# owkin/PyDESeq2

Measured on AMD Instinct MI355X. Metric: genes/sec end-to-end deseq2() (size factors->dispersion->IRLS->Wald), higher is better.
Workload: dtype f64

## Files before the change

include/deseq_hip.h:

```cpp
#ifndef DESEQ_HIP_H
#define DESEQ_HIP_H

#include <stddef.h>
#include <stdint.h>

#ifdef __cplusplus
extern "C" {
#endif

#define DSQ_ABI_VERSION 5
#define DSQ_MAX_P 128
#define DSQ_SHRINK_MAX_P 48
#define DSQ_BFGS_MAX_P 12

typedef struct dsq_ctx dsq_ctx;

enum dsq_status {
    DSQ_OK = 0,
    DSQ_ERR_HIP = -1,
    DSQ_ERR_ARG = -2,
    DSQ_ERR_RANGE = -3,
    DSQ_ERR_NOMEM = -4
};

// ... 15 lines not shown
int dsq_sync(dsq_ctx* ctx);
const char* dsq_debug_pending_error(void);
int dsq_timer_start(dsq_ctx* ctx);
int dsq_timer_stop(dsq_ctx* ctx, float* elapsed_ms);
int dsq_last_alpha_kernel(dsq_ctx* ctx, float* kernel_ms, int* n_grid_fallback);

int dsq_malloc(dsq_ctx* ctx, size_t bytes, void** dptr);
int dsq_free(dsq_ctx* ctx, void* dptr);
int dsq_memset(dsq_ctx* ctx, void* dptr, int value, size_t bytes);
int dsq_h2d(dsq_ctx* ctx, void* dst, const void* src, size_t bytes);
int dsq_d2h(dsq_ctx* ctx, void* dst, const void* src, size_t bytes);
int dsq_h2d_2d(dsq_ctx* ctx, void* dst, size_t dpitch, const void* src, size_t spitch,
               size_t row_bytes, size_t rows);
int dsq_d2h_2d(dsq_ctx* ctx, void* dst, size_t dpitch, const void* src, size_t spitch,
               size_t row_bytes, size_t rows);

int dsq_abi_version(void);
int dsq_plugin_cache_config(dsq_ctx* ctx, int enabled, long long budget_bytes);
int dsq_plugin_cache_clear(dsq_ctx* ctx);
int dsq_plugin_cache_stats(dsq_ctx* ctx, double* out, int n);
int dsq_plugin_digest_host(const void* data, int elem_type, int layout, int N, int G, int n_threads,
                           unsigned long long* out2);

int dsq_inf_lin_reg_mu(dsq_ctx* ctx, const void* counts, int count_type, int count_layout,
                       const double* size_factors, const double* design, int N, int G, int P,
                       double min_mu, double* mu_out);

int dsq_inf_irls2(dsq_ctx* ctx, const void* counts, int count_type, int count_layout,
                  const double* size_factors, const double* design, const double* disp, int N,
                  int G, int P, double min_mu, double beta_tol, double min_beta, double max_beta,
                  int maxiter, double* beta_out, double* mu_out, double* hat_out,
                  uint8_t* converged, int optimizer);
int dsq_inf_irls(dsq_ctx* ctx, const void* counts, int count_type, int count_layout,
                 const double* size_factors, const double* design, const double* disp, int N,
                 int G, int P, double min_mu, double beta_tol, double min_beta, double max_beta,
                 int maxiter, double* beta_out, double* mu_out, double* hat_out,
                 uint8_t* converged);

int dsq_inf_alpha_mle2(dsq_ctx* ctx, const void* counts, int count_type, int count_layout,
                       const double* design, const double* mu, int mu_layout,
                       const double* alpha_hat, int N, int G, int P, double min_disp,
                       double max_disp, double prior_disp_var, int cr_reg, int prior_reg,
                       double* alpha_out, uint8_t* converged, int optimizer);
int dsq_inf_alpha_mle(dsq_ctx* ctx, const void* counts, int count_type, int count_layout,
                      const double* design, const double* mu, int mu_layout,
                      const double* alpha_hat, int N, int G, int P, double min_disp,
                      double max_disp, double prior_disp_var, int cr_reg, int prior_reg,
                      double* alpha_out, uint8_t* converged);

int dsq_inf_wald_test(dsq_ctx* ctx, const double* design, const double* disp, const double* lfc,
                      const double* mu, int mu_layout, const double* ridge,
                      const double* contrast, double lfc_null, int alt, int N, int G, int P,
                      double* pvals, double* stats, double* se);

int dsq_inf_fit_rough_dispersions(dsq_ctx* ctx, const double* normed, int layout,
                                  const double* design, int N, int G, int P, double* alpha_out);
int dsq_inf_fit_moments_dispersions(dsq_ctx* ctx, const double* normed, int layout,
                                    const double* size_factors, int N, int G, double* alpha_out);
int dsq_inf_fit_moments_dispersions2(dsq_ctx* ctx, const double* normed, int layout, const double* size_factors,
                                     int N, int G, double* alpha_out, uint8_t* all_zero);

int dsq_inf_dispersion_trend_gamma_glm(dsq_ctx* ctx, const double* covariates, const double* targets, int n,
                                       double* coeffs2, double* predictions, int* converged);

int dsq_inf_grid_fit_alpha(dsq_ctx* ctx, const void* counts, int count_type, int count_layout, const double* design,
                           const double* mu, int mu_layout, int N, int G, int P, double min_disp, double max_disp,
                           double* log_alpha_out);
int dsq_inf_grid_fit_beta(dsq_ctx* ctx, const void* counts, int count_type, int count_layout,
                          const double* size_factors, const double* design, const double* disp, int N, int G,
                          double min_mu, int grid_length, double min_beta, double max_beta, double* beta_out);

int dsq_dev_trend_loss_grad(dsq_ctx* ctx, const double* d_cov, const double* d_targets,
                            const uint8_t* d_keep, int n, double a0, double a1, double* loss,
                            double* grad2);

int dsq_dev_trend_fit(dsq_ctx* ctx, const double* d_disp, const double* d_means, int n,
                      double min_disp, double max_disp, uint8_t* d_keep, double* h_coeffs2,
                      int* h_ok, int* h_n_outer);

size_t dsq_prior_mad_work_doubles(int n);
int dsq_dev_prior_mad(dsq_ctx* ctx, const double* d_gw_raw, const double* d_fitted, int n,
                      double min_disp, double max_disp, double* d_work, double* h_squared_logres);


int dsq_dev_counts_to_gene_major(dsq_ctx* ctx, const void* d_src, int count_type, int layout,
                                 int N, int G, int32_t* d_dst, int ldn, int* h_bad);
int dsq_dev_f64_to_gene_major(dsq_ctx* ctx, const double* d_src, int layout, int N, int G,
                              double* d_dst, int ldn);

int dsq_dev_logmeans(dsq_ctx* ctx, const int32_t* d_y, int ldn, int N, int G, double* d_logmeans,
                     uint8_t* d_nonzero);
size_t dsq_size_factors_work_doubles(int N, int G);
int dsq_dev_size_factors(dsq_ctx* ctx, const void* d_counts_sm, int count_type, int N, int G,
                         const double* d_logmeans, const uint8_t* d_gene_mask, double* d_work,
                         double* d_size_factors);
int dsq_dev_size_factors_new(dsq_ctx* ctx, const void* d_counts_sm, int count_type, int N, int G,
                             const double* d_logmeans, const uint8_t* d_gene_mask, double* d_work,
                             double* d_size_factors);
int dsq_dev_mom_lin_mu(dsq_ctx* ctx, const int32_t* d_y, int ldn, const double* d_sf, const double* d_Xt,
                       const double* d_pinvXt, int ldx, int N, int G, int P, double min_disp, double max_disp,
                       double min_mu, double* d_normed_mean, double* d_mom, double* d_mu);
int dsq_dev_mom(dsq_ctx* ctx, const int32_t* d_y, int ldn, const double* d_sf, const double* d_Xt,
                const double* d_pinvXt, int ldx, int N, int G, int P, double min_disp,
                double max_disp, double* d_normed_mean, double* d_rough, double* d_moments,
                double* d_mom);
int dsq_dev_lin_mu(dsq_ctx* ctx, const int32_t* d_y, int ldn, const double* d_sf,
                   const double* d_Xt, const double* d_pinvXt, int ldx, int N, int G, int P,
                   double min_mu, double* d_mu);
int dsq_dev_alpha_mle(dsq_ctx* ctx, const int32_t* d_y, const double* d_mu, int ldn,
                      const double* d_Xt, int ldx, int N, int G, int P, const double* d_alpha_hat,
                      double min_disp, double max_disp, double prior_disp_var, int cr_reg,
                      int prior_reg, double* d_alpha, uint8_t* d_converged, int32_t* d_nfev,
                      double* d_nll_const, int const_mode);
typedef struct dsq_cells {
    const int32_t* d_cell_of;
    const double* d_Xc;
    const double* d_XX;
    int n_cells;
} dsq_cells;
int dsq_dev_mom_lin_coef(dsq_ctx* ctx, const int32_t* d_y, int ldn, const double* d_sf, const double* d_Xt,
                         const double* d_pinvXt, int ldx, int N, int G, int P, double min_disp, double max_disp,
                         double min_mu, double* d_normed_mean, double* d_mom, double* d_mu, double* d_coef);
int dsq_dev_alpha_mle2(dsq_ctx* ctx, const int32_t* d_y, const double* d_mu, int ldn, const double* d_Xt, int ldx,
                       int N, int G, int P, const double* d_alpha_hat, double min_disp, double max_disp,
                       double prior_disp_var, int cr_reg, int prior_reg, double* d_alpha, uint8_t* d_converged,
                       int32_t* d_nfev, double* d_nll_const, int const_mode, const dsq_cells* cells,
                       const double* d_coef, const double* d_sf, double min_mu);
int dsq_dev_alpha_mle3(dsq_ctx* ctx, const int32_t* d_y, const double* d_mu, int ldn, const double* d_Xt, int ldx,
                       int N, int G, int P, const double* d_alpha_hat, double min_disp, double max_disp,
                       double prior_disp_var, int cr_reg, int prior_reg, double* d_alpha, uint8_t* d_converged,
                       int32_t* d_nfev, double* d_nll_const, int const_mode, const dsq_cells* cells,
                       const double* d_coef, const double* d_sf, double min_mu, const int32_t* d_rows, int n_rows,
                       const int32_t* d_waves, int n_waves, const double* d_cell_mu);
typedef struct dsq_mix dsq_mix;
int dsq_mix_create(dsq_ctx* ctx, const double* design, int N, int P, dsq_mix** out);
void dsq_mix_destroy(dsq_mix* mix);
int dsq_mix_info(const dsq_mix* mix, int* n_slots, int* n_cells, int* n_continuous);
int dsq_mix_slots(const dsq_mix* mix, int32_t* h_slot_of);
int dsq_mix_bind(dsq_ctx* ctx, const uint16_t* d_ys, const uint8_t* d_big, const double* d_mu_slots);
int dsq_mix_bind2(dsq_ctx* ctx, const uint16_t* d_ys, const uint8_t* d_big, const double* d_mu_slots, int G);
int dsq_dev_mix_counts_to_slots(dsq_ctx* ctx, const int32_t* d_y, int ldn, int G, const dsq_mix* mix, uint16_t* d_ys,
                                uint8_t* d_big);
int dsq_dev_mix_mu_slots(dsq_ctx* ctx, const dsq_mix* mix, const double* d_beta, const double* d_sf, int G,
                         double* d_mu_slots);
int dsq_mix_takes_irls(const dsq_mix* mix, int full_rank);
int dsq_mix_launch_count(void);
int dsq_dev_alpha_mle4(dsq_ctx* ctx, const int32_t* d_y, const double* d_mu, int ldn, const double* d_Xt, int ldx,
                       int N, int G, int P, const double* d_alpha_hat, double min_disp, double max_disp,
                       double prior_disp_var, int cr_reg, int prior_reg, double* d_alpha, uint8_t* d_converged,
                       int32_t* d_nfev, double* d_nll_const, int const_mode, const dsq_cells* cells,
                       const double* d_coef, const double* d_sf, double min_mu, const int32_t* d_rows, int n_rows,
                       const int32_t* d_waves, int n_waves, const double* d_cell_mu, const dsq_mix* mix,
                       const double* d_beta);
int dsq_alpha_rows_eligible(int N, int P, int n_cells);
int dsq_alpha_needs_mu(int N, int P, int n_cells);
int dsq_dev_cell_mu(dsq_ctx* ctx, const double* d_beta, const dsq_cells* cells, int G, int P, double* d_cell_mu);
int dsq_dev_alpha_row_split(dsq_ctx* ctx, const int32_t* d_y, int ldn, int N, int G, int32_t* d_flags);
int dsq_dev_robust_disp(dsq_ctx* ctx, const int32_t* d_y, int ldn, const double* d_sf, const int32_t* d_cell_offsets,
                        const int32_t* d_cell_index, int n_cells, int whole, int max_cell, int N, int G,
                        double* d_robust_disp);
int dsq_dev_robust_disp2(dsq_ctx* ctx, const int32_t* d_y, int ldn, const double* d_sf, const int32_t* d_cell_offsets,
                         const int32_t* d_cell_index, int n_cells, int whole, int max_cell, int min_cell, int N, int G,
                         double* d_robust_disp);
int dsq_dev_lfc_fit(dsq_ctx* ctx, const int32_t* d_y, int ldn, const double* d_sf, const double* d_Xt,
                    const double* d_pinvXt, int ldx, int N, int G, int P, int full_rank, const double* d_disp,
                    double min_mu, double beta_tol, double min_beta, double max_beta, int maxiter, double* d_beta,
                    double* d_mu, double* d_hat, uint8_t* d_converged, int32_t* d_iters, const dsq_cells* cells,
                    const double* d_robust_disp, const uint8_t* d_flags, double cutoff, double* d_cooks,
                    uint8_t* d_any_all, uint8_t* d_any_use, uint8_t* d_any_use_nr, uint8_t* d_few_above,
                    const double* h_ridge, const double* h_contrast, double lfc_null, int alt, double* d_pvals,
                    double* d_stats, double* d_se);
int dsq_dev_lfc_fit2(dsq_ctx* ctx, const int32_t* d_y, int ldn, const double* d_sf, const double* d_Xt,
                     const double* d_pinvXt, int ldx, int N, int G, int P, int full_rank, const double* d_disp,
                     double min_mu, double beta_tol, double min_beta, double max_beta, int maxiter, double* d_beta,
                     double* d_mu, double* d_hat, uint8_t* d_converged, int32_t* d_iters, const dsq_cells* cells,
                     const double* d_robust_disp, const uint8_t* d_flags, double cutoff, double* d_cooks,
                     uint8_t* d_any_all, uint8_t* d_any_use, uint8_t* d_any_use_nr, uint8_t* d_few_above,
                     const double* h_ridge, const double* h_contrast, double lfc_null, int alt, double* d_pvals,
                     double* d_stats, double* d_se, const dsq_mix* mix, int cooks_ld);
int dsq_dev_replace_outliers2(dsq_ctx* ctx, const int32_t* d_y, const double* d_cooks, int ldn, const double* d_sf,
                              const uint8_t* d_flags, const int32_t* d_gene_idx, int n_sel, int N, double cutoff,
                              int32_t* d_y_out, uint8_t* d_all_zero, int cooks_ld, const dsq_mix* mix);
int dsq_dev_irls_layers(dsq_ctx* ctx, const int32_t* d_y, int ldn, const double* d_sf, const double* d_Xt, int ldx,
                        int N, int G, int P, const double* d_disp, const double* d_beta, double min_mu, double* d_mu,
                        double* d_hat);
int dsq_side_begin(dsq_ctx* ctx);
int dsq_side_end(dsq_ctx* ctx);
int dsq_side_wait(dsq_ctx* ctx);
int dsq_side_abort(dsq_ctx* ctx);
int dsq_dev_irls(dsq_ctx* ctx, const int32_t* d_y, int ldn, const double* d_sf, const double* d_Xt,
                 const double* d_pinvXt, int ldx, int N, int G, int P, int full_rank,
                 const double* d_disp, double min_mu, double beta_tol, double min_beta,
                 double max_beta, int maxiter, double* d_beta, double* d_mu, double* d_hat,
                 uint8_t* d_converged, int32_t* d_iters);
int dsq_dev_cooks(dsq_ctx* ctx, const int32_t* d_y, int ldn, const double* d_sf, const double* d_mu,
                  const double* d_hat, const int32_t* d_cell_offsets, const int32_t* d_cell_index,
                  int n_cells, int whole, int max_cell, const uint8_t* d_flags, int N, int G, int P,
                  double cutoff, double* d_cooks, double* d_robust_disp, uint8_t* d_any_all,
                  uint8_t* d_any_use, uint8_t* d_any_use_nr, uint8_t* d_few_above);
int dsq_dev_replace_outliers(dsq_ctx* ctx, const int32_t* d_y, const double* d_cooks, int ldn,
                             const double* d_sf, const uint8_t* d_flags, const int32_t* d_gene_idx,
                             int n_sel, int N, double cutoff, int32_t* d_y_out,
                             uint8_t* d_all_zero);
int dsq_dev_wald(dsq_ctx* ctx, const double* d_mu, int ldn, const double* d_sf, const double* d_Xt,
                 int ldx, int N, int G, int P, const double* d_disp, const double* d_beta,
                 const double* h_ridge, const double* h_contrast, double lfc_null, int alt,
                 double* d_pvals, double* d_stats, double* d_se);
int dsq_dev_lrt(dsq_ctx* ctx, const int32_t* d_y, int ldn, const double* d_sf, const double* d_Xt, int ldx, int P,
                const double* d_Xt_reduced, int ldx_reduced, int P_reduced, int N, int G, const double* d_disp,
                const double* d_beta, const double* d_beta_reduced, double* d_stats, double* d_pvals);
int dsq_dev_chisq_sf(dsq_ctx* ctx, const double* d_x, int n, int df, double* d_out);
int dsq_dev_trend_prior(dsq_ctx* ctx, const double* d_disp, const double* d_means, int n, double min_disp,
                        double max_disp, uint8_t* d_keep, double* d_fitted, double* d_work, double* h_coeffs2,
                        int* h_ok, int* h_n_outer, double* h_squared_logres);
int dsq_lfc_fork_begin(dsq_ctx* ctx);
int dsq_lfc_fork_end(dsq_ctx* ctx);
int dsq_lfc_set_part(dsq_ctx* ctx, const uint8_t* d_part, int want, int phase);
int dsq_lfc_takes_parts(int N, int P, const dsq_cells* cells, const dsq_mix* mix, int full_rank);
int dsq_dev_select_dispersions_part(dsq_ctx* ctx, double* d_genewise_raw, double* d_map_raw, const double* d_fitted, int n,
                                    double min_disp, double max_disp, double squared_logres, double* d_disp,
                                    uint8_t* d_outlier, uint8_t* d_map_converged, const uint8_t* d_conv_late, uint8_t* d_part,
                                    int mode, int ready_limit);
int dsq_alpha_set_late_flags(dsq_ctx* ctx, uint8_t* d_conv_late);
int dsq_lfc_prepare(dsq_ctx* ctx, const double* d_sf, int N, const double* h_ridge, const double* h_contrast, int P);
int dsq_dev_trend_eval(dsq_ctx* ctx, const double* d_normed_means, int n, double a0, double a1,
                       double* d_fitted);
int dsq_dev_select_dispersions(dsq_ctx* ctx, double* d_genewise_raw, double* d_map_raw,
                               const double* d_fitted, int n, double min_disp, double max_disp,
                               double squared_logres, double* d_disp, uint8_t* d_outlier);
int dsq_dev_scatter_rows_f64(dsq_ctx* ctx, const double* d_src, const int32_t* d_idx, int n_idx, int width,
                             double* d_dst);
int dsq_dev_mom_raw(dsq_ctx* ctx, const int32_t* d_y, int ldn, const double* d_ones, const double* d_sf,
                    const double* d_Xt, const double* d_pinvXt, int ldx, int N, int G, int P, double min_disp,
                    double max_disp, double* d_normed_mean, double* d_mom);
int dsq_dev_nll_const(dsq_ctx* ctx, const int32_t* d_y, int ldn, int N, int G, const double* d_disp, double* d_cst);
int dsq_dev_nll_scaled(dsq_ctx* ctx, const int32_t* d_y, const double* d_mu, int ldn, int N, int G,
                       const double* d_disp, const double* d_scale, const double* d_cst, double* d_nll);
int dsq_dev_logmeans_poscounts(dsq_ctx* ctx, const int32_t* d_y, int ldn, int N, int G, double* d_logmeans,
                               uint8_t* d_usable);
int dsq_dev_vst(dsq_ctx* ctx, const void* d_counts_sm, int count_type, int N, int G, const double* d_sf, int mode,
                double a0, double a1, double* d_out);
int dsq_inf_lfc_shrink_nbinom_glm2(dsq_ctx* ctx, const void* counts, int count_type, int count_layout,
                                   const double* design, const double* size, const double* offset, int N, int G,
                                   int P, double prior_no_shrink_scale, double prior_scale, int shrink_index,
                                   double* beta_out, double* inv_hessian_out, uint8_t* converged, int optimizer);
int dsq_inf_lfc_shrink_nbinom_glm(dsq_ctx* ctx, const void* counts, int count_type, int count_layout,
                                  const double* design, const double* size, const double* offset, int N, int G,
                                  int P, double prior_no_shrink_scale, double prior_scale, int shrink_index,
                                  double* beta_out, double* inv_hessian_out, uint8_t* converged);
int dsq_dev_lfc_shrink(dsq_ctx* ctx, const int32_t* d_y, int ldn, const double* d_offset, const double* d_Xt,
                       int ldx, int N, int G, int P, const double* d_size, double prior_no_shrink_scale,
                       double prior_scale, int shrink_index, double* d_beta, double* d_inv_hessian,
                       uint8_t* d_converged);
int dsq_dev_lfc_shrink2(dsq_ctx* ctx, const int32_t* d_y, int ldn, const double* d_offset, const double* d_Xt,
                        int ldx, int N, int G, int P, const double* d_size, double prior_no_shrink_scale,
                        double prior_scale, int shrink_index, double* d_beta, double* d_inv_hessian,
                        uint8_t* d_converged, double* d_ih_entry);
int dsq_dev_lfc_shrink3(dsq_ctx* ctx, const int32_t* d_y, int ldn, const double* d_offset, const double* d_Xt,
                        int ldx, int N, int G, int P, const double* d_size, double prior_no_shrink_scale,
                        double prior_scale, int shrink_index, double* d_beta, double* d_inv_hessian,
                        uint8_t* d_converged, double* d_ih_entry, int optimizer);
int dsq_dev_padj_prepare(dsq_ctx* ctx, const double* d_base_mean, const double* d_pvalue, int n, double alpha,
                         unsigned long long* d_sorted_p, int32_t* d_sorted_idx, uint8_t* d_bins,
                         double* h_out200, int* h_n_valid);
int dsq_dev_padj_finish(dsq_ctx* ctx, const unsigned long long* d_sorted_p, const int32_t* d_sorted_idx,
                        const uint8_t* d_bins, int n, int n_valid, int j, double* d_padj);
int dsq_upload_counts_i32(dsq_ctx* ctx, const void* counts, int count_type, size_t n_elems, int32_t* d_dst,
                          int* h_bad);
int dsq_d2d(dsq_ctx* ctx, void* d_dst, const void* d_src, size_t bytes);
int dsq_host_alloc(dsq_ctx* ctx, size_t bytes, void** out);
int dsq_host_free(dsq_ctx* ctx, void* p);
int dsq_d2h_async(dsq_ctx* ctx, void* pinned_dst, const void* d_src, size_t bytes);
int dsq_h2d_async(dsq_ctx* ctx, void* d_dst, const void* pinned_src, size_t bytes);
int dsq_dev_gather_rows_f64(dsq_ctx* ctx, const double* d_src, int ld, const int32_t* d_idx,
                            int n_idx, int ncols, double* d_dst);
int dsq_dev_gather_rows_i32(dsq_ctx* ctx, const int32_t* d_src, int ld, const int32_t* d_idx,
                            int n_idx, int ncols, int32_t* d_dst);

int dsq_comm_unique_id(dsq_ctx* ctx, char* out128, int len);
int dsq_comm_init(dsq_ctx* ctx, const char* uid128, int rank, int world);
int dsq_comm_destroy(dsq_ctx* ctx);
int dsq_comm_allreduce_sum(dsq_ctx* ctx, void* d_buf, size_t count, int dtype );
int dsq_comm_allgather(dsq_ctx* ctx, const void* d_send, void* d_recv, size_t bytes_per_rank);
int dsq_comm_info(dsq_ctx* ctx, int* nranks, int* rank);
unsigned long long dsq_host_sync_count(void);
int dsq_dev_pack2(dsq_ctx* ctx, const double* d_a, const double* d_b, int n, int len, double* d_send);
int dsq_dev_unzip2(dsq_ctx* ctx, const double* d_recv, int world, int len, double* d_a_all, double* d_b_all);

int dsq_dev_sf_keys(dsq_ctx* ctx, const void* d_counts_sm, int count_type, int N, int G,
                    const double* d_logmeans, const uint8_t* d_gene_mask, void* d_keys);
int dsq_dev_sf_keys_compact(dsq_ctx* ctx, const void* d_counts_sm, int count_type, int N, int G,
                            const double* d_logmeans, const uint8_t* d_gene_mask, int32_t* d_idx_work, void* d_keys,
                            int* h_n_usable);
int dsq_dev_sf_count(dsq_ctx* ctx, const void* d_keys, int N, int G, uint32_t* d_counts);
int dsq_dev_sf_init(dsq_ctx* ctx, const uint32_t* d_total, int N, void* d_prefix, uint32_t* d_rank);
int dsq_dev_sf_hist(dsq_ctx* ctx, const void* d_keys, int N, int G, const void* d_prefix, int shift,
                    uint32_t* d_hist);
int dsq_dev_sf_pick(dsq_ctx* ctx, const uint32_t* d_hist, int N, int shift, void* d_prefix,
                    uint32_t* d_rank);
int dsq_dev_sf_finish(dsq_ctx* ctx, const void* d_prefix, const uint32_t* d_total, int N, double* d_sf);

#ifdef __cplusplus
}
#endif
#endif
```

pydeseq2_amd/_lib.py:

```python
from __future__ import annotations

import ctypes as C
import os

import numpy as np

_HERE = os.path.dirname(os.path.abspath(__file__))
LIB_PATH = os.environ.get("DSQ_LIB", os.path.join(_HERE, "libdeseq_hip.so"))

DSQ_MAX_P = 128
DSQ_SHRINK_MAX_P = 48
_DEBUG = bool(os.environ.get("DSQ_DEBUG"))
SAMPLE_MAJOR, GENE_MAJOR = 0, 1
I32, I64 = 0, 1
ALT = {None: 0, "greaterAbs": 1, "lessAbs": 2, "greater": 3, "less": 4}

c_void_p, c_int, c_double, c_size_t = C.c_void_p, C.c_int, C.c_double, C.c_size_t
_vp = c_void_p
HOOK_FN = C.CFUNCTYPE(None, c_void_p)


class DsqCells(C.Structure):

    _fields_ = [("d_cell_of", C.c_void_p), ("d_Xc", C.c_void_p), ("d_XX", C.c_void_p), ("n_cells", C.c_int)]


class DsqError(RuntimeError):
    """A libdeseq_hip call failed (HIP error, bad argument, out of memory)."""


_lib = None


def load():
    global _lib
    if _lib is not None:
        return _lib
    if not os.path.exists(LIB_PATH):
        raise DsqError(
            f"{LIB_PATH} not found: build it with `make -C pydeseq2_amd/csrc` "
            "(or __graft_entry__.build()).  pydeseq2_amd has no CPU fallback."
        )
    lib = C.CDLL(LIB_PATH)

    def proto(name, *argtypes, res=c_int):
        fn = getattr(lib, name)
        fn.argtypes = list(argtypes)
        fn.restype = res
        return fn

    proto("dsq_create", c_int, C.POINTER(_vp))
    proto("dsq_destroy", _vp, res=None)
    proto("dsq_last_error", _vp, res=C.c_char_p)
    proto("dsq_device_info", _vp, C.c_char_p, c_int, C.POINTER(c_int), C.POINTER(c_size_t), C.c_char_p, c_int)
    proto("dsq_sync", _vp)
    proto("dsq_debug_pending_error", res=C.c_char_p)
    proto("dsq_timer_start", _vp)
    proto("dsq_timer_stop", _vp, C.POINTER(C.c_float))
    proto("dsq_last_alpha_kernel", _vp, C.POINTER(C.c_float), C.POINTER(c_int))
    proto("dsq_malloc", _vp, c_size_t, C.POINTER(_vp))
    proto("dsq_free", _vp, _vp)
    proto("dsq_memset", _vp, _vp, c_int, c_size_t)
    proto("dsq_h2d", _vp, _vp, _vp, c_size_t)
    proto("dsq_d2h", _vp, _vp, _vp, c_size_t)
    proto("dsq_h2d_2d", _vp, _vp, c_size_t, _vp, c_size_t, c_size_t, c_size_t)
    proto("dsq_d2h_2d", _vp, _vp, c_size_t, _vp, c_size_t, c_size_t, c_size_t)
    proto("dsq_inf_lin_reg_mu", _vp, _vp, c_int, c_int, _vp, _vp, c_int, c_int, c_int, c_double, _vp)
    proto("dsq_inf_irls2", _vp, _vp, c_int, c_int, _vp, _vp, _vp, c_int, c_int, c_int, c_double, c_double,
          c_double, c_double, c_int, _vp, _vp, _vp, _vp, c_int)
    proto("dsq_inf_irls", _vp, _vp, c_int, c_int, _vp, _vp, _vp, c_int, c_int, c_int, c_double, c_double,
          c_double, c_double, c_int, _vp, _vp, _vp, _vp)
    proto("dsq_inf_alpha_mle2", _vp, _vp, c_int, c_int, _vp, _vp, c_int, _vp, c_int, c_int, c_int, c_double,
          c_double, c_double, c_int, c_int, _vp, _vp, c_int)
    proto("dsq_inf_alpha_mle", _vp, _vp, c_int, c_int, _vp, _vp, c_int, _vp, c_int, c_int, c_int, c_double,
          c_double, c_double, c_int, c_int, _vp, _vp)
    proto("dsq_abi_version", res=c_int)
    proto("dsq_plugin_cache_config", _vp, c_int, C.c_longlong)
    proto("dsq_plugin_cache_clear", _vp)
    proto("dsq_plugin_cache_stats", _vp, C.POINTER(c_double), c_int)
    proto("dsq_comm_info", _vp, C.POINTER(c_int), C.POINTER(c_int))
    proto("dsq_mix_bind", _vp, _vp, _vp, _vp)
    proto("dsq_mix_bind2", _vp, _vp, _vp, _vp, c_int)
    proto("dsq_dev_mix_counts_to_slots", _vp, _vp, c_int, c_int, _vp, _vp, _vp)
    proto("dsq_dev_mix_mu_slots", _vp, _vp, _vp, _vp, c_int, _vp)
    proto("dsq_host_sync_count", res=C.c_ulonglong)
    proto("dsq_dev_pack2", _vp, _vp, _vp, c_int, c_int, _vp)
    proto("dsq_dev_unzip2", _vp, _vp, c_int, c_int, _vp, _vp)
    proto("dsq_plugin_digest_host", _vp, c_int, c_int, c_int, c_int, c_int, C.POINTER(C.c_ulonglong))
    proto("dsq_inf_wald_test", _vp, _vp, _vp, _vp, _vp, c_int, _vp, _vp, c_double, c_int, c_int, c_int,
          c_int, _vp, _vp, _vp)
    proto("dsq_inf_fit_rough_dispersions", _vp, _vp, c_int, _vp, c_int, c_int, c_int, _vp)
    proto("dsq_inf_fit_moments_dispersions", _vp, _vp, c_int, _vp, c_int, c_int, _vp)
    proto("dsq_inf_fit_moments_dispersions2", _vp, _vp, c_int, _vp, c_int, c_int, _vp, _vp)
    proto("dsq_inf_dispersion_trend_gamma_glm", _vp, _vp, _vp, c_int, _vp, _vp, C.POINTER(c_int))
    proto("dsq_inf_grid_fit_alpha", _vp, _vp, c_int, c_int, _vp, _vp, c_int, c_int, c_int, c_int, c_double, c_double,
          _vp)
    proto("dsq_inf_grid_fit_beta", _vp, _vp, c_int, c_int, _vp, _vp, _vp, c_int, c_int, c_double, c_int, c_double,
          c_double, _vp)
    proto("dsq_dev_trend_loss_grad", _vp, _vp, _vp, _vp, c_int, c_double, c_double, C.POINTER(c_double),
          C.POINTER(c_double))
    proto("dsq_dev_trend_fit", _vp, _vp, _vp, c_int, c_double, c_double, _vp, C.POINTER(c_double),
          C.POINTER(c_int), C.POINTER(c_int))
    proto("dsq_dev_prior_mad", _vp, _vp, _vp, c_int, c_double, c_double, _vp, C.POINTER(c_double))
    proto("dsq_dev_counts_to_gene_major", _vp, _vp, c_int, c_int, c_int, c_int, _vp, c_int, C.POINTER(c_int))
    proto("dsq_dev_f64_to_gene_major", _vp, _vp, c_int, c_int, c_int, _vp, c_int)
    proto("dsq_dev_logmeans", _vp, _vp, c_int, c_int, c_int, _vp, _vp)
    proto("dsq_dev_size_factors", _vp, _vp, c_int, c_int, c_int, _vp, _vp, _vp, _vp)
    proto("dsq_dev_size_factors_new", _vp, _vp, c_int, c_int, c_int, _vp, _vp, _vp, _vp)
    proto("dsq_dev_mom", _vp, _vp, c_int, _vp, _vp, _vp, c_int, c_int, c_int, c_int, c_double, c_double,
          _vp, _vp, _vp, _vp)
    proto("dsq_dev_lin_mu", _vp, _vp, c_int, _vp, _vp, _vp, c_int, c_int, c_int, c_int, c_double, _vp)
    proto("dsq_dev_trend_eval", _vp, _vp, c_int, c_double, c_double, _vp)
    proto("dsq_dev_trend_prior", _vp, _vp, _vp, c_int, c_double, c_double, _vp, _vp, _vp, _vp, _vp, _vp, _vp)
    proto("dsq_dev_select_dispersions", _vp, _vp, _vp, _vp, c_int, c_double, c_double, c_double, _vp, _vp)
    proto("dsq_dev_scatter_rows_f64", _vp, _vp, _vp, c_int, c_int, _vp)
    proto("dsq_dev_sf_keys_compact", _vp, _vp, c_int, c_int, c_int, _vp, _vp, _vp, _vp, C.POINTER(c_int))
    proto("dsq_prior_mad_work_doubles", c_int, res=c_size_t)
    proto("dsq_size_factors_work_doubles", c_int, c_int, res=c_size_t)
    proto("dsq_dev_mom_lin_mu", _vp, _vp, c_int, _vp, _vp, _vp, c_int, c_int, c_int, c_int, c_double, c_double,
          c_double, _vp, _vp, _vp)
    proto("dsq_dev_mom_raw", _vp, _vp, c_int, _vp, _vp, _vp, _vp, c_int, c_int, c_int, c_int, c_double, c_double,
          _vp, _vp)
    proto("dsq_dev_nll_const", _vp, _vp, c_int, c_int, c_int, _vp, _vp)
    proto("dsq_dev_nll_scaled", _vp, _vp, _vp, c_int, c_int, c_int, _vp, _vp, _vp, _vp)
    proto("dsq_dev_logmeans_poscounts", _vp, _vp, c_int, c_int, c_int, _vp, _vp)
    proto("dsq_dev_vst", _vp, _vp, c_int, c_int, c_int, _vp, c_int, c_double, c_double, _vp)
    proto("dsq_inf_lfc_shrink_nbinom_glm2", _vp, _vp, c_int, c_int, _vp, _vp, _vp, c_int, c_int, c_int, c_double,
          c_double, c_int, _vp, _vp, _vp, c_int)
    proto("dsq_inf_lfc_shrink_nbinom_glm", _vp, _vp, c_int, c_int, _vp, _vp, _vp, c_int, c_int, c_int, c_double,
          c_double, c_int, _vp, _vp, _vp)
    proto("dsq_dev_lfc_shrink", _vp, _vp, c_int, _vp, _vp, c_int, c_int, c_int, c_int, _vp, c_double, c_double,
          c_int, _vp, _vp, _vp)
    proto("dsq_dev_lfc_shrink2", _vp, _vp, c_int, _vp, _vp, c_int, c_int, c_int, c_int, _vp, c_double, c_double,
          c_int, _vp, _vp, _vp, _vp)
    proto("dsq_dev_lfc_shrink3", _vp, _vp, c_int, _vp, _vp, c_int, c_int, c_int, c_int, _vp, c_double, c_double,
          c_int, _vp, _vp, _vp, _vp, c_int)
    proto("dsq_dev_padj_prepare", _vp, _vp, _vp, c_int, c_double, _vp, _vp, _vp, _vp, C.POINTER(c_int))
    proto("dsq_dev_padj_finish", _vp, _vp, _vp, _vp, c_int, c_int, c_int, _vp)
    proto("dsq_d2d", _vp, _vp, _vp, c_size_t)
    cells_p = C.POINTER(DsqCells)
    proto("dsq_dev_mom_lin_coef", _vp, _vp, c_int, _vp, _vp, _vp, c_int, c_int, c_int, c_int, c_double, c_double,
          c_double, _vp, _vp, _vp, _vp)
    proto("dsq_dev_alpha_mle2", _vp, _vp, _vp, c_int, _vp, c_int, c_int, c_int, c_int, _vp, c_double, c_double,
          c_double, c_int, c_int, _vp, _vp, _vp, _vp, c_int, cells_p, _vp, _vp, c_double)
    proto("dsq_dev_alpha_mle3", _vp, _vp, _vp, c_int, _vp, c_int, c_int, c_int, c_int, _vp, c_double, c_double,
          c_double, c_int, c_int, _vp, _vp, _vp, _vp, c_int, cells_p, _vp, _vp, c_double, _vp, c_int, _vp, c_int, _vp)
    proto("dsq_dev_alpha_mle4", _vp, _vp, _vp, c_int, _vp, c_int, c_int, c_int, c_int, _vp, c_double, c_double,
          c_double, c_int, c_int, _vp, _vp, _vp, _vp, c_int, cells_p, _vp, _vp, c_double, _vp, c_int, _vp, c_int, _vp,
          _vp, _vp)
    proto("dsq_mix_create", _vp, _vp, c_int, c_int, C.POINTER(_vp))
    proto("dsq_mix_destroy", _vp, res=None)
    proto("dsq_mix_launch_count")
    proto("dsq_mix_slots", _vp, _vp)
    proto("dsq_mix_takes_irls", _vp, c_int)
    proto("dsq_mix_info", _vp, C.POINTER(c_int), C.POINTER(c_int), C.POINTER(c_int))
    proto("dsq_alpha_rows_eligible", c_int, c_int, c_int)
    proto("dsq_alpha_needs_mu", c_int, c_int, c_int)
    proto("dsq_dev_cell_mu", _vp, _vp, cells_p, c_int, c_int, _vp)
    proto("dsq_dev_alpha_row_split", _vp, _vp, c_int, c_int, c_int, _vp)
    proto("dsq_dev_robust_disp", _vp, _vp, c_int, _vp, _vp, _vp, c_int, c_int, c_int, c_int, c_int, _vp)
    proto("dsq_dev_robust_disp2", _vp, _vp, c_int, _vp, _vp, _vp, c_int, c_int, c_int, c_int, c_int, c_int, _vp)
    proto("dsq_dev_lfc_fit", _vp, _vp, c_int, _vp, _vp, _vp, c_int, c_int, c_int, c_int, c_int, _vp, c_double,
          c_double, c_double, c_double, c_int, _vp, _vp, _vp, _vp, _vp, cells_p, _vp, _vp, c_double, _vp, _vp, _vp,
          _vp, _vp, _vp, _vp, c_double, c_int, _vp, _vp, _vp)
    proto("dsq_dev_lfc_fit2", _vp, _vp, c_int, _vp, _vp, _vp, c_int, c_int, c_int, c_int, c_int, _vp, c_double,
          c_double, c_double, c_double, c_int, _vp, _vp, _vp, _vp, _vp, cells_p, _vp, _vp, c_double, _vp, _vp, _vp,
          _vp, _vp, _vp, _vp, c_double, c_int, _vp, _vp, _vp, _vp, c_int)
    proto("dsq_dev_irls_layers", _vp, _vp, c_int, _vp, _vp, c_int, c_int, c_int, c_int, _vp, _vp, c_double, _vp, _vp)
    proto("dsq_side_begin", _vp)
    proto("dsq_side_end", _vp)
    proto("dsq_side_wait", _vp)
    proto("dsq_side_abort", _vp)
    proto("dsq_set_deferred", _vp, c_int)
    proto("dsq_lfc_fork_begin", _vp)
    proto("dsq_lfc_fork_end", _vp)
    proto("dsq_lfc_set_part", _vp, _vp, c_int, c_int)
    proto("dsq_lfc_takes_parts", c_int, c_int, cells_p, _vp, c_int)
    proto("dsq_dev_select_dispersions_part", _vp, _vp, _vp, _vp, c_int, c_double, c_double, c_double, _vp, _vp, _vp, _vp, _vp,
          c_int, c_int)
    proto("dsq_alpha_set_late_flags", _vp, _vp)
    proto("dsq_lfc_prepare", _vp, _vp, c_int, _vp, _vp, c_int)
    proto("dsq_irls_order_hint", _vp, _vp, c_int)
    proto("dsq_set_alpha_hook", _vp, _vp, _vp)
    proto("dsq_upload_counts_i32", _vp, _vp, c_int, c_size_t, _vp, C.POINTER(c_int))
    proto("dsq_host_alloc", _vp, c_size_t, C.POINTER(_vp))
    proto("dsq_host_free", _vp, _vp)
    proto("dsq_d2h_async", _vp, _vp, _vp, c_size_t)
    proto("dsq_h2d_async", _vp, _vp, _vp, c_size_t)
    proto("dsq_dev_alpha_mle", _vp, _vp, _vp, c_int, _vp, c_int, c_int, c_int, c_int, _vp, c_double,
          c_double, c_double, c_int, c_int, _vp, _vp, _vp, _vp, c_int)
    proto("dsq_dev_irls", _vp, _vp, c_int, _vp, _vp, _vp, c_int, c_int, c_int, c_int, c_int, _vp, c_double,
          c_double, c_double, c_double, c_int, _vp, _vp, _vp, _vp, _vp)
    proto("dsq_dev_cooks", _vp, _vp, c_int, _vp, _vp, _vp, _vp, _vp, c_int, c_int, c_int, _vp, c_int, c_int,
          c_int, c_double, _vp, _vp, _vp, _vp, _vp, _vp)
    proto("dsq_dev_replace_outliers", _vp, _vp, _vp, c_int, _vp, _vp, _vp, c_int, c_int, c_double, _vp, _vp)
    proto("dsq_dev_replace_outliers2", _vp, _vp, _vp, c_int, _vp, _vp, _vp, c_int, c_int, c_double, _vp, _vp, c_int, _vp)
    proto("dsq_dev_wald", _vp, _vp, c_int, _vp, _vp, c_int, c_int, c_int, c_int, _vp, _vp, _vp, _vp,
          c_double, c_int, _vp, _vp, _vp)
    proto("dsq_dev_lrt", _vp, _vp, c_int, _vp, _vp, c_int, c_int, _vp, c_int, c_int, c_int, c_int, _vp, _vp, _vp, _vp, _vp)
    proto("dsq_dev_chisq_sf", _vp, _vp, c_int, c_int, _vp)
    proto("dsq_dev_gather_rows_f64", _vp, _vp, c_int, _vp, c_int, c_int, _vp)
    proto("dsq_dev_gather_rows_i32", _vp, _vp, c_int, _vp, c_int, c_int, _vp)
    proto("dsq_comm_unique_id", _vp, C.c_char_p, c_int)
    proto("dsq_comm_init", _vp, C.c_char_p, c_int, c_int)
    proto("dsq_comm_destroy", _vp)
    proto("dsq_comm_allreduce_sum", _vp, _vp, c_size_t, c_int)
    proto("dsq_comm_allgather", _vp, _vp, _vp, c_size_t)
    proto("dsq_dev_sf_keys", _vp, _vp, c_int, c_int, c_int, _vp, _vp, _vp)
    proto("dsq_dev_sf_count", _vp, _vp, c_int, c_int, _vp)
    proto("dsq_dev_sf_init", _vp, _vp, c_int, _vp, _vp)
    proto("dsq_dev_sf_hist", _vp, _vp, c_int, c_int, _vp, c_int, _vp)
    proto("dsq_dev_sf_pick", _vp, _vp, c_int, c_int, _vp, _vp)
    proto("dsq_dev_sf_finish", _vp, _vp, _vp, c_int, _vp)
    _lib = lib
    return lib


EXPORTS = [
    "dsq_create", "dsq_destroy", "dsq_last_error", "dsq_device_info", "dsq_sync", "dsq_debug_pending_error", "dsq_timer_start",
    "dsq_timer_stop", "dsq_last_alpha_kernel", "dsq_malloc", "dsq_free", "dsq_memset", "dsq_h2d", "dsq_d2h", "dsq_h2d_2d",
    "dsq_d2h_2d", "dsq_inf_lin_reg_mu", "dsq_inf_irls", "dsq_inf_alpha_mle", "dsq_inf_wald_test",
    "dsq_inf_fit_rough_dispersions", "dsq_inf_fit_moments_dispersions", "dsq_dev_trend_loss_grad", "dsq_dev_trend_fit", "dsq_dev_prior_mad",
    "dsq_dev_counts_to_gene_major", "dsq_dev_f64_to_gene_major", "dsq_dev_logmeans",
    "dsq_dev_size_factors", "dsq_dev_mom", "dsq_dev_lin_mu", "dsq_dev_alpha_mle", "dsq_dev_irls",
    "dsq_dev_cooks", "dsq_dev_replace_outliers", "dsq_dev_wald", "dsq_dev_gather_rows_f64",
    "dsq_dev_gather_rows_i32", "dsq_comm_unique_id", "dsq_comm_init", "dsq_comm_destroy",
    "dsq_comm_allreduce_sum", "dsq_comm_allgather", "dsq_dev_sf_keys", "dsq_dev_sf_count", "dsq_dev_sf_init",
    "dsq_dev_sf_hist", "dsq_dev_sf_pick", "dsq_dev_sf_finish", "dsq_dev_trend_eval", "dsq_dev_trend_prior", "dsq_dev_select_dispersions",
    "dsq_dev_scatter_rows_f64", "dsq_d2d", "dsq_dev_mom_lin_mu", "dsq_dev_sf_keys_compact", "dsq_prior_mad_work_doubles", "dsq_size_factors_work_doubles", "dsq_dev_mom_raw", "dsq_dev_nll_const", "dsq_dev_nll_scaled", "dsq_dev_logmeans_poscounts", "dsq_dev_vst", "dsq_inf_lfc_shrink_nbinom_glm", "dsq_dev_lfc_shrink", "dsq_dev_lfc_shrink2", "dsq_dev_lfc_shrink3", "dsq_dev_padj_prepare", "dsq_dev_padj_finish", "dsq_host_alloc", "dsq_host_free", "dsq_d2h_async", "dsq_h2d_async",
    "dsq_dev_size_factors_new", "dsq_dev_mom_lin_coef", "dsq_dev_alpha_mle2", "dsq_dev_robust_disp", "dsq_dev_robust_disp2", "dsq_dev_lfc_fit", "dsq_dev_lfc_fit2", "dsq_dev_irls_layers",
    "dsq_side_begin", "dsq_side_end", "dsq_side_wait", "dsq_side_abort", "dsq_set_deferred", "dsq_irls_order_hint", "dsq_set_alpha_hook", "dsq_dev_alpha_mle3", "dsq_dev_alpha_mle4", "dsq_mix_create", "dsq_mix_destroy", "dsq_mix_info", "dsq_mix_slots", "dsq_mix_takes_irls", "dsq_dev_replace_outliers2", "dsq_mix_launch_count", "dsq_alpha_rows_eligible", "dsq_alpha_needs_mu", "dsq_dev_cell_mu", "dsq_dev_alpha_row_split",
    "dsq_upload_counts_i32", "dsq_inf_dispersion_trend_gamma_glm", "dsq_inf_grid_fit_alpha", "dsq_inf_grid_fit_beta",
    "dsq_inf_irls2", "dsq_inf_alpha_mle2", "dsq_inf_lfc_shrink_nbinom_glm2", "dsq_inf_fit_moments_dispersions2",
    "dsq_abi_version", "dsq_plugin_cache_config", "dsq_plugin_cache_clear", "dsq_plugin_cache_stats",
    "dsq_plugin_digest_host", "dsq_comm_info", "dsq_host_sync_count", "dsq_dev_pack2", "dsq_dev_unzip2",
    "dsq_mix_bind", "dsq_mix_bind2", "dsq_dev_mix_counts_to_slots", "dsq_dev_mix_mu_slots",
    "dsq_lfc_fork_begin", "dsq_lfc_fork_end", "dsq_lfc_set_part", "dsq_lfc_takes_parts", "dsq_dev_select_dispersions_part", "dsq_lfc_prepare", "dsq_alpha_set_late_flags",
    "dsq_dev_lrt", "dsq_dev_chisq_sf",
]


def ptr(a):
    if a is None:
        return None
    if isinstance(a, np.ndarray):
        return a.ctypes.data
    return a


class Context:

    def __init__(self, device: int = 0):
        self.lib = load()
        h = _vp()
        rc = self.lib.dsq_create(int(device), C.byref(h))
        if rc != 0 or not h.value:
            raise DsqError(
                f"dsq_create(device={device}) failed (rc={rc}): no usable MI355X / HIP runtime. "
                "pydeseq2_amd runs on the GPU only."
            )
        self.h = h
        self.device = device

    def close(self):
        if getattr(self, "h", None) is not None and self.h.value:
            for bufs in self.__dict__.pop("_padj_buffers", {}).values():
                for b in bufs:
                    b.free()
            self.lib.dsq_destroy(self.h)
            self.h = _vp()

    def __del__(self):
        try:
            self.close()
        except Exception:
            pass

    def call(self, name, *args):
        rc = getattr(self.lib, name)(self.h, *args)
        if _DEBUG:
            pend = self.lib.dsq_debug_pending_error().decode()
            if pend:
                print(f"[dsq debug] pending HIP error after {name}: {pend}", flush=True)
        if rc != 0:
            msg = self.lib.dsq_last_error(self.h).decode(errors="replace")
            if rc == -2:
                raise ValueError(msg)
            raise DsqError(f"{name} failed (rc={rc}): {msg}")

    def device_info(self):
        name, arch = C.create_string_buffer(256), C.create_string_buffer(256)
        cu, mem = c_int(), c_size_t()
        self.call("dsq_device_info", name, 256, C.byref(cu), C.byref(mem), arch, 256)
        return dict(name=name.value.decode(), arch=arch.value.decode(), cu_count=cu.value, mem_bytes=mem.value)

    def sync(self):
        self.call("dsq_sync")

    def timer_start(self):
        self.call("dsq_timer_start")

    def timer_stop(self) -> float:
        ms = C.c_float()
        self.call("dsq_timer_stop", C.byref(ms))
        return float(ms.value)

    def malloc(self, nbytes: int) -> int:
        p = _vp()
        self.call("dsq_malloc", c_size_t(int(nbytes)), C.byref(p))
        return p.value

    def free(self, dptr):
        if dptr:
            self.call("dsq_free", _vp(dptr))

    def memset(self, dptr, value, nbytes):
        self.call("dsq_memset", _vp(dptr), int(value), c_size_t(int(nbytes)))

    def h2d(self, dptr, arr: np.ndarray):
        arr = np.ascontiguousarray(arr)
        self.call("dsq_h2d", _vp(dptr), _vp(arr.ctypes.data), c_size_t(arr.nbytes))

    def d2h(self, arr: np.ndarray, dptr):
        assert arr.flags.c_contiguous
        self.call("dsq_d2h", _vp(arr.ctypes.data), _vp(dptr), c_size_t(arr.nbytes))
        return arr

    def d2h_rows(self, dptr, rows, cols, ld, dtype=np.float64):
        out = np.empty((rows, cols), dtype=dtype)
        isz = out.itemsize
        self.call("dsq_d2h_2d", _vp(out.ctypes.data), c_size_t(cols * isz), _vp(dptr), c_size_t(ld * isz),
                  c_size_t(cols * isz), c_size_t(rows))
        return out

    def h2d_rows(self, dptr, arr: np.ndarray, ld):
        arr = np.ascontiguousarray(arr)
        rows, cols = arr.shape
        isz = arr.itemsize
        self.call("dsq_h2d_2d", _vp(dptr), c_size_t(ld * isz), _vp(arr.ctypes.data), c_size_t(cols * isz),
                  c_size_t(cols * isz), c_size_t(rows))


class DeviceArray:

    def __init__(self, ctx: Context, shape, dtype, ld=None):
        self.ctx = ctx
        self.shape = tuple(shape) if isinstance(shape, (tuple, list)) else (int(shape),)
        self.dtype = np.dtype(dtype)
        self.ld = ld if ld is not None else (self.shape[-1] if len(self.shape) > 1 else None)
        n = self.shape[0] * (self.ld if len(self.shape) > 1 else 1)
        self.nbytes = int(n) * self.dtype.itemsize
        self.ptr = ctx.malloc(self.nbytes)

    @classmethod
    def from_host(cls, ctx, arr, ld=None):
        arr = np.ascontiguousarray(arr)
        self = cls(ctx, arr.shape, arr.dtype, ld)
        if arr.ndim == 2 and self.ld != arr.shape[1]:
            ctx.h2d_rows(self.ptr, arr, self.ld)
        else:
            ctx.h2d(self.ptr, arr)
        return self

    def to_host(self):
        if len(self.shape) == 2 and self.ld != self.shape[1]:
            return self.ctx.d2h_rows(self.ptr, self.shape[0], self.shape[1], self.ld, self.dtype)
        out = np.empty(self.shape, dtype=self.dtype)
        return self.ctx.d2h(out, self.ptr)

    def free(self):
        if self.ptr:
            self.ctx.free(self.ptr)
            self.ptr = 0

    def __del__(self):
        try:
            self.free()
        except Exception:
            pass


class _PinnedPool:

    def __init__(self, ctx):
        self.ctx, self.free, self.closed = ctx, [], False

    def take(self, nbytes):
        best = None
        for k, (cap, ptr) in enumerate(self.free):
            if nbytes <= cap <= 2 * nbytes + 65536 and (best is None or cap < self.free[best][0]):
                best = k
# ... 46 lines not shown
```

pydeseq2_amd/csrc/dsq_alpha_rows.h:

```cpp
#pragma once
#include "dsq_alpha.h"
#include "dsq_launch.h"

namespace dsq {

constexpr int kRowLanes = 16;
constexpr int kRowSlots = 4;
constexpr int kRowWaves = 4;
constexpr int kRowBlock = 64 * kRowWaves;

struct RowGene {
    Lbfgsb1d m;
    double cst, la_hat;
    double q[4];
    int g;
    int n_tail;
    int n_big;
    int pad_;
};

DSQ_HD size_t row_slot_bytes(int npad) {
    return (sizeof(RowGene) + (size_t)npad * 2 + (size_t)kRowTail * 2 + 15) & ~(size_t)15;
}

DSQ_D void stirling_big(double z, double& lg, double& psi) {
    const double l = flog_t(z), rc = frcp(z);
    lg = (z - 0.5) * l - z + kHalfLog2Pi + stirling_tail_big(rc);
    psi = l + digamma_tail_big(rc);
}


}
```

pydeseq2_amd/csrc/dsq_capi_dev.hip:

```cpp
#include "dsq_capi_internal.h"

extern "C" {

int dsq_dev_counts_to_gene_major(dsq_ctx* ctx, const void* d_src, int count_type, int layout, int N, int G,
                                 int32_t* d_dst, int ldn, int* h_bad) {
    DSQ_CHECK_ARG(ldn >= N, "ldn < N");
    int* d_bad = (int*)ctx->d_scratch;
    DSQ_HIP(hipMemsetAsync(d_bad, 0, sizeof(int), ctx->stream));
    DSQ_HIP(dsq::launch_transpose_counts(ctx->stream, d_src, count_type, layout, N, G, d_dst, ldn, d_bad));
    if (h_bad) {
        DSQ_HIP(hipMemcpyAsync(h_bad, d_bad, sizeof(int), hipMemcpyDeviceToHost, ctx->stream));
        DSQ_HIP(hipStreamSynchronize(ctx->stream));
    }
    return DSQ_OK;
}

int dsq_dev_f64_to_gene_major(dsq_ctx* ctx, const double* d_src, int layout, int N, int G, double* d_dst,
                              int ldn) {
    DSQ_HIP(dsq::launch_transpose_f64(ctx->stream, d_src, layout, N, G, d_dst, ldn));
    return DSQ_OK;
}

int dsq_dev_logmeans(dsq_ctx* ctx, const int32_t* d_y, int ldn, int N, int G, double* d_logmeans,
                     uint8_t* d_nonzero) {
    DSQ_HIP(dsq::launch_logmeans(ctx->stream, d_y, ldn, N, G, d_logmeans, d_nonzero));
    return DSQ_OK;
}

int dsq_dev_logmeans_poscounts(dsq_ctx* ctx, const int32_t* d_y, int ldn, int N, int G, double* d_logmeans,
                               uint8_t* d_usable) {
    DSQ_HIP(dsq::launch_logmeans_pos(ctx->stream, d_y, ldn, N, G, d_logmeans, d_usable));
    return DSQ_OK;
}

size_t dsq_size_factors_work_doubles(int N, int G) { return dsq::size_factors_work_doubles(N, G); }

int dsq_dev_size_factors(dsq_ctx* ctx, const void* d_counts_sm, int count_type, int N, int G,
                         const double* d_logmeans, const uint8_t* d_gene_mask, double* d_work,
                         double* d_size_factors) {
    DSQ_HIP(dsq::launch_size_factors(ctx->stream, d_counts_sm, count_type, N, G, d_logmeans, d_gene_mask,
                                     d_work, d_size_factors));
    return DSQ_OK;
}

int dsq_dev_size_factors_new(dsq_ctx* ctx, const void* d_counts_sm, int count_type, int N, int G,
                             const double* d_logmeans, const uint8_t* d_gene_mask, double* d_work,
                             double* d_size_factors) {
    DSQ_HIP(dsq::launch_size_factors(ctx->stream, d_counts_sm, count_type, N, G, d_logmeans, d_gene_mask,
                                     d_work, d_size_factors, 1));
    return DSQ_OK;
}

int dsq_dev_mom(dsq_ctx* ctx, const int32_t* d_y, int ldn, const double* d_sf, const double* d_Xt,
                const double* d_pinvXt, int ldx, int N, int G, int P, double min_disp, double max_disp,
                double* d_normed_mean, double* d_rough, double* d_moments, double* d_mom) {
    DSQ_CHECK_ARG(P >= 1 && P <= DSQ_MAX_P, "P out of range");
    DSQ_CHECK_ARG(N != P, "The number of samples and the number of design variables are equal, i.e., "
                          "there are no replicates to estimate the dispersion.");
    DSQ_HIP(dsq::launch_mom(ctx->stream, d_y, ldn, d_sf, d_Xt, d_pinvXt, ldx, N, G, P, min_disp, max_disp,
                            d_normed_mean, d_rough, d_moments, d_mom, ctx->d_scratch + 8));
    return DSQ_OK;
}

int dsq_dev_mom_lin_mu(dsq_ctx* ctx, const int32_t* d_y, int ldn, const double* d_sf, const double* d_Xt,
                       const double* d_pinvXt, int ldx, int N, int G, int P, double min_disp, double max_disp,
                       double min_mu, double* d_normed_mean, double* d_mom, double* d_mu) {
    DSQ_CHECK_ARG(P >= 1 && P <= DSQ_MAX_P, "P out of range");
    DSQ_CHECK_ARG(N != P, "The number of samples and the number of design variables are equal, i.e., "
                          "there are no replicates to estimate the dispersion.");
    DSQ_HIP(dsq::launch_mom_lin_mu(ctx->stream, d_y, ldn, d_sf, d_Xt, d_pinvXt, ldx, N, G, P, min_disp, max_disp,
                                   min_mu, d_normed_mean, d_mom, d_mu, ctx->d_scratch + 8));
    return DSQ_OK;
}

int dsq_dev_mom_lin_coef(dsq_ctx* ctx, const int32_t* d_y, int ldn, const double* d_sf, const double* d_Xt,
                         const double* d_pinvXt, int ldx, int N, int G, int P, double min_disp, double max_disp,
                         double min_mu, double* d_normed_mean, double* d_mom, double* d_mu, double* d_coef) {
    DSQ_CHECK_ARG(P >= 1 && P <= DSQ_MAX_P, "P out of range");
    DSQ_CHECK_ARG(N != P, "The number of samples and the number of design variables are equal, i.e., "
                          "there are no replicates to estimate the dispersion.");
    DSQ_HIP(dsq::launch_mom_lin_mu(ctx->stream, d_y, ldn, d_sf, d_Xt, d_pinvXt, ldx, N, G, P, min_disp, max_disp,
                                   min_mu, d_normed_mean, d_mom, d_mu, ctx->d_scratch + 8, d_coef));
    return DSQ_OK;
}

int dsq_dev_mom_raw(dsq_ctx* ctx, const int32_t* d_y, int ldn, const double* d_ones, const double* d_sf,
                    const double* d_Xt, const double* d_pinvXt, int ldx, int N, int G, int P, double min_disp,
                    double max_disp, double* d_normed_mean, double* d_mom) {
    DSQ_CHECK_ARG(P >= 1 && P <= DSQ_MAX_P, "P out of range");
    DSQ_CHECK_ARG(N != P, "The number of samples and the number of design variables are equal, i.e., "
                          "there are no replicates to estimate the dispersion.");
    DSQ_HIP(dsq::launch_mom(ctx->stream, d_y, ldn, d_ones, d_Xt, d_pinvXt, ldx, N, G, P, min_disp, max_disp,
                            d_normed_mean, nullptr, nullptr, d_mom, ctx->d_scratch + 8, d_sf));
    return DSQ_OK;
}

int dsq_dev_nll_const(dsq_ctx* ctx, const int32_t* d_y, int ldn, int N, int G, const double* d_disp, double* d_cst) {
    DSQ_HIP(dsq::launch_nll_const(ctx->stream, d_y, ldn, N, G, d_disp, d_cst));
    return DSQ_OK;
}

int dsq_dev_nll_scaled(dsq_ctx* ctx, const int32_t* d_y, const double* d_mu, int ldn, int N, int G,
                       const double* d_disp, const double* d_scale, const double* d_cst, double* d_nll) {
    DSQ_HIP(dsq::launch_nll_scaled(ctx->stream, d_y, d_mu, ldn, N, G, d_disp, d_scale, d_cst, d_nll));
    return DSQ_OK;
}

int dsq_dev_lin_mu(dsq_ctx* ctx, const int32_t* d_y, int ldn, const double* d_sf, const double* d_Xt,
                   const double* d_pinvXt, int ldx, int N, int G, int P, double min_mu, double* d_mu) {
    DSQ_CHECK_ARG(P >= 1 && P <= DSQ_MAX_P, "P out of range");
    DSQ_HIP(dsq::launch_lin_mu(ctx->stream, d_y, ldn, d_sf, d_Xt, d_pinvXt, ldx, N, G, P, min_mu, d_mu));
    return DSQ_OK;
}

int dsq_dev_alpha_mle(dsq_ctx* ctx, const int32_t* d_y, const double* d_mu, int ldn, const double* d_Xt,
                      int ldx, int N, int G, int P, const double* d_alpha_hat, double min_disp,
                      double max_disp, double prior_disp_var, int cr_reg, int prior_reg, double* d_alpha,
                      uint8_t* d_converged, int32_t* d_nfev, double* d_nll_const, int const_mode) {
    DSQ_CHECK_ARG(P >= 1 && P <= DSQ_MAX_P, "P out of range");
    DSQ_CHECK_ARG(const_mode >= DSQ_CONST_COMPUTE && const_mode <= DSQ_CONST_LOAD, "const_mode out of range");
    return run_alpha(ctx, d_y, d_mu, ldn, d_Xt, ldx, N, G, P, d_alpha_hat, min_disp, max_disp, prior_disp_var,
                     cr_reg, prior_reg, d_alpha, d_converged, d_nfev, d_nll_const, const_mode);
}


int dsq_set_alpha_hook(dsq_ctx* ctx, dsq_hook_fn fn, void* arg) {
    ctx->alpha_hook = fn;
    ctx->alpha_hook_arg = arg;
    return DSQ_OK;
}

int dsq_irls_order_hint(dsq_ctx* ctx, const int32_t* d_iters, int G) {
    ctx->d_irls_hint = d_iters;
    ctx->irls_hint_genes = d_iters != nullptr ? G : 0;
    return DSQ_OK;
}


int dsq_dev_irls(dsq_ctx* ctx, const int32_t* d_y, int ldn, const double* d_sf, const double* d_Xt,
                 const double* d_pinvXt, int ldx, int N, int G, int P, int full_rank, const double* d_disp,
                 double min_mu, double beta_tol, double min_beta, double max_beta, int maxiter,
                 double* d_beta, double* d_mu, double* d_hat, uint8_t* d_converged, int32_t* d_iters) {
    DSQ_CHECK_ARG(P >= 1 && P <= DSQ_MAX_P, "P out of range");
    return run_irls(ctx, d_y, ldn, d_sf, d_Xt, d_pinvXt, ldx, N, G, P, full_rank, d_disp, min_mu, beta_tol, min_beta,
                    max_beta, maxiter, d_beta, d_mu, d_hat, d_converged, d_iters, nullptr);
}


int dsq_dev_alpha_mle4(dsq_ctx* ctx, const int32_t* d_y, const double* d_mu, int ldn, const double* d_Xt, int ldx,
                       int N, int G, int P, const double* d_alpha_hat, double min_disp, double max_disp,
                       double prior_disp_var, int cr_reg, int prior_reg, double* d_alpha, uint8_t* d_converged,
                       int32_t* d_nfev, double* d_nll_const, int const_mode, const dsq_cells* cells,
                       const double* d_coef, const double* d_sf, double min_mu, const int32_t* d_rows, int n_rows,
                       const int32_t* d_waves, int n_waves, const double* d_cell_mu, const dsq_mix* mix,
                       const double* d_beta) {
    DSQ_CHECK_ARG(P >= 1 && P <= DSQ_MAX_P, "P out of range");
    DSQ_CHECK_ARG(const_mode >= DSQ_CONST_COMPUTE && const_mode <= DSQ_CONST_LOAD, "const_mode out of range");
    DSQ_CHECK_ARG(d_mu != nullptr || (d_coef != nullptr && d_sf != nullptr) ||
                      (d_cell_mu != nullptr && d_sf != nullptr && cells != nullptr && cells->n_cells > 0) ||
                      (mix != nullptr && d_beta != nullptr && d_sf != nullptr),
                  "mu_hat is needed as a matrix, as (coef, sf), as (cell_mu, sf, cells) or as (mix, beta, sf)");
    DSQ_CHECK_ARG(mix == nullptr || (mix->d.P == P && mix->d.N == N && d_rows != nullptr),
                  "mix: built for another design, or the gene lists are missing");
    DSQ_CHECK_ARG(d_beta == nullptr || (mix != nullptr && d_mu == nullptr && d_coef == nullptr && d_cell_mu == nullptr &&
                                        n_waves == 0),
                  "beta: with mix only, alone, and every gene on the mixed-design kernel");
    DSQ_CHECK_ARG(d_cell_mu == nullptr || (d_mu == nullptr && d_coef == nullptr && !dsq::alpha_is_wide(P, cells->n_cells)),
                  "cell_mu: alone, on the register kernels");
    DSQ_CHECK_ARG(cells == nullptr || cells->n_cells <= dsq::kMaxCells, "too many design cells for the cell path");
    DSQ_CHECK_ARG(d_rows == nullptr || (n_rows >= 0 && n_waves >= 0 && n_rows + n_waves == G &&
                                        (n_waves == 0 || d_waves != nullptr)),
                  "the two gene lists must partition the G genes of the call");
    dsq::AlphaExtras ex{};
    ex.cells = to_cells(cells);
    if (d_mu == nullptr) { ex.coef = d_coef; ex.cell_mu = d_cell_mu; ex.sf = d_sf; ex.min_mu = min_mu; }
    if (d_rows != nullptr) { ex.rows = d_rows; ex.n_rows = n_rows; ex.waves = d_waves; ex.n_waves = n_waves; }
    if (mix != nullptr) { ex.mix = &mix->d; ex.mix_beta = d_beta; ex.sf = d_sf; }
    return run_alpha(ctx, d_y, d_mu, ldn, d_Xt, ldx, N, G, P, d_alpha_hat, min_disp, max_disp, prior_disp_var, cr_reg,
                     prior_reg, d_alpha, d_converged, d_nfev, d_nll_const, const_mode, &ex);
}

int dsq_dev_alpha_mle3(dsq_ctx* ctx, const int32_t* d_y, const double* d_mu, int ldn, const double* d_Xt, int ldx,
                       int N, int G, int P, const double* d_alpha_hat, double min_disp, double max_disp,
                       double prior_disp_var, int cr_reg, int prior_reg, double* d_alpha, uint8_t* d_converged,
                       int32_t* d_nfev, double* d_nll_const, int const_mode, const dsq_cells* cells,
                       const double* d_coef, const double* d_sf, double min_mu, const int32_t* d_rows, int n_rows,
                       const int32_t* d_waves, int n_waves, const double* d_cell_mu) {
    return dsq_dev_alpha_mle4(ctx, d_y, d_mu, ldn, d_Xt, ldx, N, G, P, d_alpha_hat, min_disp, max_disp, prior_disp_var,
                              cr_reg, prior_reg, d_alpha, d_converged, d_nfev, d_nll_const, const_mode, cells, d_coef,
                              d_sf, min_mu, d_rows, n_rows, d_waves, n_waves, d_cell_mu, nullptr, nullptr);
}

int dsq_dev_alpha_mle2(dsq_ctx* ctx, const int32_t* d_y, const double* d_mu, int ldn, const double* d_Xt, int ldx,
                       int N, int G, int P, const double* d_alpha_hat, double min_disp, double max_disp,
                       double prior_disp_var, int cr_reg, int prior_reg, double* d_alpha, uint8_t* d_converged,
                       int32_t* d_nfev, double* d_nll_const, int const_mode, const dsq_cells* cells,
                       const double* d_coef, const double* d_sf, double min_mu) {
    return dsq_dev_alpha_mle3(ctx, d_y, d_mu, ldn, d_Xt, ldx, N, G, P, d_alpha_hat, min_disp, max_disp, prior_disp_var,
                              cr_reg, prior_reg, d_alpha, d_converged, d_nfev, d_nll_const, const_mode, cells, d_coef,
                              d_sf, min_mu, nullptr, 0, nullptr, 0, nullptr);
}

int dsq_mix_create(dsq_ctx* ctx, const double* design, int N, int P, dsq_mix** out) {
    DSQ_CHECK_ARG(out != nullptr && design != nullptr, "null argument");
    *out = nullptr;
    DSQ_HIP(hipSetDevice(ctx->device));
    if (P < 1 || P > dsq::kMixMaxP || N < 2 || N > 65535 || !dsq::alpha_mix_enabled()) return DSQ_OK;
    const bool force = getenv("DSQ_MIX_FORCE") != nullptr;
    std::vector<int> nd((size_t)P), order((size_t)P);
    for (int j = 0; j < P; ++j) {
        std::vector<double> col((size_t)N);
        for (int n = 0; n < N; ++n) col[(size_t)n] = design[(size_t)n * P + j];
        std::sort(col.begin(), col.end());
        nd[(size_t)j] = (int)(std::unique(col.begin(), col.end()) - col.begin());
        order[(size_t)j] = j;
    }
    std::stable_sort(order.begin(), order.end(), [&](int a, int b) { return nd[(size_t)a] > nd[(size_t)b]; });
    std::vector<char> cont((size_t)P, 0);
    std::vector<int> idx((size_t)N), cell((size_t)N);
    int C = 0;
    auto less_cat = [&](int a, int b) {
        for (int j = 0; j < P; ++j) {
            if (cont[(size_t)j]) continue;
            const double va = design[(size_t)a * P + j], vb = design[(size_t)b * P + j];
            if (va != vb) return va < vb;
        }
        return a < b;
    };
    auto same_cat = [&](int a, int b) {
        for (int j = 0; j < P; ++j)
            if (!cont[(size_t)j] && design[(size_t)a * P + j] != design[(size_t)b * P + j]) return false;
        return true;
    };
    auto find_cells = [&]() {
        for (int n = 0; n < N; ++n) idx[(size_t)n] = n;
        std::sort(idx.begin(), idx.end(), less_cat);
        C = 0;
        for (int k = 0; k < N; ++k) {
            if (k > 0 && !same_cat(idx[(size_t)k - 1], idx[(size_t)k])) ++C;
            cell[(size_t)idx[(size_t)k]] = C;
        }
        ++C;
    };
    int Q = 0;
    find_cells();
    while (C > dsq::kMixMaxCells && Q < dsq::kMixMaxQ && Q < P) {
        cont[(size_t)order[(size_t)Q]] = 1;
        ++Q;
        find_cells();
    }
    if (Q == 0 || C > dsq::kMixMaxCells) return DSQ_OK;
    std::vector<int> count((size_t)C, 0);
    for (int n = 0; n < N; ++n) ++count[(size_t)cell[(size_t)n]];
    const int blk = 64 * dsq::kMixU;
    int Ns = 0;
    for (int c = 0; c < C; ++c) Ns += (count[(size_t)c] + blk - 1) / blk * blk;
    Ns = (Ns + 255) & ~255;
    if (!force && Ns > N + N / 2 + 256) return DSQ_OK;
    dsq::MixDesign M{};
    M.Ns = Ns; M.C = C; M.Q = Q; M.P = P; M.N = N;
    {
        int q = 0;
        for (int j = 0; j < P; ++j) {
            M.colq[j] = cont[(size_t)j] ? q : -1;
            if (cont[(size_t)j]) M.zcol[q++] = j;
        }
    }
    if (!dsq::alpha_mix_fits(M)) return DSQ_OK;
    std::vector<int32_t> perm((size_t)Ns, -1), slot_of((size_t)N, 0);
    std::vector<uint8_t> trip_cell((size_t)(Ns / 64), (uint8_t)(C - 1));
    std::vector<double> Zs((size_t)Q * Ns, 0.0), Xc((size_t)C * P, 0.0), Ginv;
    {
        int s = 0, k = 0;
        for (int c = 0; c < C; ++c) {
            const int s0 = s;
            for (int i = 0; i < count[(size_t)c]; ++i, ++k, ++s) {
                const int n = idx[(size_t)k];
                perm[(size_t)s] = n;
                slot_of[(size_t)n] = s;
                for (int q = 0; q < Q; ++q) Zs[(size_t)q * Ns + s] = design[(size_t)n * P + M.zcol[q]];
                if (i == 0)
                    for (int j = 0; j < P; ++j) Xc[(size_t)c * P + j] = cont[(size_t)j] ? 0.0 : design[(size_t)n * P + j];
            }
            s = s0 + (count[(size_t)c] + blk - 1) / blk * blk;
            for (int t = s0 / 64; t < s / 64; ++t) trip_cell[(size_t)t] = (uint8_t)c;
        }
    }
    {
        std::vector<long double> A((size_t)P * P, 0.0L), Li((size_t)P * P, 0.0L);
        for (int n = 0; n < N; ++n)
            for (int i = 0; i < P; ++i)
                for (int j = 0; j <= i; ++j) A[(size_t)i * P + j] += (long double)design[(size_t)n * P + i] * design[(size_t)n * P + j];
        bool ok = true;
        long double dmax_ = 0.0L;
        for (int i = 0; i < P; ++i) dmax_ = std::max(dmax_, A[(size_t)i * P + i]);
        for (int j = 0; j < P && ok; ++j) {
            long double d = A[(size_t)j * P + j];
            for (int k = 0; k < j; ++k) d -= A[(size_t)j * P + k] * A[(size_t)j * P + k];
            if (!(d > dmax_ * 1e-13L)) { ok = false; break; }
            d = std::sqrt(d);
            A[(size_t)j * P + j] = d;
            for (int i = j + 1; i < P; ++i) {
                long double v = A[(size_t)i * P + j];
                for (int k = 0; k < j; ++k) v -= A[(size_t)i * P + k] * A[(size_t)j * P + k];
                A[(size_t)i * P + j] = v / d;
            }
        }
        if (ok) {
            for (int j = 0; j < P; ++j) {
                Li[(size_t)j * P + j] = 1.0L / A[(size_t)j * P + j];
                for (int i = j + 1; i < P; ++i) {
                    long double v = 0.0L;
                    for (int k = j; k < i; ++k) v -= A[(size_t)i * P + k] * Li[(size_t)k * P + j];
                    Li[(size_t)i * P + j] = v / A[(size_t)i * P + i];
                }
            }
            Ginv.assign((size_t)P * P, 0.0);
            for (int i = 0; i < P; ++i)
                for (int j = 0; j < P; ++j) {
                    long double v = 0.0L;
                    for (int k = std::max(i, j); k < P; ++k) v += Li[(size_t)k * P + i] * Li[(size_t)k * P + j];
                    Ginv[(size_t)i * P + j] = (double)v;
                }
        }
    }
    auto up = [](size_t b) { return (b + 255) & ~(size_t)255; };
    const size_t b_perm = up((size_t)Ns * 4), b_tc = up((size_t)Ns / 64), b_z = up((size_t)Q * Ns * 8),
                 b_xc = up((size_t)C * P * 8), b_g = up((size_t)P * P * 8), b_so = up((size_t)N * 4);
    dsq_mix* m = new dsq_mix();
    m->device = ctx->device;
    hipError_t e = hipMalloc(&m->d_block, b_perm + b_tc + b_z + b_xc + b_g + b_so);
    if (e != hipSuccess) { delete m; return fail(ctx, DSQ_ERR_HIP, std::string("dsq_mix_create: ") + hipGetErrorString(e)); }
    char* p = (char*)m->d_block;
    auto put = [&](const void* src, size_t bytes, size_t slot) {
        char* dst = p;
        if (e == hipSuccess && bytes) e = hipMemcpy(dst, src, bytes, hipMemcpyHostToDevice);
        p += slot;
        return dst;
    };
    M.perm = (const int32_t*)put(perm.data(), (size_t)Ns * 4, b_perm);
    M.trip_cell = (const uint8_t*)put(trip_cell.data(), (size_t)Ns / 64, b_tc);
    M.Zs = (const double*)put(Zs.data(), (size_t)Q * Ns * 8, b_z);
    M.Xc = (const double*)put(Xc.data(), (size_t)C * P * 8, b_xc);
    const char* g = put(Ginv.empty() ? nullptr : Ginv.data(), Ginv.empty() ? 0 : (size_t)P * P * 8, b_g);
    M.Ginv = Ginv.empty() ? nullptr : (const double*)g;
    M.slot_of = (const int32_t*)put(slot_of.data(), (size_t)N * 4, b_so);
    if (e != hipSuccess) {
        (void)hipFree(m->d_block);
        delete m;
        return fail(ctx, DSQ_ERR_HIP, std::string("dsq_mix_create: ") + hipGetErrorString(e));
    }
    m->d = M;
    *out = m;
    return DSQ_OK;
}

void dsq_mix_destroy(dsq_mix* mix) {
    if (mix == nullptr) return;
    (void)hipSetDevice(mix->device);
    if (mix->d_block) (void)hipFree(mix->d_block);
    delete mix;
}

int dsq_mix_slots(const dsq_mix* mix, int32_t* h_slot_of) {
    if (mix == nullptr || h_slot_of == nullptr) return DSQ_ERR_ARG;
    return hipMemcpy(h_slot_of, mix->d.slot_of, (size_t)mix->d.N * sizeof(int32_t), hipMemcpyDeviceToHost) == hipSuccess
               ? DSQ_OK
               : DSQ_ERR_HIP;
}

int dsq_mix_bind(dsq_ctx* ctx, const uint16_t* d_ys, const uint8_t* d_big, const double* d_mu_slots) {
    ctx->bind_ys = d_ys;
    ctx->bind_big = d_big;
    ctx->bind_mu = d_mu_slots;
    ctx->bind_G = 0;
    return DSQ_OK;
}

int dsq_mix_bind2(dsq_ctx* ctx, const uint16_t* d_ys, const uint8_t* d_big, const double* d_mu_slots, int G) {
    const int rc = dsq_mix_bind(ctx, d_ys, d_big, d_mu_slots);
    ctx->bind_G = (rc == DSQ_OK && G > 0) ? G : 0;
    return rc;
}
int dsq_dev_mix_counts_to_slots(dsq_ctx* ctx, const int32_t* d_y, int ldn, int G, const dsq_mix* mix, uint16_t* d_ys,
                                uint8_t* d_big) {
    DSQ_CHECK_ARG(mix != nullptr && d_y != nullptr && d_ys != nullptr && d_big != nullptr, "null argument");
    DSQ_HIP(dsq::launch_mix_counts_to_slots(ctx->stream, d_y, ldn, mix->d, G, d_ys, d_big));
    return DSQ_OK;
}
int dsq_dev_mix_mu_slots(dsq_ctx* ctx, const dsq_mix* mix, const double* d_beta, const double* d_sf, int G,
                         double* d_mu_slots) {
    DSQ_CHECK_ARG(mix != nullptr && d_beta != nullptr && d_sf != nullptr && d_mu_slots != nullptr, "null argument");
    DSQ_HIP(dsq::launch_mix_mu_slots(ctx->stream, d_beta, d_sf, mix->d, G, d_mu_slots));
    return DSQ_OK;
}

int dsq_mix_takes_irls(const dsq_mix* mix, int full_rank) {
    return (mix != nullptr && dsq::irls_takes_mix(&mix->d, full_rank)) ? 1 : 0;
}

int dsq_mix_launch_count(void) { return dsq::alpha_mix_launches(); }

int dsq_mix_info(const dsq_mix* mix, int* n_slots, int* n_cells, int* n_continuous) {
    if (mix == nullptr) return DSQ_ERR_ARG;
    if (n_slots) *n_slots = mix->d.Ns;
    if (n_cells) *n_cells = mix->d.C;
    if (n_continuous) *n_continuous = mix->d.Q;
    return DSQ_OK;
}

int dsq_alpha_needs_mu(int N, int P, int n_cells) { return dsq::alpha_needs_mu(N, P, n_cells) ? 1 : 0; }

int dsq_alpha_rows_eligible(int N, int P, int n_cells) {
    if (dsq::alpha_rows_eligible(N, P, n_cells, true, 1)) return 1;
    return dsq::alpha_rowsc_tail(N, P, n_cells) > 0 ? 2 : 0;
}

int dsq_dev_cell_mu(dsq_ctx* ctx, const double* d_beta, const dsq_cells* cells, int G, int P, double* d_cell_mu) {
    DSQ_CHECK_ARG(P >= 1 && P <= 12 && cells != nullptr && cells->n_cells > 0, "cells / P out of range");
    DSQ_HIP(dsq::launch_cell_mu(ctx->stream, d_beta, cells->d_Xc, cells->n_cells, G, P, d_cell_mu));
    return DSQ_OK;
}

int dsq_dev_alpha_row_split(dsq_ctx* ctx, const int32_t* d_y, int ldn, int N, int G, int32_t* d_flags) {
    DSQ_HIP(dsq::launch_count_big(ctx->stream, d_y, ldn, N, G, d_flags));
    return DSQ_OK;
}

int dsq_dev_robust_disp2(dsq_ctx* ctx, const int32_t* d_y, int ldn, const double* d_sf, const int32_t* d_cell_offsets,
                         const int32_t* d_cell_index, int n_cells, int whole, int max_cell, int min_cell, int N, int G,
                         double* d_robust_disp) {
    if (whole) min_cell = N;
    {
        const hipError_t pend = hipGetLastError();
        if (pend != hipSuccess)
            return fail(ctx, DSQ_ERR_HIP, std::string("HIP error pending before dsq_dev_robust_disp2: ") + hipGetErrorString(pend));
    }
    if ((size_t)G + 1 > ctx->redo_cap) {
        if (ctx->d_redo) (void)hipFree(ctx->d_redo);
        ctx->d_redo = nullptr; ctx->redo_cap = 0;
        DSQ_HIP(hipMalloc((void**)&ctx->d_redo, ((size_t)G + 1 + (size_t)G / 4) * sizeof(int32_t)));
        ctx->redo_cap = (size_t)G + 1 + (size_t)G / 4;
    }
    DSQ_HIP(dsq::launch_robust_disp(ctx->stream, d_y, ldn, d_sf, d_cell_offsets, d_cell_index, n_cells, whole, max_cell,
                                    N, G, d_robust_disp, min_cell, ctx->d_redo));
    return DSQ_OK;
}

int dsq_dev_robust_disp(dsq_ctx* ctx, const int32_t* d_y, int ldn, const double* d_sf, const int32_t* d_cell_offsets,
                        const int32_t* d_cell_index, int n_cells, int whole, int max_cell, int N, int G,
                        double* d_robust_disp) {
    return dsq_dev_robust_disp2(ctx, d_y, ldn, d_sf, d_cell_offsets, d_cell_index, n_cells, whole, max_cell, 0, N, G,
                                d_robust_disp);
}

int dsq_dev_irls_layers(dsq_ctx* ctx, const int32_t* d_y, int ldn, const double* d_sf, const double* d_Xt, int ldx,
                        int N, int G, int P, const double* d_disp, const double* d_beta, double min_mu, double* d_mu,
                        double* d_hat) {
    DSQ_CHECK_ARG(P >= 1 && P <= DSQ_MAX_P, "P out of range");
    DSQ_HIP(dsq::launch_irls_layers(ctx->stream, d_y, ldn, d_sf, d_Xt, ldx, N, G, P, d_disp, d_beta, min_mu, d_mu,
                                    d_hat));
    return DSQ_OK;
}


int dsq_dev_lfc_fit2(dsq_ctx* ctx, const int32_t* d_y, int ldn, const double* d_sf, const double* d_Xt,
                     const double* d_pinvXt, int ldx, int N, int G, int P, int full_rank, const double* d_disp,
                     double min_mu, double beta_tol, double min_beta, double max_beta, int maxiter, double* d_beta,
                     double* d_mu, double* d_hat, uint8_t* d_converged, int32_t* d_iters, const dsq_cells* cells,
                     const double* d_robust_disp, const uint8_t* d_flags, double cutoff, double* d_cooks,
                     uint8_t* d_any_all, uint8_t* d_any_use, uint8_t* d_any_use_nr, uint8_t* d_few_above,
                     const double* h_ridge, const double* h_contrast, double lfc_null, int alt, double* d_pvals,
                     double* d_stats, double* d_se, const dsq_mix* mix, int cooks_ld) {
    DSQ_CHECK_ARG(P >= 1 && P <= DSQ_MAX_P, "P out of range");
    DSQ_CHECK_ARG(mix == nullptr || (mix->d.P == P && mix->d.N == N), "mix: built for another design");
    DSQ_CHECK_ARG(cooks_ld == 0 || (mix != nullptr && cooks_ld >= mix->d.Ns && dsq::irls_takes_mix(&mix->d, full_rank)),
                  "cooks_ld: a slot-ordered Cook's layer needs a mixed design the kernel takes and a pitch >= its slots");
    DSQ_CHECK_ARG(cells == nullptr || cells->n_cells <= dsq::kMaxCells, "too many design cells for the cell path");
    DSQ_CHECK_ARG(d_flags == nullptr || (d_robust_disp && d_any_all && d_any_use && d_any_use_nr && d_few_above),
                  "the fused Cook's bookkeeping needs the robust dispersions and the four flag vectors");
    DSQ_CHECK_ARG(h_ridge == nullptr || (h_contrast && d_pvals && d_stats && d_se && alt >= 0 && alt <= 4),
                  "the fused Wald test needs contrast, outputs and a valid alternative");
    if (G <= 0) return DSQ_OK;
    dsq::IrlsExtras ex{};
    ex.cells = to_cells(cells);
    if (mix != nullptr) ex.mix = &mix->d;
    ex.cooks_ld = cooks_ld;
    if (d_flags != nullptr) {
        ex.robust_disp = d_robust_disp; ex.flags = d_flags; ex.cutoff = cutoff; ex.cooks = d_cooks;
        ex.any_all = d_any_all; ex.any_use = d_any_use; ex.any_use_nr = d_any_use_nr; ex.few_above = d_few_above;
    }
    if (h_ridge != nullptr) {
        double* d_ridge;
        double* h_stage;
        { const int rc = ridge_stage(ctx, P, &d_ridge, &h_stage); if (rc != DSQ_OK) return fail(ctx, rc, "ridge staging: out of memory"); }
        double* d_contrast = d_ridge + P * P;
        const bool in_place = ctx->lfc_part != nullptr &&
                              (ctx->lfc_phase == 2 || (ctx->lfc_phase == 1 && ctx->lfc_prepared_wald &&
                                                       ctx->lfc_prepared_N == N && ctx->lfc_prepared_P == P));
        if (!in_place) {
            std::memcpy(h_stage, h_ridge, (size_t)P * P * sizeof(double));
            std::memcpy(h_stage + P * P, h_contrast, (size_t)P * sizeof(double));
            DSQ_HIP(hipMemcpyAsync(d_ridge, h_stage, (size_t)(P * P + P) * sizeof(double), hipMemcpyHostToDevice,
                                   ctx->stream));
        }
        ex.ridge = d_ridge; ex.contrast = d_contrast; ex.lfc_null = lfc_null; ex.alt = alt;
        ex.pvals = d_pvals; ex.stats = d_stats; ex.se = d_se;
    }
    return run_irls(ctx, d_y, ldn, d_sf, d_Xt, d_pinvXt, ldx, N, G, P, full_rank, d_disp, min_mu, beta_tol, min_beta,
                    max_beta, maxiter, d_beta, d_mu, d_hat, d_converged, d_iters, &ex);
}

int dsq_dev_lfc_fit(dsq_ctx* ctx, const int32_t* d_y, int ldn, const double* d_sf, const double* d_Xt,
                    const double* d_pinvXt, int ldx, int N, int G, int P, int full_rank, const double* d_disp,
                    double min_mu, double beta_tol, double min_beta, double max_beta, int maxiter, double* d_beta,
                    double* d_mu, double* d_hat, uint8_t* d_converged, int32_t* d_iters, const dsq_cells* cells,
                    const double* d_robust_disp, const uint8_t* d_flags, double cutoff, double* d_cooks,
                    uint8_t* d_any_all, uint8_t* d_any_use, uint8_t* d_any_use_nr, uint8_t* d_few_above,
                    const double* h_ridge, const double* h_contrast, double lfc_null, int alt, double* d_pvals,
                    double* d_stats, double* d_se) {
    return dsq_dev_lfc_fit2(ctx, d_y, ldn, d_sf, d_Xt, d_pinvXt, ldx, N, G, P, full_rank, d_disp, min_mu, beta_tol,
                            min_beta, max_beta, maxiter, d_beta, d_mu, d_hat, d_converged, d_iters, cells, d_robust_disp,
                            d_flags, cutoff, d_cooks, d_any_all, d_any_use, d_any_use_nr, d_few_above, h_ridge, h_contrast,
                            lfc_null, alt, d_pvals, d_stats, d_se, nullptr, 0);
}

int dsq_dev_cooks(dsq_ctx* ctx, const int32_t* d_y, int ldn, const double* d_sf, const double* d_mu,
                  const double* d_hat, const int32_t* d_cell_offsets, const int32_t* d_cell_index,
                  int n_cells, int whole, int max_cell, const uint8_t* d_flags, int N, int G, int P,
                  double cutoff, double* d_cooks, double* d_robust_disp, uint8_t* d_any_all,
                  uint8_t* d_any_use, uint8_t* d_any_use_nr, uint8_t* d_few_above) {
    DSQ_CHECK_ARG((whole ? N : max_cell) <= 16384, "a design cell with more than 16384 samples is not supported");
    DSQ_HIP(dsq::launch_cooks(ctx->stream, d_y, ldn, d_sf, d_mu, d_hat, d_cell_offsets, d_cell_index,
                              n_cells, whole, max_cell, d_flags, N, G, P, cutoff, d_cooks, d_robust_disp,
                              d_any_all, d_any_use, d_any_use_nr, d_few_above));
    return DSQ_OK;
}

int dsq_dev_replace_outliers2(dsq_ctx* ctx, const int32_t* d_y, const double* d_cooks, int ldn,
                              const double* d_sf, const uint8_t* d_flags, const int32_t* d_gene_idx,
                              int n_sel, int N, double cutoff, int32_t* d_y_out, uint8_t* d_all_zero, int cooks_ld,
                              const dsq_mix* mix) {
    DSQ_CHECK_ARG(cooks_ld == 0 || (mix != nullptr && mix->d.N == N && cooks_ld >= mix->d.Ns),
                  "cooks_ld: a slot-ordered Cook's layer comes with the mixed design that wrote it");
    DSQ_HIP(dsq::launch_replace(ctx->stream, d_y, d_cooks, ldn, d_sf, d_flags, d_gene_idx, n_sel, N, cutoff,
                                d_y_out, d_all_zero, cooks_ld, cooks_ld != 0 ? mix->d.slot_of : nullptr));
    return DSQ_OK;
}

int dsq_dev_replace_outliers(dsq_ctx* ctx, const int32_t* d_y, const double* d_cooks, int ldn,
                             const double* d_sf, const uint8_t* d_flags, const int32_t* d_gene_idx,
                             int n_sel, int N, double cutoff, int32_t* d_y_out, uint8_t* d_all_zero) {
    return dsq_dev_replace_outliers2(ctx, d_y, d_cooks, ldn, d_sf, d_flags, d_gene_idx, n_sel, N, cutoff, d_y_out,
                                     d_all_zero, 0, nullptr);
}

int dsq_dev_wald(dsq_ctx* ctx, const double* d_mu, int ldn, const double* d_sf, const double* d_Xt, int ldx,
                 int N, int G, int P, const double* d_disp, const double* d_beta, const double* h_ridge,
                 const double* h_contrast, double lfc_null, int alt, double* d_pvals, double* d_stats,
                 double* d_se) {
    DSQ_CHECK_ARG(P >= 1 && P <= DSQ_MAX_P, "P out of range");
    DSQ_CHECK_ARG(alt >= 0 && alt <= 4, "unknown alternative hypothesis");
    double* d_ridge;
    double* h_unused;
    { const int rc = ridge_stage(ctx, P, &d_ridge, &h_unused); if (rc != DSQ_OK) return fail(ctx, rc, "ridge staging: out of memory"); }
// ... 289 lines not shown
```

pydeseq2_amd/csrc/dsq_k_alpha.hip:

```cpp
#include <atomic>
#include <type_traits>

#include "dsq_alpha.h"
#include "dsq_dispatch.h"
#include "dsq_launch.h"

#ifndef DSQ_ALPHA_WAVES_WIDE
#define DSQ_ALPHA_WAVES_WIDE 2
#endif
#ifndef DSQ_ALPHA_WAVES_NARROW
#define DSQ_ALPHA_WAVES_NARROW 3
#endif
constexpr int alpha_min_waves(int p) { return p <= 3 ? DSQ_ALPHA_WAVES_NARROW : (p <= 5 ? 2 : DSQ_ALPHA_WAVES_WIDE); }

namespace dsq {

#if defined(DSQ_PHASE_TIMING)
__device__ unsigned long long g_phase_total[16];
#endif

template <int P, bool STAGE, bool CELL = false>
__global__ __launch_bounds__(kBlock, CELL ? cell_min_waves(P) : alpha_min_waves(P)) void k_alpha(const int32_t* __restrict__ y,
                                                  const double* __restrict__ mu, int ldn,
                                                  const double* __restrict__ Xt, int ldx, int N, int G,
// ... 186 lines not shown
        GridBest o;
        o.f = __shfl_xor(best.f, m, 64);
        o.i = __shfl_xor(best.i, m, 64);
        o.nan = __shfl_xor((int)best.nan, m, 64) != 0;
        if (o.i != 0x7fffffff && (best.i == 0x7fffffff || grid_better(o, best))) best = o;
    }
    if (lane == 0) {
        const double c = linspace_at(lo, hi, kGridLen, best.i);
        if (stage == 0) {
            const double delta = linspace_at(lo, hi, kGridLen, 1) - linspace_at(lo, hi, kGridLen, 0);
            lohi[2 * k] = c - delta;
            lohi[2 * k + 1] = c + delta;
            done[k] = 0;
        } else {
            alpha[g] = exp(c);
        }
    }
}

template <int P>
__global__ __launch_bounds__(kBlock, alpha_min_waves(P)) void k_alpha_bfgs(const int32_t* __restrict__ y, const double* __restrict__ mu,
                                                       int ldn, const double* __restrict__ Xt, int ldx, int N, int G,
                                                       const double* __restrict__ alpha_hat, double min_disp,
                                                       double max_disp, double prior_var, int cr_reg, int prior_reg,
                                                       double* __restrict__ alpha, uint8_t* __restrict__ conv,
                                                       int32_t* __restrict__ nfev, int32_t* __restrict__ grid_count,
                                                       int32_t* __restrict__ grid_list) {
    log_tab_fill();
    __syncthreads();
    const int g = blockIdx.x * kWavesPerBlock + (threadIdx.x >> 6);
    if (g >= G) return;
    const int32_t* yg = y + (size_t)g * ldn;
    int maxc = 0;
    for (int n = threadIdx.x & 63; n < N; n += 64) maxc = yg[n] > maxc ? yg[n] : maxc;
    maxc = DeviceWave::maxi(maxc);
    const int memo_blocks = __builtin_amdgcn_readfirstlane(min(kMemoBlocks, (maxc >> 6) + 1));
    const AlphaOut o = fit_alpha_gene_bfgs<DeviceWave, P, false>(yg, mu + (size_t)g * ldn, Xt, ldx, N, alpha_hat[g],
                                                                 min_disp, max_disp, prior_var, cr_reg != 0,
                                                                 prior_reg != 0, memo_blocks);
    if ((threadIdx.x & 63) == 0) {
        alpha[g] = o.alpha;
        conv[g] = (uint8_t)o.converged;
        if (nfev != nullptr) nfev[g] = o.nfev;
        if (!o.converged) grid_list[atomicAdd(grid_count, 1)] = g;
    }
}

bool no_two_phase();

#define DSQ_MIX_DECL(Q_)                                                                                               \
    void alpha_mix_grid_q##Q_(int Ns, int P, int n_list, int* blocks, int* nw);                                        \
    hipError_t launch_alpha_mix_q##Q_(hipStream_t, const uint16_t*, const double*, const MixDesign&, const int32_t*, int, \
                                      const int32_t*, int32_t*, const double*, double, double, double, int, double*,   \
                                      uint8_t*, int32_t*, int32_t*, int32_t*, double*, int, int, int, void*, int32_t*,  \
                                      int32_t*);
DSQ_MIX_DECL(1)
DSQ_MIX_DECL(2)
DSQ_MIX_DECL(3)
#undef DSQ_MIX_DECL

static std::atomic<int> g_mix_launches{0};
int alpha_mix_launches() { return g_mix_launches.load(std::memory_order_relaxed); }

bool alpha_mix_enabled() {
    static const bool off = getenv("DSQ_NO_ALPHA_MIX") != nullptr;
    return !off;
}

bool alpha_mix_fits(const MixDesign& D) {
    int blocks = 0, nw = 0;
    if (D.Q == 1) alpha_mix_grid_q1(D.Ns, D.P, 1, &blocks, &nw);
    else if (D.Q == 2) alpha_mix_grid_q2(D.Ns, D.P, 1, &blocks, &nw);
    else if (D.Q == 3) alpha_mix_grid_q3(D.Ns, D.P, 1, &blocks, &nw);
    return blocks > 0;
}

hipError_t launch_alpha_mix(hipStream_t st, const uint16_t* ys, const double* mu_s, const MixDesign& D, const int32_t* list,
                            int n_list, const int32_t* n_dev, int32_t* queue, const double* alpha_hat, double min_disp,
                            double max_disp, double prior_var, int prior_reg, double* alpha, uint8_t* conv, int32_t* nfev,
                            int32_t* grid_count, int32_t* grid_list, double* nll_const, int const_mode, int eval_cap,
                            int resume, void* park_state, int32_t* park_count, int32_t* park_list) {
    g_mix_launches.fetch_add(1, std::memory_order_relaxed);
#define DSQ_MIX_CALL(Q_)                                                                                              \
    return launch_alpha_mix_q##Q_(st, ys, mu_s, D, list, n_list, n_dev, queue, alpha_hat, min_disp, max_disp, prior_var, \
                                  prior_reg, alpha, conv, nfev, grid_count, grid_list, nll_const, const_mode, eval_cap, \
                                  resume, park_state, park_count, park_list)
    switch (D.Q) {
        case 1: DSQ_MIX_CALL(1);
        case 2: DSQ_MIX_CALL(2);
        case 3: DSQ_MIX_CALL(3);
        default: return hipErrorInvalidValue;
    }
#undef DSQ_MIX_CALL
}

hipError_t launch_alpha_bfgs(hipStream_t st, const int32_t* y, const double* mu, int ldn, const double* Xt, int ldx,
                             int N, int G, int P_, const double* alpha_hat, double min_disp, double max_disp,
                             double prior_var, int cr_reg, int prior_reg, double* alpha, uint8_t* conv,
                             int32_t* nfev, int32_t* grid_count, int32_t* grid_list) {
    if (G <= 0) return hipSuccess;
    if (P_ > DSQ_REG_MAX_P || mu == nullptr) return hipErrorInvalidValue;
    DSQ_DISPATCH_P(P_, hipLaunchKernelGGL(k_alpha_bfgs<P>, dim3(genes_to_blocks(G)), dim3(kBlock), 0, st, y, mu, ldn,
                                          Xt, ldx, N, G, alpha_hat, min_disp, max_disp, prior_var, cr_reg, prior_reg,
                                          alpha, conv, nfev, grid_count, grid_list))
    return hipGetLastError();
}

hipError_t launch_alpha(hipStream_t st, const int32_t* y, const double* mu, int ldn, const double* Xt,
                        int ldx, int N, int G, int P_, const double* alpha_hat, double min_disp,
                        double max_disp, double prior_var, int cr_reg, int prior_reg, double* alpha,
                        uint8_t* conv, int32_t* nfev, int32_t* grid_count, int32_t* grid_list,
                        double* nll_const, int const_mode, const AlphaExtras* extras, int32_t* queue) {
    if (G <= 0) return hipSuccess;
    if (nll_const == nullptr) const_mode = DSQ_CONST_COMPUTE;
    AlphaExtras ex{};
    if (extras != nullptr) ex = *extras;
    ex.list = nullptr;
    bool parked = false;
    const int G_rows = ex.n_rows;
    ex.cell_mu_of = ex.cells.cell_of;
    ex.cell_mu_C = ex.cells.C;
    const bool have_lists = ex.rows != nullptr && queue != nullptr && ex.n_rows + ex.n_waves == G;
    const bool rows_reg = have_lists && ex.cell_mu == nullptr &&
                          alpha_rows_eligible(N, P_, ex.cells.C, ex.coef != nullptr, cr_reg);
    const bool rows_lds = have_lists && !rows_reg && cr_reg != 0 && (ex.coef != nullptr || ex.cell_mu != nullptr) &&
                          alpha_rowsc_tail(N, P_, ex.cells.C) > 0;
    const bool rows_mix = have_lists && ex.mix != nullptr && cr_reg != 0 && ex.mix_ys != nullptr && ex.mix_mu != nullptr &&
                          alpha_mix_enabled();
    if (rows_mix) {
        const bool park = ex.resume_state != nullptr && ex.resume_count != nullptr && ex.resume_list != nullptr &&
                          nll_const != nullptr && ex.eval_cap > 0 && !no_two_phase();
        hipError_t e = launch_alpha_mix(st, ex.mix_ys, ex.mix_mu, *ex.mix, ex.rows, ex.n_rows, nullptr, queue, alpha_hat,
                                        min_disp, max_disp, prior_var, prior_reg, alpha, conv, nfev, grid_count, grid_list,
                                        nll_const, const_mode, park ? ex.eval_cap : 0, 0, ex.resume_state, ex.resume_count,
                                        ex.resume_list);
        if (e != hipSuccess) return e;
        if (ex.mid_hook != nullptr) { ex.mid_hook(ex.mid_arg); ex.mid_hook = nullptr; }
        if (ex.conv_late != nullptr) conv = ex.conv_late;
        if (park) {
            e = launch_alpha_mix(st, ex.mix_ys, ex.mix_mu, *ex.mix, ex.resume_list, ex.n_rows, ex.resume_count, queue + 2,
                                 alpha_hat, min_disp, max_disp, prior_var, prior_reg, alpha, conv, nfev, grid_count,
                                 grid_list, nll_const, const_mode, 0, 1, ex.resume_state, ex.resume_count, ex.resume_list);
            if (e != hipSuccess) return e;
        }
        if (ex.n_waves <= 0) return hipSuccess;
        ex.list = ex.waves;
        G = ex.n_waves;
    }
    if (!rows_mix && (rows_reg || rows_lds)) {
        const bool park = ex.resume_state != nullptr && ex.resume_count != nullptr && ex.resume_list != nullptr &&
                          nll_const != nullptr && ex.eval_cap > 0 && !no_two_phase();
        hipError_t e;
        if (rows_reg)
            e = launch_alpha_rows(st, y, ldn, N, ex.rows, ex.n_rows, queue, ex.coef, ex.sf, ex.cells, P_, ex.min_mu,
                                  alpha_hat, min_disp, max_disp, prior_var, cr_reg, prior_reg, alpha, conv, nfev,
                                  grid_count, grid_list, nll_const, const_mode, park ? ex.eval_cap : 0, ex.resume_state,
                                  ex.resume_count, ex.resume_list);
        else
            e = launch_alpha_rows_c(st, y, ldn, N, ex.rows, ex.n_rows, queue, ex.coef, ex.cell_mu, ex.sf, ex.cells, P_,
                                    ex.min_mu, alpha_hat, min_disp, max_disp, prior_var, prior_reg, alpha, conv, nfev,
                                    grid_count, grid_list, nll_const, const_mode, park ? ex.eval_cap : 0,
                                    ex.resume_state, ex.resume_count, ex.resume_list);
        if (e != hipSuccess) return e;
        if (ex.mid_hook != nullptr) { ex.mid_hook(ex.mid_arg); ex.mid_hook = nullptr; }
        if (ex.conv_late != nullptr) conv = ex.conv_late;
        parked = park;
        if (parked && rows_reg && alpha_wg_eligible(N)) {
            const hipError_t e2 = launch_alpha_wg(st, y, ldn, N, ex.resume_list, ex.resume_count, ex.n_rows, ex.coef,
                                                  ex.sf, ex.cells, P_, ex.min_mu, alpha_hat, prior_var, prior_reg, alpha,
                                                  conv, nfev, grid_count, grid_list, nll_const, ex.resume_state);
            if (e2 != hipSuccess) return e2;
            parked = false;
        }
        if (ex.n_waves <= 0 && !parked) return hipSuccess;
        ex.list = ex.waves;
        G = ex.n_waves;
    }
    if (ex.cells.C <= kSmallCells) ex.cells = CellDesign{};
    if (P_ > DSQ_REG_MAX_P || (P_ >= wide_min_p() && (ex.cells.C == 0 || wide_with_cells()))) {
        if (mu == nullptr) return hipErrorInvalidValue;
        return launch_wide_alpha(st, y, mu, ldn, Xt, ldx, N, G, P_, alpha_hat, min_disp, max_disp, prior_var, cr_reg,
                                 prior_reg, alpha, conv, nfev, nll_const, const_mode,
                                 ex.cells.C > 0 ? &ex.cells : nullptr);
    }
    const dim3 block(kBlock);
    const int npad = (N + 63) & ~63;
    const size_t smem = (size_t)kWavesPerBlock * (npad + npad / 2) * sizeof(double);
    const bool stage = smem <= 80 * 1024;
    if (!stage && (ex.coef != nullptr || ex.cell_mu != nullptr)) return hipErrorInvalidValue;
    const bool cell = stage && ex.cells.C > kSmallCells && P_ >= 3 && cr_reg != 0;
#define DSQ_ALPHA_LAUNCH(KERNEL, SMEM)                                                                            \
    do {                                                                                                          \
        if ((SMEM) > 48 * 1024) {                                                                                 \
            (void)hipFuncSetAttribute((const void*)KERNEL, hipFuncAttributeMaxDynamicSharedMemorySize, (int)(SMEM)); \
            (void)hipGetLastError();                                                                              \
        }                                                                                                         \
        hipLaunchKernelGGL(KERNEL, grid, block, (SMEM), st, y, mu, ldn, Xt, ldx, N, G, alpha_hat, min_disp,      \
                           max_disp, prior_var, cr_reg, prior_reg, alpha, conv, nfev, grid_count, grid_list,     \
                           nll_const, const_mode, ex);                                                           \
    } while (0)
    ex.eval_cap = 0;
    for (int pass = 0; pass < (parked ? 2 : 1); ++pass) {
        if (pass == 1) {
            ex.resume = 1;
            ex.list = ex.resume_list;
            ex.n_dev = ex.resume_count;
            G = G_rows;
        }
        if (G <= 0) continue;
        const dim3 grid(genes_to_blocks(G));
        if (cell) {
            const size_t smem_c = smem + (size_t)ex.cells.C * (P_ * (P_ + 1) / 2 + P_) * sizeof(double);
            DSQ_DISPATCH_P(P_, {
                if constexpr (P >= 3) DSQ_ALPHA_LAUNCH((k_alpha<P, true, true>), smem_c);
            })
        } else if (stage) {
            DSQ_DISPATCH_P(P_, DSQ_ALPHA_LAUNCH((k_alpha<P, true, false>), smem))
        } else {
            DSQ_DISPATCH_P(P_, DSQ_ALPHA_LAUNCH((k_alpha<P, false, false>), (size_t)0))
        }
        if (ex.mid_hook != nullptr) {
            ex.mid_hook(ex.mid_arg); ex.mid_hook = nullptr;
            if (ex.conv_late != nullptr) conv = ex.conv_late;
        }
    }
#undef DSQ_ALPHA_LAUNCH
    return hipGetLastError();
}

size_t alpha_resume_bytes(int G) { return (size_t)G * sizeof(Lbfgsb1d); }
bool no_two_phase() {
    static const bool off = getenv("DSQ_NO_TWO_PHASE") != nullptr;
    return off;
}

bool alpha_is_wide(int P_, int n_cells) {
    if (n_cells <= kSmallCells) n_cells = 0;
    return P_ > DSQ_REG_MAX_P || (P_ >= wide_min_p() && (n_cells == 0 || wide_with_cells()));
}

bool alpha_needs_mu(int N, int P_, int n_cells) {
    if (alpha_is_wide(P_, n_cells)) return true;
    const int npad = (N + 63) & ~63;
    return (size_t)kWavesPerBlock * (npad + npad / 2) * sizeof(double) > 80 * 1024;
}

hipError_t launch_alpha_grid(hipStream_t st, const int32_t* y, const double* mu, int ldn, const double* Xt,
                             int ldx, int N, int P_, double min_disp, double max_disp, double* alpha,
                             const int32_t* grid_list, int n_grid, double* work, const int32_t* n_dev,
                             bool mu_compact) {
    if (n_grid <= 0) return hipSuccess;
    if (P_ > DSQ_REG_MAX_P) {
        if (n_dev != nullptr || mu_compact) return hipErrorInvalidValue;
        return launch_wide_alpha_grid(st, y, mu, ldn, Xt, ldx, N, P_, min_disp, max_disp, alpha, grid_list, n_grid);
    }
    double* lohi = work;
    double* ll = work + 2 * (size_t)n_grid;
    int32_t* done = (int32_t*)(ll + (size_t)n_grid * kGridLen);
    const dim3 ge(genes_to_blocks(n_grid * kGridLen)), block(kBlock);
    hipError_t e = hipMemsetAsync(done, 0, (size_t)n_grid * sizeof(int32_t), st);
    if (e != hipSuccess) return e;
    for (int stage = 0; stage < 2; ++stage) {
        DSQ_DISPATCH_P(P_, hipLaunchKernelGGL(k_alpha_grid_eval<P>, ge, block, 0, st, y, mu, ldn, Xt, ldx, N,
                                              grid_list, n_grid, mu_compact ? 1 : 0, stage, log(min_disp),
                                              log(max_disp), lohi, ll, done, alpha, n_dev))
    }
    return hipGetLastError();
}

}

#if defined(DSQ_PHASE_TIMING)
extern "C" int dsq_debug_phase_read(unsigned long long* out, int reset) {
    if (hipMemcpyFromSymbol(out, HIP_SYMBOL(dsq::g_phase_total), 16 * sizeof(unsigned long long)) != hipSuccess) return -1;
    if (reset) {
        unsigned long long z[16] = {0};
        if (hipMemcpyToSymbol(HIP_SYMBOL(dsq::g_phase_total), z, sizeof(z)) != hipSuccess) return -1;
    }
    return 0;
}
#endif
```

pydeseq2_amd/csrc/dsq_k_alpha_rows.hip:

```cpp
#include <cstdio>
#include <type_traits>

#include "dsq_alpha_rows.h"
#include "dsq_dispatch.h"

namespace dsq {

#if defined(DSQ_ROWS_PHASES)
__device__ unsigned long long g_rows_phase[8];
#define ROWS_PH(k)                                                      \
    do {                                                                \
        __builtin_amdgcn_sched_barrier(0);                              \
        const long long t_ = clock64();                                 \
        ph_acc[ph_cur] += t_ - ph_last; ph_last = t_; ph_cur = (k);     \
        __builtin_amdgcn_sched_barrier(0);                              \
    } while (0)
#else
#define ROWS_PH(k) ((void)0)
#endif

template <int P>
__global__ __launch_bounds__(kRowBlock, 2) void k_alpha_rows(
    const int32_t* __restrict__ y, int ldn, int N, const int32_t* __restrict__ list, int n_list,
    int32_t* __restrict__ queue, const double* __restrict__ coef, const double* __restrict__ sf,
    const int32_t* __restrict__ cell_of, const double* __restrict__ Xc, const double* __restrict__ XXc, double min_mu,
    const double* __restrict__ alpha_hat, double min_disp, double max_disp, double prior_var, int cr_reg, int prior_reg,
    double* __restrict__ alpha_out, uint8_t* __restrict__ conv, int32_t* __restrict__ nfev,
    int32_t* __restrict__ grid_count, int32_t* __restrict__ grid_list, double* __restrict__ nll_const, int const_mode,
    int eval_cap, Lbfgsb1d* __restrict__ park_state, int32_t* __restrict__ park_count, int32_t* __restrict__ park_list) {
    constexpr int C = P;
    constexpr int T = Tri<P>::N;
    extern __shared__ __attribute__((aligned(16))) double dyn[];
    const int npad = (N + 63) & ~63;
    double* const sf_s = dyn;
    uint8_t* const cell_s = (uint8_t*)(sf_s + npad);
    char* const slots0 = (char*)(cell_s + npad);
    const size_t slot_bytes = row_slot_bytes(npad);
    unsigned int* const hist0 = (unsigned int*)(slots0 + slot_bytes * kRowSlots * kRowWaves);

    const int lane = threadIdx.x & 63, w = threadIdx.x >> 6;
    const int row = lane >> 4, rl = lane & 15;
    log_tab_fill();
    for (int n = threadIdx.x; n < npad; n += kRowBlock) {
        sf_s[n] = n < N ? sf[n] : 0.0;
        cell_s[n] = (uint8_t)(n < N ? cell_of[n] : 0);
    }
    __syncthreads();

    auto slot_of = [&](int r) { return (RowGene*)(slots0 + slot_bytes * (size_t)(w * kRowSlots + r)); };
    RowGene* const S = slot_of(row);
    uint16_t* const cnt = (uint16_t*)((char*)S + sizeof(RowGene));
    uint16_t* const tail = cnt + npad;
    unsigned int* const hist = hist0 + (size_t)w * kRowTail;
    if (rl == 0) { S->g = -1; S->n_tail = 0; S->n_big = 0; }
    DeviceWave::sync();

    const double lo = log(min_disp), hi = log(max_disp);
    double xx[C][T];
#pragma unroll
    for (int c = 0; c < C; ++c)
#pragma unroll
        for (int k = 0; k < T; ++k) xx[c][k] = XXc[c * T + k];

#if defined(DSQ_ROWS_PHASES)
    long long ph_acc[8] = {0, 0, 0, 0, 0, 0, 0, 0}, ph_last = clock64();
    int ph_cur = 0;
#endif
    bool queue_open = true;
    for (;;) {
        ROWS_PH(1);
        int mine = S->g;
        if (queue_open) {
            int want = -1;
            if (mine < 0 && rl == 0) {
                const int k = atomicAdd(queue, 1);
                want = k < n_list ? (list != nullptr ? list[k] : k) : -2;
            }
            unsigned long long todo = __ballot(want >= 0);
            if (__any(want == -2)) queue_open = false;
            while (todo) {
                const int src = __ffsll((long long)todo) - 1;
                todo &= todo - 1;
                const int g = __shfl(want, src, 64);
                const int r = src >> 4;
                RowGene* const Sr = slot_of(r);
                uint16_t* const cr = (uint16_t*)((char*)Sr + sizeof(RowGene));
                uint16_t* const tr = cr + npad;
                for (int i = lane; i < kRowTail; i += 64) hist[i] = 0u;
                double q[C];
                {
                    double b[P];
#pragma unroll
                    for (int j = 0; j < P; ++j) b[j] = coef[(size_t)g * P + j];
#pragma unroll
                    for (int c = 0; c < C; ++c) {
                        double yh = 0.0;
#pragma unroll
                        for (int j = 0; j < P; ++j) yh += Xc[c * P + j] * b[j];
                        q[c] = yh;
                    }
                }
                DeviceWave::sync();
                const int32_t* yg = y + (size_t)g * ldn;
                const bool want_cst = const_mode != DSQ_CONST_LOAD;
                KSum cs;
                int maxc = 0, nbig = 0;
                constexpr int CH = 8;
                for (int base = 0; base < npad; base += 64 * CH) {
                    int v8[CH];
#pragma unroll
                    for (int k = 0; k < CH; ++k) {
                        const int n = base + 64 * k + lane;
                        v8[k] = n < N ? yg[n] : 0;
                    }
#pragma unroll
                    for (int k = 0; k < CH; ++k) {
                        const int n = base + 64 * k + lane;
                        if (base + 64 * k >= npad) break;
                        const bool in = n < N;
                        const int v = v8[k];
                        cr[n] = (uint16_t)v;
                        maxc = v > maxc ? v : maxc;
                        const bool isbig = v >= kRowTail;
                        if (in && v > 0 && !isbig) atomicAdd(&hist[v], 1u);
                        const unsigned long long bm = __ballot(isbig);
                        if (isbig) {
                            if (want_cst) {
                                const double z = (double)v + 1.0, zM = (double)kRowTail + 1.0;
                                cs.add(((z - 0.5) * flog(z) - z + stirling_tail(frcp(z))) -
                                       ((zM - 0.5) * flog(zM) - zM + stirling_tail(frcp(zM))));
                            }
                        }
                        nbig += __popcll(bm);
                        if (want_cst && in) {
                            const int cl = cell_s[n];
                            double qq = q[0];
#pragma unroll
                            for (int c = 1; c < C; ++c) qq = (cl == c) ? q[c] : qq;
                            const double mu = dmax(sf_s[n] * qq, min_mu);
                            cs.add(-((double)v * flog_t(mu)));
                        }
                    }
                }
                maxc = DeviceWave::maxi(maxc);
                DeviceWave::sync();
                {
                    constexpr int BPL = kRowTail / 64;
                    int h[BPL], tot = 0;
#pragma unroll
                    for (int k = 0; k < BPL; ++k) { h[k] = (int)hist[lane * BPL + k]; tot += h[k]; }
                    const int below = DeviceWave::excl_scan_i(tot);
                    const int all = DeviceWave::sumi(tot);
                    int above = all - below - tot + nbig;
#pragma unroll
                    for (int k = BPL - 1; k >= 0; --k) {
                        tr[lane * BPL + k] = (uint16_t)above;
                        if (want_cst && above > 0) cs.add((double)above * flog_t((double)(lane * BPL + k + 1)));
                        above += h[k];
                    }
                }
                double cst = 0.0;
                if (want_cst) cst = DeviceWave::sum_comp(cs);
                else cst = nll_const[g];
                if (const_mode == DSQ_CONST_STORE && lane == 0) nll_const[g] = cst;
                if (lane == 0) {
                    Sr->g = g;
                    Sr->cst = cst;
                    const int mt = maxc < kRowTail ? maxc : kRowTail;
                    Sr->n_tail = (mt + 2 * kRowLanes - 1) & ~(2 * kRowLanes - 1);
                    Sr->n_big = nbig;
#pragma unroll
                    for (int c = 0; c < C; ++c) Sr->q[c] = q[c];
                    const double lah = log(alpha_hat[g]);
                    Sr->la_hat = lah;
                    Sr->m.start(lah, lo, hi);
                }
                DeviceWave::sync();
            }
            mine = S->g;
        }
        if (!__any(mine >= 0)) break;
        const bool active = mine >= 0;
        ROWS_PH(2);

        const double la = active ? S->m.x : 0.0;
        const double alpha = exp(la);
        const double a = frcp(alpha);
        const double lal = flog_t(alpha);
        KSum accf;
        double accg = 0.0;
        {
            const int ntl = active ? S->n_tail : 0;
            for (int i = rl; i < ntl; i += kRowLanes) {
                const double t = a + (double)i;
                const double ti = (double)tail[i];
                accf.add(-(ti * flog_t(t)));
                accg -= ti * frcp(t);
            }
            const int nb = active ? S->n_big : 0;
            if (__any(nb > 0)) {
                double lgM, psiM;
                stirling_big((double)kRowTail + a, lgM, psiM);
                if (nb > 0) {
                    for (int n = rl; n < npad; n += kRowLanes) {
                        const int yi = cnt[n];
                        if (yi >= kRowTail) {
                            double lgz, psiz;
                            stirling_big((double)yi + a, lgz, psiz);
                            accf.add(lgM - lgz);
                            accg += psiM - psiz;
                        }
                    }
                }
            }
        }
        ROWS_PH(3);
        double q[C], wc[C], dwc[C];
#pragma unroll
        for (int c = 0; c < C; ++c) { q[c] = S->q[c]; wc[c] = 0.0; dwc[c] = 0.0; }
        constexpr int U = 4;
        KSum af[U];
        double ag[U];
#pragma unroll
        for (int u = 0; u < U; ++u) ag[u] = 0.0;
        double wt = 0.0, dwt = 0.0;
        for (int n0 = rl; n0 < npad; n0 += kRowLanes * U) {
            int yi[U], cl[U];
            double sfn[U], m[U], r1[U], L1[U];
#pragma unroll
            for (int u = 0; u < U; ++u) {
                yi[u] = cnt[n0 + kRowLanes * u];
                sfn[u] = sf_s[n0 + kRowLanes * u];
                cl[u] = cell_s[n0 + kRowLanes * u];
            }
#pragma unroll
            for (int u = 0; u < U; ++u) {
                double qq = q[0];
#pragma unroll
                for (int c = 1; c < C; ++c) qq = (cl[u] == c) ? q[c] : qq;
                const double mm = dmax(sfn[u] * qq, min_mu);
                m[u] = (sfn[u] == 0.0) ? 0.0 : mm;
            }
#pragma unroll
            for (int u = 0; u < U; ++u) r1[u] = frcp(1.0 + m[u] * alpha);
            {
                int kk[U];
                double cc[U], rc[U], tt[U], mant[U];
#pragma unroll
                for (int u = 0; u < U; ++u) {
                    const double ma = m[u] * alpha;
                    const double wv = 1.0 + ma;
                    cc[u] = (ma - (wv - 1.0)) * r1[u];
                    detail::log_split(wv, kk[u], rc[u], tt[u], mant[u]);
                }
#pragma unroll
                for (int u = 0; u < U; ++u) {
                    const double r = fma(mant[u], rc[u], -1.0);
                    const double pl = detail::log1p_tail(r);
                    const double dk = (double)kk[u];
                    L1[u] = fma(dk, detail::kLn2Hi, tt[u] + (r + (pl + fma(dk, detail::kLn2Lo, cc[u]))));
                }
            }
#pragma unroll
            for (int u = 0; u < U; ++u) {
                const double yv = (double)yi[u];
                af[u].add(yv * (L1[u] - lal) + a * L1[u]);
                ag[u] += L1[u] + (yv - m[u]) * alpha * r1[u];
                const double wv = m[u] * r1[u];
                const double dwv = -(wv * wv);
                wt += wv;
                dwt += dwv;
#pragma unroll
                for (int c = 1; c < C; ++c) {
                    const double on = (cl[u] == c) ? 1.0 : 0.0;
                    wc[c] = fma(wv, on, wc[c]);
                    dwc[c] = fma(dwv, on, dwc[c]);
                }
            }
        }
        {
            double rest = 0.0, drest = 0.0;
#pragma unroll
            for (int c = 1; c < C; ++c) { rest += wc[c]; drest += dwc[c]; }
            wc[0] = wt - rest;
            dwc[0] = dwt - drest;
        }
#pragma unroll
        for (int u = 0; u < U; ++u) { accf.merge(af[u].s, af[u].c); accg += ag[u]; }
        const bool cr = true;
        ROWS_PH(4);
        const double sumf = RowWave::sum_comp(accf);
        accg = RowWave::sum(accg);
        double f = sumf + S->cst;
        double gr = alpha * (-(a * a * accg));
        if (cr) {
            double M[T], dM[T];
#pragma unroll
            for (int k = 0; k < T; ++k) { M[k] = 0.0; dM[k] = 0.0; }
#pragma unroll
            for (int c = 0; c < C; ++c) {
                const double ws = RowWave::sum(wc[c]), dws = RowWave::sum(dwc[c]);
#pragma unroll
                for (int k = 0; k < T; ++k) { M[k] += ws * xx[c][k]; dM[k] += dws * xx[c][k]; }
            }
            chol<P>(M);
            f += 0.5 * chol_logdet<P>(M);
            double inv[T];
            chol_inverse<P>(M, inv);
            gr += 0.5 * sym_frob<P>(inv, dM) * alpha;
        }
        if (prior_reg != 0) {
            const double dl = la - S->la_hat;
            f += dl * dl / (2.0 * prior_var);
            gr += dl / prior_var;
        }
        ROWS_PH(5);
        if (active) {
            S->m.feed(f, gr);
            if (S->m.done) {
                if (rl == 0) {
                    const int g = mine;
                    alpha_out[g] = exp(S->m.x);
                    conv[g] = (uint8_t)(S->m.success ? 1 : 0);
                    if (nfev != nullptr) nfev[g] = S->m.nfev;
                    if (!S->m.success) grid_list[atomicAdd(grid_count, 1)] = g;
                    S->g = -1;
                }
            } else if (eval_cap > 0 && S->m.nfev >= eval_cap) {
                constexpr int kDw = (int)(sizeof(Lbfgsb1d) / 4);
                uint32_t* dst = (uint32_t*)(park_state + mine);
                const uint32_t* src = (const uint32_t*)&S->m;
                for (int i = rl; i < kDw; i += kRowLanes) dst[i] = src[i];
                if (rl == 0) {
                    park_list[atomicAdd(park_count, 1)] = mine;
                    S->g = -1;
                }
            }
        }
        DeviceWave::sync();
    }
#if defined(DSQ_ROWS_PHASES)
    ROWS_PH(0);
    if (lane == 0) {
        unsigned long long life = 0;
        for (int k = 0; k < 6; ++k) { atomicAdd(&g_rows_phase[k], (unsigned long long)ph_acc[k]); life += ph_acc[k]; }
        atomicMax(&g_rows_phase[6], life);
        atomicAdd(&g_rows_phase[7], 1ull);
    }
#endif
}

constexpr int kWgSpt = 4;

template <int P, int TPB>
__global__ __launch_bounds__(TPB) void k_alpha_wg(
    const int32_t* __restrict__ y, int ldn, int N, const int32_t* __restrict__ list, const int32_t* __restrict__ n_dev,
    const double* __restrict__ coef, const double* __restrict__ sf, const int32_t* __restrict__ cell_of,
    const double* __restrict__ Xc, const double* __restrict__ XXc, double min_mu, const double* __restrict__ alpha_hat,
    double prior_var, int prior_reg, double* __restrict__ alpha_out, uint8_t* __restrict__ conv,
    int32_t* __restrict__ nfev, int32_t* __restrict__ grid_count, int32_t* __restrict__ grid_list,
    const double* __restrict__ nll_const, const Lbfgsb1d* __restrict__ park_state) {
    constexpr int C = P;
    constexpr int T = Tri<P>::N;
    constexpr int NV = 3 + 2 * C;
    const int n_parked = *n_dev;
    if ((int)blockIdx.x >= n_parked) return;
    __shared__ unsigned int hist[kRowTail];
    __shared__ int wave_tot[kRowTail / 64];
    __shared__ double part[16][NV];
    __shared__ Lbfgsb1d mach[16];
    __shared__ int s_nbig;
    const int tid = threadIdx.x, lane = tid & 63, w = tid >> 6, nthreads = blockDim.x, nwaves = nthreads >> 6;
    log_tab_fill();
    double xx[C][T];
#pragma unroll
    for (int c = 0; c < C; ++c)
#pragma unroll
        for (int k = 0; k < T; ++k) xx[c][k] = XXc[c * T + k];
    for (int item = blockIdx.x; item < n_parked; item += gridDim.x) {
    const int g = list[item];
    __syncthreads();
    for (int i = tid; i < kRowTail; i += nthreads) hist[i] = 0u;
    if (tid == 0) s_nbig = 0;
    {
        constexpr int kDw = (int)(sizeof(Lbfgsb1d) / 4);
        const uint32_t* src = (const uint32_t*)(park_state + g);
        uint32_t* dst = (uint32_t*)&mach[w];
        for (int i = lane; i < kDw; i += 64) dst[i] = src[i];
    }
    double q[C];
    {
        double b[P];
#pragma unroll
        for (int j = 0; j < P; ++j) b[j] = coef[(size_t)g * P + j];
#pragma unroll
        for (int c = 0; c < C; ++c) {
            double yh = 0.0;
#pragma unroll
            for (int j = 0; j < P; ++j) yh += Xc[c * P + j] * b[j];
            q[c] = yh;
        }
    }
    __syncthreads();
    const int32_t* yg = y + (size_t)g * ldn;
    int yi[kWgSpt], cl[kWgSpt];
    double mu[kWgSpt];
    int nbig = 0;
#pragma unroll
    for (int k = 0; k < kWgSpt; ++k) {
        const int n = tid + k * nthreads;
        const bool in = n < N;
        yi[k] = in ? yg[n] : 0;
        cl[k] = in ? cell_of[n] : 0;
        double qq = q[0];
#pragma unroll
        for (int c = 1; c < C; ++c) qq = (cl[k] == c) ? q[c] : qq;
        mu[k] = in ? dmax(sf[n] * qq, min_mu) : 0.0;
        if (yi[k] >= kRowTail) nbig += 1;
        else if (yi[k] > 0) atomicAdd(&hist[yi[k]], 1u);
    }
    nbig = DeviceWave::sumi(nbig);
    if (lane == 0 && nbig > 0) atomicAdd(&s_nbig, nbig);
    __syncthreads();
    constexpr int TPT = (kRowTail + TPB - 1) / TPB;
    double my_tail[TPT];
    {
        int suf[TPT];
#pragma unroll
        for (int k = 0; k < TPT; ++k) {
            const int i = tid + k * TPB;
            suf[k] = 0;
            if (i < kRowTail) {
                const int h = (int)hist[i];
                int v = h;
#pragma unroll
                for (int d = 1; d < 64; d <<= 1) {
                    const int o = __shfl_down(v, d, 64);
                    if (lane + d < 64) v += o;
// ... 9 lines not shown
            my_tail[k] = 0.0;
            if (i < kRowTail) {
                int above = s_nbig + suf[k];
                for (int cc = (i >> 6) + 1; cc < kRowTail / 64; ++cc) above += wave_tot[cc];
                my_tail[k] = (double)above;
            }
        }
    }
    const double cst = nll_const[g];
    const double la_hat = log(alpha_hat[g]);
    Lbfgsb1d m = mach[w];
    DeviceWave::sync();
    while (!m.done) {
        const double la = m.x;
        const double alpha = exp(la);
        const double a = frcp(alpha);
        const double lal = flog_t(alpha);
        KSum accf;
        double accg = 0.0, wc[C], dwc[C];
#pragma unroll
        for (int c = 0; c < C; ++c) { wc[c] = 0.0; dwc[c] = 0.0; }
#pragma unroll
        for (int k = 0; k < TPT; ++k) {
            if (my_tail[k] > 0.0) {
                const double t = a + (double)(tid + k * TPB);
                accf.add(-(my_tail[k] * flog_t(t)));
                accg -= my_tail[k] * frcp(t);
            }
        }
        double lgM = 0.0, psiM = 0.0;
        if (s_nbig > 0) stirling_big((double)kRowTail + a, lgM, psiM);
#pragma unroll
        for (int k = 0; k < kWgSpt; ++k) {
            if (tid + k * nthreads < N) {
                const double mm = mu[k], yv = (double)yi[k];
                const double ma = mm * alpha;
                const double r1 = frcp(1.0 + ma);
                const double L1 = flog1p_t(ma, r1);
                accf.add(yv * (L1 - lal) + a * L1);
                accg += L1 + (yv - mm) * alpha * r1;
                const double wv = mm * r1, dwv = -(wv * wv);
#pragma unroll
                for (int c = 0; c < C; ++c) {
                    wc[c] += (cl[k] == c) ? wv : 0.0;
                    dwc[c] += (cl[k] == c) ? dwv : 0.0;
                }
                if (yi[k] >= kRowTail) {
                    double lgz, psiz;
                    stirling_big(yv + a, lgz, psiz);
                    accf.add(lgM - lgz);
                    accg += psiM - psiz;
                }
            }
        }
        {
            KSum k1 = accf;
            const double f1 = DeviceWave::sum_comp(k1);
            const double g1 = DeviceWave::sum(accg);
            double v[NV];
            v[0] = f1; v[1] = 0.0; v[2] = g1;
#pragma unroll
            for (int c = 0; c < C; ++c) { v[3 + c] = DeviceWave::sum(wc[c]); v[3 + C + c] = DeviceWave::sum(dwc[c]); }
            if (lane == 0)
#pragma unroll
                for (int i = 0; i < NV; ++i) part[w][i] = v[i];
        }
        __syncthreads();
        KSum fs;
        double gs = 0.0, ws[C], dws[C];
#pragma unroll
        for (int c = 0; c < C; ++c) { ws[c] = 0.0; dws[c] = 0.0; }
        for (int ww = 0; ww < nwaves; ++ww) {
            fs.add(part[ww][0]);
            gs += part[ww][2];
#pragma unroll
            for (int c = 0; c < C; ++c) { ws[c] += part[ww][3 + c]; dws[c] += part[ww][3 + C + c]; }
        }
        __syncthreads();
        double f = fs.value() + cst;
        double gr = alpha * (-(a * a * gs));
        {
            double M[T], dM[T];
#pragma unroll
            for (int k = 0; k < T; ++k) { M[k] = 0.0; dM[k] = 0.0; }
#pragma unroll
            for (int c = 0; c < C; ++c)
#pragma unroll
                for (int k = 0; k < T; ++k) { M[k] += ws[c] * xx[c][k]; dM[k] += dws[c] * xx[c][k]; }
            chol<P>(M);
            f += 0.5 * chol_logdet<P>(M);
            double inv[T];
            chol_inverse<P>(M, inv);
            gr += 0.5 * sym_frob<P>(inv, dM) * alpha;
        }
        if (prior_reg != 0) {
            const double dl = la - la_hat;
            f += dl * dl / (2.0 * prior_var);
            gr += dl / prior_var;
        }
        m.feed(f, gr);
        DeviceWave::sync();
    }
    if (tid == 0) {
        alpha_out[g] = exp(m.x);
        conv[g] = (uint8_t)(m.success ? 1 : 0);
        if (nfev != nullptr) nfev[g] = m.nfev;
        if (!m.success) grid_list[atomicAdd(grid_count, 1)] = g;
    }
    }
}

static bool wg_narrow_enabled() {
    static const bool v = getenv("DSQ_WG_512") == nullptr;
    return v;
}
bool alpha_wg_eligible(int N) { return N <= 1024 * kWgSpt && getenv("DSQ_NO_ALPHA_WG") == nullptr; }

hipError_t launch_alpha_wg(hipStream_t st, const int32_t* y, int ldn, int N, const int32_t* list, const int32_t* n_dev,
                           int n_cap, const double* coef, const double* sf, const CellDesign& cells, int P_,
                           double min_mu, const double* alpha_hat, double prior_var, int prior_reg, double* alpha,
                           uint8_t* conv, int32_t* nfev, int32_t* grid_count, int32_t* grid_list,
                           const double* nll_const, const void* park_state) {
    if (n_cap <= 0) return hipSuccess;
    const bool wide = N > 512 * kWgSpt, narrow = N <= 256 * kWgSpt && wg_narrow_enabled();
#define DSQ_WG_LAUNCH(PP)                                                                                            \
    do {                                                                                                             \
        if (narrow)                                                                                                  \
            hipLaunchKernelGGL((k_alpha_wg<PP, 256>), dim3(n_cap < 768 ? n_cap : 768), dim3(256), 0, st, y, ldn, N, list, \
                               n_dev, coef, sf, cells.cell_of, cells.Xc, cells.XX, min_mu, alpha_hat, prior_var,     \
                               prior_reg, alpha, conv, nfev, grid_count, grid_list, nll_const,                       \
                               (const Lbfgsb1d*)park_state);                                                         \
        else if (wide)                                                                                               \
            hipLaunchKernelGGL((k_alpha_wg<PP, 1024>), dim3(n_cap < 768 ? n_cap : 768), dim3(1024), 0, st, y, ldn, N, list, \
                               n_dev, coef, sf, cells.cell_of, cells.Xc, cells.XX, min_mu, alpha_hat, prior_var,     \
                               prior_reg, alpha, conv, nfev, grid_count, grid_list, nll_const,                       \
                               (const Lbfgsb1d*)park_state);                                                         \
        else                                                                                                         \
            hipLaunchKernelGGL((k_alpha_wg<PP, 512>), dim3(n_cap < 768 ? n_cap : 768), dim3(512), 0, st, y, ldn, N, list, \
                               n_dev, coef, sf, cells.cell_of, cells.Xc, cells.XX, min_mu, alpha_hat, prior_var,     \
                               prior_reg, alpha, conv, nfev, grid_count, grid_list, nll_const,                       \
                               (const Lbfgsb1d*)park_state);                                                         \
    } while (0)
    switch (P_) {
        case 1: DSQ_WG_LAUNCH(1); break;
        case 2: DSQ_WG_LAUNCH(2); break;
        case 3: DSQ_WG_LAUNCH(3); break;
        case 4: DSQ_WG_LAUNCH(4); break;
        default: return hipErrorInvalidValue;
    }
#undef DSQ_WG_LAUNCH
    return hipGetLastError();
}

size_t alpha_rows_smem(int N) {
    const int npad = (N + 63) & ~63;
    return (size_t)npad * 8 + (size_t)npad + row_slot_bytes(npad) * kRowSlots * kRowWaves +
           (size_t)kRowWaves * kRowTail * 4;
}

bool alpha_rows_eligible(int N, int P_, int n_cells, bool has_coef, int cr_reg) {
    static const bool off = getenv("DSQ_NO_ALPHA_ROWS") != nullptr;
    return !off && has_coef && cr_reg != 0 && P_ >= 1 && P_ <= 4 && n_cells == P_ && N <= 65535 &&
           alpha_rows_smem(N) <= 78 * 1024;
}

hipError_t launch_alpha_rows(hipStream_t st, const int32_t* y, int ldn, int N, const int32_t* list, int n_list,
                             int32_t* queue, const double* coef, const double* sf, const CellDesign& cells, int P_,
                             double min_mu, const double* alpha_hat, double min_disp, double max_disp, double prior_var,
                             int cr_reg, int prior_reg, double* alpha, uint8_t* conv, int32_t* nfev, int32_t* grid_count,
                             int32_t* grid_list, double* nll_const, int const_mode, int eval_cap, void* park_state,
                             int32_t* park_count, int32_t* park_list) {
    if (n_list <= 0) return hipSuccess;
    const int n_cu = current_device_cus();
    if (n_cu <= 0) return hipGetLastError();
    const size_t smem = alpha_rows_smem(N);
    const int per_block = kRowSlots * kRowWaves;
    int blocks = (n_list + per_block - 1) / per_block;
    if (blocks > 2 * n_cu) blocks = 2 * n_cu;
    if (nll_const == nullptr) const_mode = DSQ_CONST_COMPUTE;
#define DSQ_ROWS_LAUNCH(PP)                                                                                          \
    do {                                                                                                             \
        if (smem > 48 * 1024) {                                                                                      \
            (void)hipFuncSetAttribute((const void*)k_alpha_rows<PP>, hipFuncAttributeMaxDynamicSharedMemorySize,    \
                                      (int)smem);                                                                    \
            (void)hipGetLastError();                                                                                 \
        }                                                                                                            \
        if (getenv("DSQ_DEBUG_ROWS")) {                                                                              \
            int nb = -1;                                                                                             \
            (void)hipOccupancyMaxActiveBlocksPerMultiprocessor(&nb, (const void*)k_alpha_rows<PP>, kRowBlock, smem); \
            fprintf(stderr, "[k_alpha_rows<%d>] smem %zu blocks %d n_list %d occupancy %d blocks/CU\n", PP, smem,    \
                    blocks, n_list, nb);                                                                             \
        }                                                                                                            \
        hipLaunchKernelGGL(k_alpha_rows<PP>, dim3(blocks), dim3(kRowBlock), smem, st, y, ldn, N, list, n_list, queue, \
                           coef, sf, cells.cell_of, cells.Xc, cells.XX, min_mu, alpha_hat, min_disp, max_disp,       \
                           prior_var, cr_reg, prior_reg, alpha, conv, nfev, grid_count, grid_list, nll_const,        \
                           const_mode, eval_cap, (Lbfgsb1d*)park_state, park_count, park_list);                     \
    } while (0)
    switch (P_) {
        case 1: DSQ_ROWS_LAUNCH(1); break;
        case 2: DSQ_ROWS_LAUNCH(2); break;
        case 3: DSQ_ROWS_LAUNCH(3); break;
        case 4: DSQ_ROWS_LAUNCH(4); break;
        default: return hipErrorInvalidValue;
    }
#undef DSQ_ROWS_LAUNCH
    return hipGetLastError();
}

__global__ __launch_bounds__(kBlock) void k_count_big(const int32_t* __restrict__ y, int ldn, int N, int G,
                                                      int32_t* __restrict__ out) {
    const int g = blockIdx.x * kWavesPerBlock + (threadIdx.x >> 6);
    if (g >= G) return;
    const int32_t* yg = y + (size_t)g * ldn;
    int nb = 0, mx = 0;
    for (int n = threadIdx.x & 63; n < N; n += 64) {
        const int v = yg[n];
        nb += v >= kRowTail ? 1 : 0;
        mx = v > mx ? v : mx;
    }
    nb = DeviceWave::sumi(nb);
    mx = DeviceWave::maxi(mx);
    if ((threadIdx.x & 63) == 0) out[g] = mx >= 0xFFFE ? -1 : nb;
}

hipError_t launch_count_big(hipStream_t st, const int32_t* y, int ldn, int N, int G, int32_t* out) {
    if (G <= 0) return hipSuccess;
    hipLaunchKernelGGL(k_count_big, dim3(genes_to_blocks(G)), dim3(kBlock), 0, st, y, ldn, N, G, out);
    return hipGetLastError();
}

}

#if defined(DSQ_ROWS_PHASES)
extern "C" int dsq_debug_rows_phase_read(unsigned long long* out, int reset) {
    if (hipMemcpyFromSymbol(out, HIP_SYMBOL(dsq::g_rows_phase), 8 * sizeof(unsigned long long)) != hipSuccess) return -1;
    if (reset) {
        unsigned long long z[8] = {0};
        if (hipMemcpyToSymbol(HIP_SYMBOL(dsq::g_rows_phase), z, sizeof(z)) != hipSuccess) return -1;
    }
    return 0;
}
#endif
```

pydeseq2_amd/csrc/dsq_launch.h:

```cpp
#pragma once
#include <hip/hip_runtime.h>

#include <cstdint>

#include "../../include/deseq_hip.h"
#include "dsq_linalg.h"
#include "dsq_mix.h"

namespace dsq {

constexpr int kWavesPerBlock = 4;
constexpr int kBlock = 64 * kWavesPerBlock;

inline int genes_to_blocks(int G) { return (G + kWavesPerBlock - 1) / kWavesPerBlock; }

inline int current_device_cus() {
    static int cache[64] = {0};
    int dev = 0;
    if (hipGetDevice(&dev) != hipSuccess) return 0;
    if (dev >= 0 && dev < 64 && cache[dev] > 0) return cache[dev];
    hipDeviceProp_t prop;
    if (hipGetDeviceProperties(&prop, dev) != hipSuccess) return 0;
    if (dev >= 0 && dev < 64) cache[dev] = prop.multiProcessorCount;
    return prop.multiProcessorCount;
}

#ifndef DSQ_CELL_WAVES_WIDE
#define DSQ_CELL_WAVES_WIDE 2
#endif
constexpr int cell_min_waves(int p) { return p <= 6 ? 3 : DSQ_CELL_WAVES_WIDE; }

int wide_min_p();
bool wide_with_cells();
struct IrlsExtras;
hipError_t launch_wide_mom(hipStream_t st, const int32_t* y, int ldn, const double* sf, const double* Xt,
                           const double* pinvXt, int ldx, int N, int G, int P, double min_disp, double max_disp,
                           double min_mu, double* normed_mean, double* rough, double* moments, double* mom,
                           double* mu, double* coef, const double* d_s_mean_inv);
hipError_t launch_wide_rough_normed(hipStream_t st, const double* normed, int ldn, const double* Xt,
                                    const double* pinvXt, int ldx, int N, int G, int P, double* out);
hipError_t launch_wide_alpha(hipStream_t st, const int32_t* y, const double* mu, int ldn, const double* Xt, int ldx,
                             int N, int G, int P, const double* alpha_hat, double min_disp, double max_disp,
                             double prior_var, int cr_reg, int prior_reg, double* alpha, uint8_t* conv,
                             int32_t* nfev, double* nll_const, int const_mode, const CellDesign* cells);
hipError_t launch_wide_alpha_grid(hipStream_t st, const int32_t* y, const double* mu, int ldn, const double* Xt,
                                  int ldx, int N, int P, double min_disp, double max_disp, double* alpha,
                                  const int32_t* list, int n_list);
hipError_t launch_wide_irls(hipStream_t st, const int32_t* y, int ldn, const double* sf, const double* lsf,
                            const double* Xt, const double* pinvXt, int ldx, int N, int G, int P, int full_rank,
                            const double* disp, double min_mu, double beta_tol, double min_beta, double max_beta,
                            int maxiter, double* beta, double* mu, double* hat, uint8_t* conv, int32_t* iters,
                            int32_t* fb_count, int32_t* fb_list, const IrlsExtras* extras);
hipError_t launch_wide_irls_rescue(hipStream_t st, const int32_t* y, int ldn, const double* sf, const double* lsf,
                                   const double* Xt, const double* pinvXt, int ldx, int N, int P, int full_rank,
                                   const double* disp, double min_mu, double beta_tol, double min_beta,
                                   double max_beta, int maxiter, double* beta, double* mu, double* hat, uint8_t* conv,
                                   int32_t* iters, const int32_t* fb_list, int n_fb, const IrlsExtras* extras);
hipError_t launch_wide_irls_layers(hipStream_t st, const int32_t* y, int ldn, const double* sf, const double* Xt,
                                   int ldx, int N, int G, int P, const double* disp, const double* beta, double min_mu,
                                   double* mu, double* hat);
hipError_t launch_wide_wald(hipStream_t st, const double* mu, int ldn, const double* sf, const double* Xt, int ldx,
                            int N, int G, int P, const double* disp, const double* beta, const double* d_ridge,
                            const double* d_contrast, double lfc_null, int alt, double* pvals, double* stats,
                            double* se);
void wider_release(hipStream_t st);
hipError_t launch_wider_mom(hipStream_t st, const int32_t* y, int ldn, const double* sf, const double* Xt,
                            const double* pinvXt, int ldx, int N, int G, int P, double min_disp, double max_disp,
                            double min_mu, double* normed_mean, double* rough, double* moments, double* mom,
                            double* mu, double* coef, const double* d_s_mean_inv);
hipError_t launch_wider_rough_normed(hipStream_t st, const double* normed, int ldn, const double* Xt,
                                     const double* pinvXt, int ldx, int N, int G, int P, double* out);
hipError_t launch_wider_alpha(hipStream_t st, const int32_t* y, const double* mu, int ldn, const double* Xt, int ldx,
                              int N, int G, int P, const double* alpha_hat, double min_disp, double max_disp,
                              double prior_var, int cr_reg, int prior_reg, double* alpha, uint8_t* conv,
                              int32_t* nfev, double* nll_const, int const_mode);
hipError_t launch_wider_alpha_grid(hipStream_t st, const int32_t* y, const double* mu, int ldn, const double* Xt,
                                   int ldx, int N, int P, double min_disp, double max_disp, double* alpha,
                                   const int32_t* list, int n_list);
hipError_t launch_wider_irls(hipStream_t st, const int32_t* y, int ldn, const double* sf, const double* lsf,
                             const double* Xt, const double* pinvXt, int ldx, int N, int G, int P, int full_rank,
                             const double* disp, double min_mu, double beta_tol, double min_beta, double max_beta,
                             int maxiter, double* beta, double* mu, double* hat, uint8_t* conv, int32_t* iters,
                             int32_t* fb_count, int32_t* fb_list, const IrlsExtras* extras);
hipError_t launch_wider_irls_rescue(hipStream_t st, const int32_t* y, int ldn, const double* sf, const double* lsf,
                                    const double* Xt, const double* pinvXt, int ldx, int N, int P, int full_rank,
                                    const double* disp, double min_mu, double beta_tol, double min_beta,
                                    double max_beta, int maxiter, double* beta, double* mu, double* hat, uint8_t* conv,
                                    int32_t* iters, const int32_t* fb_list, int n_fb, const IrlsExtras* extras);
hipError_t launch_wider_irls_layers(hipStream_t st, const int32_t* y, int ldn, const double* sf, const double* Xt,
                                    int ldx, int N, int G, int P, const double* disp, const double* beta, double min_mu,
                                    double* mu, double* hat);
hipError_t launch_wider_wald(hipStream_t st, const double* mu, int ldn, const double* sf, const double* Xt, int ldx,
                             int N, int G, int P, const double* disp, const double* beta, const double* d_ridge,
                             const double* d_contrast, double lfc_null, int alt, double* pvals, double* stats,
                             double* se);

struct AlphaExtras {
    CellDesign cells;
    const double* coef;
    const double* sf;
    double min_mu;
    const int32_t* rows;
    const int32_t* waves;
    int n_rows, n_waves;
    const double* cell_mu;
    const int32_t* cell_mu_of;
    int cell_mu_C;
    const int32_t* list;
    int eval_cap;
    int resume;
    void* resume_state;
    int32_t* resume_count;
    int32_t* resume_list;
    const int32_t* n_dev;
    void (*mid_hook)(void*);
    void* mid_arg;
    uint8_t* conv_late;
    const MixDesign* mix;
    const double* mix_beta;
    const uint16_t* mix_ys;
    const double* mix_mu;
};
constexpr int kAlphaEvalCap = 8;
size_t alpha_resume_bytes(int G);
constexpr int kRowTail = 512;
bool alpha_rows_eligible(int N, int P, int n_cells, bool has_coef, int cr_reg);
hipError_t launch_alpha_rows(hipStream_t st, const int32_t* y, int ldn, int N, const int32_t* list, int n_list,
                             int32_t* queue, const double* coef, const double* sf, const CellDesign& cells, int P,
                             double min_mu, const double* alpha_hat, double min_disp, double max_disp, double prior_var,
                             int cr_reg, int prior_reg, double* alpha, uint8_t* conv, int32_t* nfev, int32_t* grid_count,
                             int32_t* grid_list, double* nll_const, int const_mode, int eval_cap, void* park_state,
                             int32_t* park_count, int32_t* park_list);
hipError_t launch_count_big(hipStream_t st, const int32_t* y, int ldn, int N, int G, int32_t* out);
int alpha_rowsc_tail(int N, int P, int n_cells);
hipError_t launch_alpha_rows_c(hipStream_t st, const int32_t* y, int ldn, int N, const int32_t* list, int n_list,
                               int32_t* queue, const double* coef, const double* cell_mu, const double* sf,
                               const CellDesign& cells, int P, double min_mu, const double* alpha_hat, double min_disp,
                               double max_disp, double prior_var, int prior_reg, double* alpha, uint8_t* conv,
                               int32_t* nfev, int32_t* grid_count, int32_t* grid_list, double* nll_const,
                               int const_mode, int eval_cap, void* park_state, int32_t* park_count,
                               int32_t* park_list);
hipError_t launch_cell_mu(hipStream_t st, const double* beta, const double* Xc, int C, int G, int P, double* cell_mu);
hipError_t launch_mu_from_cells(hipStream_t st, const double* cell_mu, int C, const double* sf, const int32_t* cell_of,
                                int N, const int32_t* list, int n_list, double* dst, int ldn, int32_t* idx_out,
                                const int32_t* n_dev = nullptr);
bool alpha_mix_enabled();
int alpha_mix_launches();
bool alpha_mix_fits(const MixDesign& D);
hipError_t launch_alpha_mix(hipStream_t st, const uint16_t* ys, const double* mu_s, const MixDesign& D, const int32_t* list,
                            int n_list, const int32_t* n_dev, int32_t* queue, const double* alpha_hat, double min_disp,
                            double max_disp, double prior_var, int prior_reg, double* alpha, uint8_t* conv, int32_t* nfev,
                            int32_t* grid_count, int32_t* grid_list, double* nll_const, int const_mode, int eval_cap,
                            int resume, void* park_state, int32_t* park_count, int32_t* park_list);
hipError_t launch_mu_from_beta(hipStream_t st, const double* beta, const double* sf, const double* Xt, int ldx, int N,
                               int P, const int32_t* list, int n_list, double* dst, int ldn, int32_t* idx_out,
                               const int32_t* n_dev = nullptr);
bool alpha_wg_eligible(int N);
hipError_t launch_alpha_wg(hipStream_t st, const int32_t* y, int ldn, int N, const int32_t* list, const int32_t* n_dev,
                           int n_cap, const double* coef, const double* sf, const CellDesign& cells, int P,
                           double min_mu, const double* alpha_hat, double prior_var, int prior_reg, double* alpha,
                           uint8_t* conv, int32_t* nfev, int32_t* grid_count, int32_t* grid_list,
                           const double* nll_const, const void* park_state);
hipError_t launch_alpha_bfgs(hipStream_t st, const int32_t* y, const double* mu, int ldn, const double* Xt, int ldx,
                             int N, int G, int P, const double* alpha_hat, double min_disp, double max_disp,
                             double prior_var, int cr_reg, int prior_reg, double* alpha, uint8_t* conv,
                             int32_t* nfev, int32_t* grid_count, int32_t* grid_list);
hipError_t launch_alpha(hipStream_t st, const int32_t* y, const double* mu, int ldn, const double* Xt,
                        int ldx, int N, int G, int P, const double* alpha_hat, double min_disp,
                        double max_disp, double prior_var, int cr_reg, int prior_reg, double* alpha,
                        uint8_t* conv, int32_t* nfev, int32_t* grid_count, int32_t* grid_list,
                        double* nll_const, int const_mode, const AlphaExtras* extras = nullptr, int32_t* queue = nullptr);
hipError_t launch_alpha_grid(hipStream_t st, const int32_t* y, const double* mu, int ldn, const double* Xt,
                             int ldx, int N, int P, double min_disp, double max_disp, double* alpha,
                             const int32_t* grid_list, int n_grid, double* work, const int32_t* n_dev = nullptr,
                             bool mu_compact = false);
constexpr int kAlphaGridWorkDoubles = 103;

struct IrlsExtras {
    CellDesign cells;
    const double* robust_disp;
    const uint8_t* flags;
    double cutoff;
    double* cooks;
    int cooks_ld;
    double* cooks_tmp;
    uint8_t *any_all, *any_use, *any_use_nr, *few_above;
    const double* ridge;
    const double* contrast;
    double lfc_null;
    int alt;
    double *pvals, *stats, *se;
    int optimizer;
    const int32_t* order;
    const MixDesign* mix;
    void* mix_work;
    size_t mix_work_bytes;
    int32_t* mix_queue;
    const uint16_t* mix_ys;
    const uint8_t* mix_big;
    const uint8_t* part;
    int part_want;
    int part_shared_ready;
};
bool irls_takes_parts(int N, int P, int n_cells, const MixDesign* mix, int full_rank);
bool irls_takes_mix(const MixDesign* mix, int full_rank);
size_t irls_mix_work_bytes(const MixDesign& D, int G, int n_layers);
hipError_t launch_replace(hipStream_t st, const int32_t* y, const double* cooks, int ldn,
                          const double* sf, const uint8_t* flags, const int32_t* gene_idx, int n_sel,
                          int N, double cutoff, int32_t* y_out, uint8_t* all_zero, int cooks_ld,
                          const int32_t* slot_of);
bool irls_takes_rows(int N, int P, int n_cells);
hipError_t launch_irls_order(hipStream_t st, const double* disp, const int32_t* hint_iters, int G, int32_t* order,
                             int32_t* work);
int irls_order_work_ints();
hipError_t launch_irls(hipStream_t st, const int32_t* y, int ldn, const double* sf, const double* lsf,
                       const double* Xt,
                       const double* pinvXt, int ldx, int N, int G, int P, int full_rank,
                       const double* disp, double min_mu, double beta_tol, double min_beta,
                       double max_beta, int maxiter, double* beta, double* mu, double* hat,
                       uint8_t* conv, int32_t* iters, int32_t* fb_count, int32_t* fb_list,
                       const IrlsExtras* extras = nullptr);
hipError_t launch_irls_rescue(hipStream_t st, const int32_t* y, int ldn, const double* sf,
                              const double* lsf, const double* Xt, const double* pinvXt, int ldx, int N, int P,
                              int full_rank, const double* disp, double min_mu, double beta_tol,
                              double min_beta, double max_beta, int maxiter, double* beta, double* mu,
                              double* hat, uint8_t* conv, int32_t* iters, const int32_t* fb_list,
                              int n_fb, const IrlsExtras* extras = nullptr, const int32_t* n_dev = nullptr);

bool irls_is_wide(int P, int n_cells);
bool alpha_is_wide(int P, int n_cells);
bool alpha_needs_mu(int N, int P, int n_cells);

hipError_t launch_widen_u16(hipStream_t st, const uint16_t* src, int32_t* dst, size_t n);
hipError_t launch_transpose_counts(hipStream_t st, const void* src, int count_type, int layout, int N,
                                   int G, int32_t* dst, int ldn, int* bad_flag);
hipError_t launch_transpose_f64(hipStream_t st, const double* src, int layout, int N, int G,
                                double* dst, int ldn);
hipError_t launch_logmeans(hipStream_t st, const int32_t* y, int ldn, int N, int G, double* logmeans,
                           uint8_t* nonzero);
hipError_t launch_size_factors(hipStream_t st, const void* counts_sm, int count_type, int N, int G,
                               const double* logmeans, const uint8_t* gene_mask, double* work,
                               double* sf, int zeros_low = 0);
hipError_t launch_mom(hipStream_t st, const int32_t* y, int ldn, const double* sf, const double* Xt,
                      const double* pinvXt, int ldx, int N, int G, int P, double min_disp,
                      double max_disp, double* normed_mean, double* rough, double* moments,
                      double* mom, double* d_scalar, const double* sf_moments = nullptr);
hipError_t launch_mom_lin_mu(hipStream_t st, const int32_t* y, int ldn, const double* sf, const double* Xt,
                             const double* pinvXt, int ldx, int N, int G, int P, double min_disp, double max_disp,
                             double min_mu, double* normed_mean, double* mom, double* mu, double* d_scalar,
                             double* coef = nullptr);
hipError_t launch_mu_from_coef(hipStream_t st, const double* coef, const double* sf, const double* Xt, int ldx, int N,
                               int P, double min_mu, const int32_t* list, int n_list, double* dst, int ldn,
                               int32_t* idx_out, const int32_t* n_dev = nullptr);
hipError_t launch_irls_layers(hipStream_t st, const int32_t* y, int ldn, const double* sf, const double* Xt, int ldx,
                              int N, int G, int P, const double* disp, const double* beta, double min_mu, double* mu,
                              double* hat);
hipError_t launch_nll_const(hipStream_t st, const int32_t* y, int ldn, int N, int G, const double* disp, double* cst);
hipError_t launch_nll_scaled(hipStream_t st, const int32_t* y, const double* mu, int ldn, int N, int G,
                             const double* disp, const double* scale, const double* cst, double* nll);
hipError_t launch_lin_mu(hipStream_t st, const int32_t* y, int ldn, const double* sf, const double* Xt,
                         const double* pinvXt, int ldx, int N, int G, int P, double min_mu,
                         double* mu);
hipError_t launch_wald(hipStream_t st, const double* mu, int ldn, const double* sf, const double* Xt,
                       int ldx, int N, int G, int P, const double* disp, const double* beta,
                       const double* d_ridge, const double* d_contrast, double lfc_null, int alt,
                       double* pvals, double* stats, double* se);
hipError_t launch_lrt(hipStream_t st, const int32_t* y, int ldn, const double* sf, const double* Xf, int ldf, int Pf,
                      const double* Xr, int ldr, int Pr, int N, int G, const double* disp, const double* beta_f,
                      const double* beta_r, double* stat, double* pval);
hipError_t launch_chisq_sf(hipStream_t st, const double* x, int n, int df, double* out);
hipError_t launch_cooks(hipStream_t st, const int32_t* y, int ldn, const double* sf, const double* mu,
                        const double* hat, const int32_t* cell_offsets, const int32_t* cell_index,
                        int n_cells, int whole, int max_cell, const uint8_t* flags, int N, int G,
                        int P, double cutoff, double* cooks, double* robust_disp, uint8_t* any_all,
                        uint8_t* any_use, uint8_t* any_use_nr, uint8_t* few_above);
hipError_t launch_robust_disp(hipStream_t st, const int32_t* y, int ldn, const double* sf,
                              const int32_t* cell_offsets, const int32_t* cell_index, int n_cells, int whole,
                              int max_cell, int N, int G, double* robust_disp, int min_cell = 0, int32_t* redo = nullptr);
hipError_t launch_gather_rows_f64(hipStream_t st, const double* src, int ld, const int32_t* idx,
                                  int n_idx, int ncols, double* dst);
hipError_t launch_shrink(hipStream_t st, const int32_t* y, int ldn, const double* offset, const double* Xt, int ldx,
                         int N, int G, int P, const double* size, double sigma0, double sigma, int shrink_index,
                         double* beta, double* invh, uint8_t* conv, double* ih_entry = nullptr, int optimizer = 0);
size_t summary_sort_temp_bytes(int n);
hipError_t launch_padj_prepare(hipStream_t st, const double* base_mean, const double* pvalue, int n, double alpha,
// ... 66 lines not shown
```

pydeseq2_amd/pipeline.py:

```python
from __future__ import annotations

import os
import time
import warnings
from dataclasses import dataclass, field

import numpy as np
from scipy.stats import f as f_dist

from . import trend as _trend
from ._design import DesignPack, pad16
from ._lib import ALT, HOOK_FN, I32, I64, SAMPLE_MAJOR, Context, DeviceArray, DsqCells, _PinnedPool, _PinnedSlab

import ctypes as C
import functools

_vp, c_double = C.c_void_p, C.c_double


@dataclass
class DeseqResult:
    size_factors: np.ndarray = None
    normed_means: np.ndarray = None
    non_zero: np.ndarray = None
    mom_dispersions: np.ndarray = None
    genewise_dispersions: np.ndarray = None
    genewise_converged: np.ndarray = None
    trend_coeffs: np.ndarray = None
    disp_function_type: str = "parametric"
    mean_disp: float = None
    fitted_dispersions: np.ndarray = None
    squared_logres: float = None
    prior_disp_var: float = None
    MAP_dispersions: np.ndarray = None
    MAP_converged: np.ndarray = None
    outlier_genes: np.ndarray = None
    dispersions: np.ndarray = None
    LFC: np.ndarray = None
    LFC_converged: np.ndarray = None
    replaced: np.ndarray = None
    refitted: np.ndarray = None
    new_all_zeroes: np.ndarray = None
    cooks_outlier: np.ndarray = None
    pvalue: np.ndarray = None
    stat: np.ndarray = None
    lfcSE: np.ndarray = None
    timings: dict = field(default_factory=dict)
    kernel_ms: dict = field(default_factory=dict)


def _scatter(G, idx, v, fill=np.nan):
    out = np.full(G, fill)
    out[idx] = v
    return out


@functools.lru_cache(maxsize=64)
def _trigamma(x):
    from scipy.special import polygamma

    return float(polygamma(1, x))


def check_reduced_design(X, reduced_design):
    X = np.asarray(X, dtype=np.float64)
    Xr = np.asarray(reduced_design, dtype=np.float64)
    N, P = X.shape
    if Xr.ndim != 2:
        raise ValueError("The reduced design must be a samples x columns matrix.")
    if Xr.shape[0] != N:
        raise ValueError(f"The reduced design has {Xr.shape[0]} rows; the data set has {N} samples.")
    if not 1 <= Xr.shape[1] <= P - 1:
        raise ValueError(f"The reduced design must have between 1 and {P - 1} columns (fewer than the full design's "
                         f"{P}); it has {Xr.shape[1]}.")
    if np.isnan(Xr).any():
        raise ValueError("NaNs are not allowed in the reduced design.")
    if np.linalg.matrix_rank(Xr) != Xr.shape[1]:
        raise ValueError("The reduced design is rank deficient (its columns are linearly dependent).")
    if np.linalg.matrix_rank(np.hstack([Xr, X])) != np.linalg.matrix_rank(X):
        raise ValueError("The reduced design is not nested in the full design: its columns must lie in the span of the "
                         "full design's columns.")
    return np.ascontiguousarray(Xr)


class _Respeculate(Exception):
    """The pass was enqueued on the previous pass's non-zero mask and the matrix has another one: run it again, in order."""


class _Step:
    """State of one pass of the path: device handles and host scalars the stages hand to each other."""


class _View:

    __slots__ = ("ptr",)

    def __init__(self, ptr):
        self.ptr = ptr


class DeseqPipeline:

    def __init__(self, counts, design_matrix, *, ctx: Context | None = None, device: int = 0, min_mu=0.5,
                 min_disp=1e-8, max_disp=10.0, refit_cooks=True, min_replicates=7, beta_tol=1e-8,
                 fit_type="parametric", keep_cooks=True, size_factors_fit_type="ratio", control_genes=None,
                 irls_maxiter=250):
        self.ctx = ctx if ctx is not None else Context(device)
        counts = np.asarray(counts)
        if counts.ndim != 2:
            raise ValueError("counts must be samples x genes")
        if counts.dtype.kind == "f":
            if np.isnan(counts).any():
                raise ValueError("NaNs are not allowed in the count matrix.")
            if (counts % 1 != 0).any():
                raise ValueError("The count matrix should only contain integers.")
            counts = counts.astype(np.int64)
        elif counts.dtype.kind not in "iu":
            raise ValueError("The count matrix should only contain numbers.")
        if counts.dtype not in (np.int32, np.int64):
            counts = counts.astype(np.int64)
        self.N, self.G = counts.shape
        self.design = DesignPack(design_matrix, min_replicates)
        if self.design.N != self.N:
            raise ValueError("design matrix and counts disagree on the number of samples")
        self.P = self.design.P
        self.min_mu, self.min_disp = float(min_mu), float(min_disp)
        self.max_disp = float(max(max_disp, self.N))
        self.refit_cooks, self.min_replicates = bool(refit_cooks), int(min_replicates)
        self.beta_tol, self.fit_type = float(beta_tol), fit_type
        self.irls_maxiter = int(irls_maxiter)
        self.keep_cooks = keep_cooks
        if size_factors_fit_type not in ("ratio", "poscounts", "iterative"):
            raise ValueError("size_factors_fit_type: 'ratio' (median of ratios), 'poscounts' or 'iterative'")
        self.size_factors_fit_type = size_factors_fit_type
        self._control_mask = None
        if control_genes is not None:
            m = np.zeros(self.G if hasattr(self, "G") else counts.shape[1], dtype=np.uint8)
            m[np.asarray(control_genes)] = 1
            self._control_mask = m
        self.ldn = pad16(self.N)
        ctx_ = self.ctx
        counts = np.ascontiguousarray(counts)
        self._count_type = I32
        self.d_raw = DeviceArray(ctx_, (self.N, self.G), np.int32)
        bad = C.c_int(0)
        ctx_.call("dsq_upload_counts_i32", _vp(counts.ctypes.data), I32 if counts.dtype == np.int32 else I64,
                  C.c_size_t(counts.size), _vp(self.d_raw.ptr), C.byref(bad))
        if bad.value:
            raise ValueError("The count matrix should only contain non-negative integers below 2^31.")
        self.d_y = DeviceArray(ctx_, (self.G, self.N), np.int32, ld=self.ldn)
        ctx_.call("dsq_dev_counts_to_gene_major", _vp(self.d_raw.ptr), I32, SAMPLE_MAJOR, self.N,
                  self.G, _vp(self.d_y.ptr), self.ldn, C.byref(bad))
        D = self.design
        self.d_Xt = DeviceArray.from_host(ctx_, D.Xt)
        self.d_pinv = DeviceArray.from_host(ctx_, D.pinvXt)
        self.d_flags = DeviceArray.from_host(ctx_, D.flags)
        self.d_cell_off = DeviceArray.from_host(ctx_, D.cell_offsets)
        self.d_cell_idx = DeviceArray.from_host(ctx_, D.cell_index)
        self._cells = None
        if D.cell_path and not os.environ.get("DSQ_NO_CELL_PATH"):
            self._d_cell_of = DeviceArray.from_host(ctx_, D.cell_of)
            self._d_Xc = DeviceArray.from_host(ctx_, D.Xc)
            self._d_XXc = DeviceArray.from_host(ctx_, D.XXc)
            self._cells = DsqCells(self._d_cell_of.ptr, self._d_Xc.ptr, self._d_XXc.ptr, int(D.n_design_cells))
        self._row_flags, self._row_lists = None, None
        self._row_mode = 0 if (self._cells is None or os.environ.get("DSQ_NO_ALPHA_ROWS")) else \
            int(ctx_.lib.dsq_alpha_rows_eligible(self.N, self.P, int(D.n_design_cells)))
        if self._row_mode == 1 and not D.linear_mu:
            self._row_mode = 0
        self._mix, self._mix_slots, self._slot_of, self._mix_ys_cache = None, 0, None, None
        if self._row_mode == 0 and not D.linear_mu and not os.environ.get("DSQ_NO_ALPHA_MIX"):
            mp = _vp()
            ctx_.call("dsq_mix_create", _vp(D.X.ctypes.data), self.N, self.P, C.byref(mp))
            if mp.value:
                self._mix, self._row_mode = mp.value, 3
                ns = C.c_int()
                if ctx_.lib.dsq_mix_info(mp, C.byref(ns), None, None) != 0:
                    raise RuntimeError("dsq_mix_info failed")
                self._mix_slots = int(ns.value)
                self._slot_of = np.empty(self.N, dtype=np.int32)
                if ctx_.lib.dsq_mix_slots(mp, _vp(self._slot_of.ctypes.data)) != 0:
                    raise RuntimeError("dsq_mix_slots failed")
        if self._row_mode:
            d_fl = DeviceArray(ctx_, (self.G,), np.int32)
            ctx_.call("dsq_dev_alpha_row_split", _vp(self.d_y.ptr), self.ldn, self.N, self.G, _vp(d_fl.ptr))
            self._row_flags = d_fl.to_host()
            d_fl.free()
        self.keep_layers = False
        self.overlap = not os.environ.get("DSQ_NO_OVERLAP")
        self._robust_early = bool(os.environ.get("DSQ_ROBUST_EARLY"))
        self._robust_late = bool(os.environ.get("DSQ_ROBUST_LATE"))
        mw = os.environ.get("DSQ_MAP_WAIT")
        self._map_waits_side = (self._row_mode == 1) if mw is None else (mw != "0")
        self._robust_split = float(os.environ.get("DSQ_ROBUST_SPLIT", "0.78"))
        lo = os.environ.get("DSQ_LFC_OVERLAP")
        max_work = float(os.environ.get("DSQ_LFC_OVERLAP_MAX_WORK", "1.5e8"))
        auto = self._row_mode == 3 and float(self.G) * self.N <= max_work
        self._lfc_overlap = auto if lo is None else (lo != "0")
        self._lfc_min_genes = int(os.environ.get("DSQ_LFC_OVERLAP_MIN_GENES", "2048"))
        self._lfc_forked = False
        self.lfc_forks = 0
        self._work = None
        self.layers = {}
        self.time_kernels = False
        self.collect_nfev = False
        self.kernel_log = {}
        self._pool_free, self._pool_used = [], []
        self._inflight = []
        self._side_pending = False
        self._pinned = _PinnedPool(ctx_)
        self._replace_buf, self._replace_keep = None, None
        d_lm0, d_nz0 = DeviceArray(ctx_, (self.G,), np.float64), DeviceArray(ctx_, (self.G,), np.uint8)
        ctx_.call("dsq_dev_logmeans", _vp(self.d_y.ptr), self.ldn, self.N, self.G, _vp(d_lm0.ptr), _vp(d_nz0.ptr))
        self._nz_pred = d_nz0.to_host().astype(bool)
        d_lm0.free(); d_nz0.free()
        self._row_lists_for(self._nz_pred)
        self._cooks_cutoff = float(f_dist.ppf(0.99, self.P, self.N - self.P)) if self.N > self.P else float("nan")
        ctx_.sync()

    def _take(self, nbytes):
        nbytes = max(int(nbytes), 8)
        best = None
        for i, (cap, ptr) in enumerate(self._pool_free):
            if cap >= nbytes and (best is None or cap < self._pool_free[best][0]) and cap <= 2 * nbytes + 4096:
                best = i
        if best is not None:
            cap, ptr = self._pool_free.pop(best)
        else:
            cap, ptr = nbytes, self.ctx.malloc(nbytes)
        self._pool_used.append((cap, ptr))
        return ptr

    def _pool_reset(self):
        if getattr(self, "_side_pending", False) or getattr(self, "_lfc_forked", False):
            self.ctx.call("dsq_side_abort")
            self._side_pending = False
            self._lfc_forked = False
        self._pool_free.extend(self._pool_used)
        self._pool_used = []
        self._serial = getattr(self, "_serial", 0) + 1
        if getattr(self, "_inflight", None):
            self.ctx.sync()
        self._inflight = []
        self.layers = {}

    def _pooled(self, shape, dtype, ld=None):
        arr = DeviceArray.__new__(DeviceArray)
        arr.ctx = self.ctx
        arr.shape = tuple(shape)
        arr.dtype = np.dtype(dtype)
        arr.ld = ld if ld is not None else (arr.shape[-1] if len(arr.shape) > 1 else None)
        n = arr.shape[0] * (arr.ld if len(arr.shape) > 1 else 1)
        arr.nbytes = int(n) * arr.dtype.itemsize
        arr.ptr = self._take(arr.nbytes)
        arr.free = lambda: None
        return arr

    def _dvec(self, n, dtype=np.float64):
        return self._pooled((max(int(n), 1),), dtype)

    def _dmat(self, rows, dtype=np.float64):
        return self._pooled((max(int(rows), 1), self.N), dtype, ld=self.ldn)

    def _up(self, arr, dtype=np.float64):
        arr = np.ascontiguousarray(arr, dtype=dtype)
        d = self._pooled(arr.shape if arr.ndim else (1,), arr.dtype)
        if arr.size:
            if arr.nbytes <= 65536:
                hs = self._host_slab(arr.nbytes)
                hs.view(0, arr.size, arr.dtype)[:] = arr.reshape(-1)
                self.ctx.call("dsq_h2d_async", _vp(d.ptr), _vp(hs.ptr), C.c_size_t(arr.nbytes))
                self._inflight.append(hs)
            else:
                self.ctx.h2d(d.ptr, arr)
        return d

    def _down_nonzero(self):
        return self._nz_cache

    def _all_genes_host(self, d_vec, n):
        return self._down(d_vec, n)

    def _down(self, darr, n, dtype=np.float64):
        out = np.empty(int(n), dtype=dtype)
        if n:
            self.ctx.d2h(out, darr.ptr)
        return out

    def _k(self, name, genes, cname, *args):
        if self.time_kernels:
            self.ctx.timer_start()
            self.ctx.call(cname, *args)
            ms = self.ctx.timer_stop()
            self.kernel_log.setdefault(name, []).append((ms, int(genes)))
        else:
            self.ctx.call(cname, *args)
        if cname in ("dsq_dev_alpha_mle", "dsq_dev_alpha_mle2", "dsq_dev_alpha_mle3", "dsq_dev_alpha_mle4"):
            kms, ng = C.c_float(), C.c_int()
            self.ctx.call("dsq_last_alpha_kernel", C.byref(kms), C.byref(ng))
            if kms.value >= 0.0:
                self.kernel_log.setdefault("k_alpha", []).append((float(kms.value), int(genes)))
                self.kernel_log.setdefault("k_alpha_stage", []).append((name, int(genes)))
                self.kernel_log.setdefault("grid_fallback_genes", []).append((float(ng.value), int(genes)))

    _F64 = ("nm", "mom", "gw", "fit", "map", "disp", "p", "stat", "se", "rd")
    _U8 = ("gconv", "mconv", "outl", "lconv", "any_all", "any_use", "any_use_nr", "few_above", "naz")

    def _slab_layout(self, Gs):
        off, o = {}, 0
        for k in self._F64:
            off[k] = o
            o += 8 * Gs
        off["beta"] = o
        o += 8 * Gs * self.P
        n_f64 = o
        for k in self._U8:
            off[k] = o
            o += Gs
        return off, n_f64, ((o + 63) // 64) * 64

    def _dev_slab(self, Gs):
        off, n_f64, total = self._slab_layout(Gs)
        base = self._take(total)
        v = {k: _View(base + o) for k, o in off.items()}
        v["_base"], v["_off"], v["_n_f64"], v["_total"], v["_Gs"] = base, off, n_f64, total, Gs
        return v

    def _host_slab(self, nbytes):
        return self._pinned.take(nbytes)

    def _fetch(self, slab, names=None):
        tok = self._fetch_begin(slab, names)
        self.ctx.sync()
        return self._fetch_end(tok)

    def _fetch_begin(self, slab, names=None):
        Gs, off = slab["_Gs"], slab["_off"]
        width = lambda k: Gs * (8 * self.P if k == "beta" else (8 if k in self._F64 else 1))
        if names is None:
            host, hoff = self._host_slab(slab["_total"]), off
            self.ctx.call("dsq_d2h_async", _vp(host.ptr), _vp(slab["_base"]), C.c_size_t(slab["_total"]))
            names = list(self._F64) + ["beta"] + list(self._U8)
        else:
            hoff, o = {}, 0
            for k in names:
                hoff[k] = o
                o += (width(k) + 63) // 64 * 64
            host = self._host_slab(o)
            for k in names:
                self.ctx.call("dsq_d2h_async", _vp(host.ptr + hoff[k]), _vp(slab["_base"] + off[k]),
                              C.c_size_t(width(k)))
        return host, hoff, names, Gs

    def _fetch_end(self, tok):
        host, hoff, names, Gs = tok
        out = {}
        for k in names:
            if k == "beta":
                out[k] = host.view(hoff[k], Gs * self.P, np.float64).reshape(Gs, self.P)
            elif k in self._F64:
                out[k] = host.view(hoff[k], Gs, np.float64)
            else:
                out[k] = host.view(hoff[k], Gs, np.uint8)
        return out

    def _cells_arg(self):
        return C.byref(self._cells) if self._cells is not None else None

    def _row_lists_for(self, non_zero):
        if self._row_flags is None:
            return None
        c = self._row_lists
        if c is None or not np.array_equal(c[0], non_zero):
            fl = self._row_flags[non_zero]
            rows, waves = np.nonzero(fl >= 0)[0], np.nonzero(fl < 0)[0].astype(np.int32)
            rows = rows[np.argsort(-fl[rows], kind="stable")].astype(np.int32)
            if c is not None:
                c[1].free(); c[3].free()
            d_rows = DeviceArray.from_host(self.ctx, rows if len(rows) else np.zeros(1, np.int32))
            d_waves = DeviceArray.from_host(self.ctx, waves if len(waves) else np.zeros(1, np.int32))
            c = self._row_lists = (non_zero.copy(), d_rows, len(rows), d_waves, len(waves))
        return (c[1], c[2], c[3], c[4]) if c[2] > 0 else None

    def _mix_slots_for(self, d_y, Gs, persistent_key=None):
        if self._mix is None:
            return None
        if persistent_key is not None:
            c = self._mix_ys_cache
            if c is not None and np.array_equal(c[0], persistent_key):
                return c[1], c[2]
            if c is not None:
                c[1].free(); c[2].free()
            d_ys = DeviceArray(self.ctx, (max(Gs, 1) * self._mix_slots,), np.uint16)
            d_big = DeviceArray(self.ctx, (max(Gs, 1),), np.uint8)
        else:
            d_ys = self._pooled((max(Gs, 1) * self._mix_slots,), np.uint16)
            d_big = self._pooled((max(Gs, 1),), np.uint8)
        self.ctx.call("dsq_dev_mix_counts_to_slots", _vp(d_y.ptr), self.ldn, Gs, _vp(self._mix), _vp(d_ys.ptr),
                      _vp(d_big.ptr))
        if persistent_key is not None:
            self._mix_ys_cache = (np.array(persistent_key, copy=True), d_ys, d_big)
        return d_ys, d_big

    def _mix_bind(self, slots, d_mu_slots=None, genes=0):
        if slots is not None:
            self.ctx.call("dsq_mix_bind2", _vp(slots[0].ptr), _vp(slots[1].ptr), _vp(d_mu_slots.ptr) if d_mu_slots else None,
                          int(genes))

    def _stage_genewise(self, d_y, Gs, d_sf, S, row_lists=None, pre_alpha=None, mix_slots=None):
        D = self.design
        mh = type("MuHat", (), {})()
        mh.d_mu, mh.d_coef, mh.d_cell_mu, mh.d_beta, mh.row_lists = None, None, None, None, row_lists
        mh.mix_slots, mh.d_mu_slots, mh.d_beta_fit = mix_slots, None, None
        if D.linear_mu:
            mh.d_coef = self._dvec(Gs * self.P)
            if self.ctx.lib.dsq_alpha_needs_mu(self.N, self.P, int(D.n_design_cells) if self._cells is not None else 0):
                mh.d_mu = self._dmat(Gs)
            self._k("mom_lin_mu", Gs, "dsq_dev_mom_lin_coef", _vp(d_y.ptr), self.ldn, _vp(d_sf.ptr),
                    _vp(self.d_Xt.ptr), _vp(self.d_pinv.ptr), D.ldx, self.N, Gs, self.P, c_double(self.min_disp),
                    c_double(self.max_disp), c_double(self.min_mu), _vp(S["nm"].ptr), _vp(S["mom"].ptr),
                    _vp(mh.d_mu.ptr) if mh.d_mu else None, _vp(mh.d_coef.ptr))
        else:
            per_cell = (self._row_mode == 2 and row_lists is not None and row_lists[3] == 0
                        and not self.ctx.lib.dsq_alpha_needs_mu(self.N, self.P, int(D.n_design_cells)))
            from_beta = self._row_mode == 3 and row_lists is not None and row_lists[3] == 0
            mh.d_mu = None if (per_cell or from_beta) else self._dmat(Gs)
            self._k("mom", Gs, "dsq_dev_mom", _vp(d_y.ptr), self.ldn, _vp(d_sf.ptr), _vp(self.d_Xt.ptr),
                    _vp(self.d_pinv.ptr), D.ldx, self.N, Gs, self.P, c_double(self.min_disp), c_double(self.max_disp),
                    _vp(S["nm"].ptr), None, None, _vp(S["mom"].ptr))
            d_b, d_c = self._dvec(Gs * self.P), self._dvec(Gs, np.uint8)
            S["_irls_it"] = self._dvec(Gs, np.int32)
            self._mix_bind(mix_slots, genes=Gs)
            self._k("irls_mu", Gs, "dsq_dev_lfc_fit2", _vp(d_y.ptr), self.ldn, _vp(d_sf.ptr), _vp(self.d_Xt.ptr),
                    _vp(self.d_pinv.ptr), D.ldx, self.N, Gs, self.P, int(D.full_rank), _vp(S["mom"].ptr),
                    c_double(self.min_mu), c_double(self.beta_tol), c_double(-30.0), c_double(30.0), self.irls_maxiter,
                    _vp(d_b.ptr), _vp(mh.d_mu.ptr) if mh.d_mu else None, None, _vp(d_c.ptr), _vp(S["_irls_it"].ptr),
                    self._cells_arg(),
                    None, None, c_double(0.0), None, None, None, None, None,
                    None, None, c_double(0.0), 0, None, None, None, _vp(self._mix) if self._mix else None, 0)
            mh.d_beta_fit = d_b
            if from_beta:
                mh.d_beta = d_b
                if mix_slots is not None:
                    mh.d_mu_slots = self._pooled((max(Gs, 1) * self._mix_slots,), np.float64)
                    self.ctx.call("dsq_dev_mix_mu_slots", _vp(self._mix), _vp(d_b.ptr), _vp(d_sf.ptr), Gs,
                                  _vp(mh.d_mu_slots.ptr))
            if per_cell:
                mh.d_cell_mu = self._dvec(Gs * int(D.n_design_cells))
                self.ctx.call("dsq_dev_cell_mu", _vp(d_b.ptr), self._cells_arg(), Gs, self.P, _vp(mh.d_cell_mu.ptr))
        mh.nll_const = self._dvec(Gs)
        if pre_alpha is not None:
            pre_alpha()
        self._alpha_fit("alpha_mle", d_y, mh, Gs, d_sf, S["mom"], 1.0, 0, S["gw"], S["gconv"], 1)
        return mh

    def _alpha_fit(self, name, d_y, mh, Gs, d_sf, d_start, prior_var, prior_reg, d_out, d_conv, const_mode):
        d_nfev = self._dvec(Gs, np.int32) if self.collect_nfev else None
        d_cell_mu = getattr(mh, "d_cell_mu", None)
        d_beta = getattr(mh, "d_beta", None)
        use_coef = mh.d_mu is None and d_cell_mu is None and d_beta is None
        use_cell = d_cell_mu is not None
        mix = self._mix if (self._row_mode == 3 and getattr(mh, "row_lists", None) is not None) else None
        rows = getattr(mh, "row_lists", None) if (mh.d_mu is None or mix) else None
        if mix and rows:
            self._mix_bind(getattr(mh, "mix_slots", None), getattr(mh, "d_mu_slots", None), genes=Gs)
        self._k(name, Gs, "dsq_dev_alpha_mle4", _vp(d_y.ptr), _vp(mh.d_mu.ptr) if mh.d_mu else None, self.ldn,
                _vp(self.d_Xt.ptr), self.design.ldx, self.N, Gs, self.P, _vp(d_start.ptr), c_double(self.min_disp),
                c_double(self.max_disp), c_double(prior_var), 1, int(prior_reg), _vp(d_out.ptr), _vp(d_conv.ptr),
                _vp(d_nfev.ptr) if d_nfev else None, _vp(mh.nll_const.ptr), const_mode, self._cells_arg(),
                _vp(mh.d_coef.ptr) if use_coef else None, _vp(d_sf.ptr) if (use_coef or use_cell or d_beta) else None,
                c_double(self.min_mu), _vp(rows[0].ptr) if rows else None, rows[1] if rows else 0,
                _vp(rows[2].ptr) if rows and rows[3] else None, rows[3] if rows else 0,
                _vp(d_cell_mu.ptr) if use_cell else None, _vp(mix) if (mix and rows) else None,
                _vp(d_beta.ptr) if d_beta else None)
        if d_nfev:
            self.kernel_log.setdefault("nfev", []).append((float(self._down(d_nfev, Gs, np.int32).sum()), Gs))

    def _stage_map(self, d_y, mh, Gs, d_sf, prior_var, squared_logres, S, fork=None):
        if fork is not None:
            self.ctx.call("dsq_alpha_set_late_flags", _vp(fork[1].ptr))
        self._alpha_fit("alpha_map", d_y, mh, Gs, d_sf, S["fit"], prior_var, 1, S["map"], S["mconv"], 2)
        if fork is not None:
            d_part, d_late, forked = fork
            if not forked():
                self.ctx.call("dsq_memset", _vp(d_part.ptr), 0, C.c_size_t(Gs))
            self.ctx.call("dsq_dev_select_dispersions_part", _vp(S["gw"].ptr), _vp(S["map"].ptr), _vp(S["fit"].ptr), Gs,
                          c_double(self.min_disp), c_double(self.max_disp), c_double(squared_logres),
                          _vp(S["disp"].ptr), _vp(S["outl"].ptr), _vp(S["mconv"].ptr), _vp(d_late.ptr), _vp(d_part.ptr),
                          0, 0)
        else:
            self.ctx.call("dsq_dev_select_dispersions", _vp(S["gw"].ptr), _vp(S["map"].ptr), _vp(S["fit"].ptr), Gs,
                          c_double(self.min_disp), c_double(self.max_disp), c_double(squared_logres),
                          _vp(S["disp"].ptr), _vp(S["outl"].ptr))

    def _stage_lfc(self, d_y, Gs, d_sf, S, wald, cooks=None, mix_slots=None, bufs=None, part=None):
        D = self.design
        want = self.keep_layers and cooks is not None
        if bufs is not None:
            d_mu, d_hat = bufs
        else:
            d_mu = self._dmat(Gs) if want else None
            d_hat = self._dmat(Gs) if want else None
        ridge, contrast, lfc_null, alt = wald
        ck = [None, None, c_double(0.0), None, None, None, None, None]
        cooks_ld = 0
        if cooks is not None:
            d_rd, cutoff, d_cooks = cooks
            cooks_ld = self._cooks_ld()
            ck = [_vp(d_rd.ptr), _vp(self.d_flags.ptr), c_double(cutoff), _vp(d_cooks.ptr)] + \
                 [_vp(S[x].ptr) for x in ("any_all", "any_use", "any_use_nr", "few_above")]
        if S.get("_irls_it") is not None:
            self.ctx.call("dsq_irls_order_hint", _vp(S["_irls_it"].ptr), Gs)
        self._mix_bind(mix_slots, genes=Gs)
        if part is not None:
            self.ctx.call("dsq_lfc_set_part", _vp(part[0].ptr), int(part[1]), int(part[2]))
        self._k("lfc_fit", Gs, "dsq_dev_lfc_fit2", _vp(d_y.ptr), self.ldn, _vp(d_sf.ptr), _vp(self.d_Xt.ptr),
                _vp(self.d_pinv.ptr), D.ldx, self.N, Gs, self.P, int(D.full_rank), _vp(S["disp"].ptr),
                c_double(self.min_mu), c_double(self.beta_tol), c_double(-30.0), c_double(30.0), self.irls_maxiter,
                _vp(S["beta"].ptr), _vp(d_mu.ptr) if d_mu else None, _vp(d_hat.ptr) if d_hat else None,
                _vp(S["lconv"].ptr), None, self._cells_arg(), *ck,
                _vp(ridge.ctypes.data), _vp(contrast.ctypes.data), c_double(lfc_null), alt,
                _vp(S["p"].ptr), _vp(S["stat"].ptr), _vp(S["se"].ptr), _vp(self._mix) if self._mix else None, cooks_ld)
        return d_mu, d_hat

    def _replace_rows(self, Gr):
        if self._replace_buf is None or self._replace_buf.shape[0] < Gr:
            if self._replace_buf is not None:
                self.ctx.sync()
                self._replace_buf.free()
            self._replace_buf = DeviceArray(self.ctx, (int(Gr), self.N), np.int32, ld=self.ldn)
        return self._replace_buf

    def _cooks_ld(self):
        if self._mix and self.ctx.lib.dsq_mix_takes_irls(_vp(self._mix), int(self.design.full_rank)):
            return self._mix_slots
        return 0

    def _size_factors(self, d_lm):
        if self._work is None:
            self._work = DeviceArray(self.ctx, (self.ctx.lib.dsq_size_factors_work_doubles(self.N, self.G),),
                                     np.float64)
        d_sf = self._dvec(self.N)
        d_lm, d_mask = self._sf_inputs(d_lm)
        self._k("size_factors", self.G, "dsq_dev_size_factors", _vp(self.d_raw.ptr), self._count_type, self.N,
                self.G, _vp(d_lm.ptr), _vp(d_mask.ptr) if d_mask is not None else None, _vp(self._work.ptr),
                _vp(d_sf.ptr))
        return self._sf_finish(d_sf)

    def _sf_inputs(self, d_lm):
        d_mask = None
        if self.size_factors_fit_type == "poscounts":
            d_lm, d_use = self._dvec(self.G), self._dvec(self.G, np.uint8)
            self.ctx.call("dsq_dev_logmeans_poscounts", _vp(self.d_y.ptr), self.ldn, self.N, self.G, _vp(d_lm.ptr),
                          _vp(d_use.ptr))
            d_mask = d_use
            if self._control_mask is not None:
                d_mask = self._up(self._down(d_use, self.G, np.uint8) & self._control_mask, np.uint8)
        elif self._control_mask is not None:
            d_mask = self._up(self._control_mask, np.uint8)
        return d_lm, d_mask

    def _sf_finish(self, d_sf):
        if self.size_factors_fit_type == "poscounts":
            sf = self._down(d_sf, self.N)
            d_sf = self._up(sf / np.exp(np.mean(np.log(sf))))
        return d_sf

    def _fit_trend(self, Gn):
        d_gw, d_nm = self._last_gw_dev
        return self._run_trend_kernel(d_gw, d_nm, Gn)

    def _run_trend_kernel(self, d_gw, d_nm, n):
        c2, ok, n_outer = (C.c_double * 2)(), C.c_int(0), C.c_int(0)
        d_keep = self._dvec(n, np.uint8)
        self._k("trend_fit", n, "dsq_dev_trend_fit", _vp(d_gw.ptr), _vp(d_nm.ptr), int(n),
                c_double(self.min_disp), c_double(self.max_disp), _vp(d_keep.ptr), c2, C.byref(ok),
                C.byref(n_outer))
        return np.array([c2[0], c2[1]]) if ok.value else None

    def _trend_prior_fused(self, Gn, d_fit):
        d_gw, d_nm = self._last_gw_dev
        c2, ok, n_outer, sq = (C.c_double * 2)(), C.c_int(0), C.c_int(0), C.c_double()
        d_keep = self._dvec(Gn, np.uint8)
        d_work = self._dvec(self.ctx.lib.dsq_prior_mad_work_doubles(int(Gn)))
        self.ctx.call("dsq_dev_trend_prior", _vp(d_gw.ptr), _vp(d_nm.ptr), int(Gn), c_double(self.min_disp),
                      c_double(self.max_disp), _vp(d_keep.ptr), _vp(d_fit.ptr), _vp(d_work.ptr), c2, C.byref(ok),
                      C.byref(n_outer), C.byref(sq))
        if not ok.value:
            return None, None
        return np.array([c2[0], c2[1]]), float(sq.value)

    def _mean_trend(self, Gn):
        d_gw, _ = self._last_gw_dev
        gw = np.clip(self._down(d_gw, Gn), self.min_disp, self.max_disp)
        return _trend.mean_trend(gw, self.min_disp)

    def _prior(self, Gn, d_fit, r):
        d_gw, _ = self._last_gw_dev
        sq = C.c_double()
        d_work = self._dvec(self.ctx.lib.dsq_prior_mad_work_doubles(int(Gn)))
        self._k("prior_mad", Gn, "dsq_dev_prior_mad", _vp(d_gw.ptr), _vp(d_fit.ptr), Gn,
                c_double(self.min_disp), c_double(self.max_disp), _vp(d_work.ptr), C.byref(sq))
        sq = float(sq.value)
        return sq, float(max(sq - _trigamma((self.N - self.P) / 2), 0.25))

    STAGES = ("open", "size_factors", "genewise", "trend", "map", "lfc", "refit", "finish")

    def deseq2(self, contrast=None, lfc_null=0.0, alt_hypothesis=None, profile=False,
               stop_after_trend=False, stop_after_size_factors=False, size_factors=None) -> DeseqResult:
        upto = "size_factors" if stop_after_size_factors else ("trend" if stop_after_trend else "finish")
        while True:
            st = self.begin_step(contrast, lfc_null, alt_hypothesis, profile=profile, size_factors=size_factors,
                                 upto=upto)
            try:
                return self.advance(st, upto)
            except _Respeculate:
                continue

    def begin_step(self, contrast=None, lfc_null=0.0, alt_hypothesis=None, *, profile=False, size_factors=None,
                   upto=None):
        if alt_hypothesis not in ALT:
            raise KeyError(alt_hypothesis)
        if lfc_null < 0 and alt_hypothesis in {"greaterAbs", "lessAbs"}:
            raise ValueError(f"The alternative hypothesis being {alt_hypothesis}, please provide a "
                             f"positive lfc_null value (got {lfc_null}).")
        if contrast is None:
            contrast = np.zeros(self.P)
# ... 676 lines not shown
```

Measured before the change: 10.85 million.

## Regroup samples by design cell into padded slots in the row-alpha kernel

```diff
diff --git a/include/deseq_hip.h b/include/deseq_hip.h
--- a/include/deseq_hip.h
+++ b/include/deseq_hip.h
@@ -191,6 +191,20 @@
                        const double* d_coef, const double* d_sf, double min_mu, const int32_t* d_rows, int n_rows,
                        const int32_t* d_waves, int n_waves, const double* d_cell_mu, const dsq_mix* mix,
                        const double* d_beta);
+typedef struct dsq_row_plan {
+    const uint16_t* d_slot_of;
+    int32_t trips[4];
+} dsq_row_plan;
+int dsq_row_slot_plan(const int32_t* h_cell_of, int N, int n_cells, uint16_t* h_slot_of, int32_t* h_first,
+                      int32_t* h_trips);
+int dsq_row_slots_bound(int N, int n_cells);
+int dsq_dev_alpha_mle5(dsq_ctx* ctx, const int32_t* d_y, const double* d_mu, int ldn, const double* d_Xt, int ldx,
+                       int N, int G, int P, const double* d_alpha_hat, double min_disp, double max_disp,
+                       double prior_disp_var, int cr_reg, int prior_reg, double* d_alpha, uint8_t* d_converged,
+                       int32_t* d_nfev, double* d_nll_const, int const_mode, const dsq_cells* cells,
+                       const double* d_coef, const double* d_sf, double min_mu, const int32_t* d_rows, int n_rows,
+                       const int32_t* d_waves, int n_waves, const double* d_cell_mu, const dsq_mix* mix,
+                       const double* d_beta, const dsq_row_plan* row_plan);
 int dsq_alpha_rows_eligible(int N, int P, int n_cells);
 int dsq_alpha_needs_mu(int N, int P, int n_cells);
 int dsq_dev_cell_mu(dsq_ctx* ctx, const double* d_beta, const dsq_cells* cells, int G, int P, double* d_cell_mu);
diff --git a/pydeseq2_amd/_lib.py b/pydeseq2_amd/_lib.py
--- a/pydeseq2_amd/_lib.py
+++ b/pydeseq2_amd/_lib.py
@@ -23,6 +23,11 @@
 class DsqCells(C.Structure):
 
     _fields_ = [("d_cell_of", C.c_void_p), ("d_Xc", C.c_void_p), ("d_XX", C.c_void_p), ("n_cells", C.c_int)]
+
+
+class DsqRowPlan(C.Structure):
+
+    _fields_ = [("d_slot_of", C.c_void_p), ("trips", C.c_int32 * 4)]
 
 
 class DsqError(RuntimeError):
@@ -148,6 +153,11 @@
     proto("dsq_dev_alpha_mle4", _vp, _vp, _vp, c_int, _vp, c_int, c_int, c_int, c_int, _vp, c_double, c_double,
           c_double, c_int, c_int, _vp, _vp, _vp, _vp, c_int, cells_p, _vp, _vp, c_double, _vp, c_int, _vp, c_int, _vp,
           _vp, _vp)
+    proto("dsq_dev_alpha_mle5", _vp, _vp, _vp, c_int, _vp, c_int, c_int, c_int, c_int, _vp, c_double, c_double,
+          c_double, c_int, c_int, _vp, _vp, _vp, _vp, c_int, cells_p, _vp, _vp, c_double, _vp, c_int, _vp, c_int, _vp,
+          _vp, _vp, C.POINTER(DsqRowPlan))
+    proto("dsq_row_slot_plan", _vp, c_int, c_int, _vp, _vp, _vp)
+    proto("dsq_row_slots_bound", c_int, c_int)
     proto("dsq_mix_create", _vp, _vp, c_int, c_int, C.POINTER(_vp))
     proto("dsq_mix_destroy", _vp, res=None)
     proto("dsq_mix_launch_count")
@@ -237,6 +247,7 @@
     "dsq_mix_bind", "dsq_mix_bind2", "dsq_dev_mix_counts_to_slots", "dsq_dev_mix_mu_slots",
     "dsq_lfc_fork_begin", "dsq_lfc_fork_end", "dsq_lfc_set_part", "dsq_lfc_takes_parts", "dsq_dev_select_dispersions_part", "dsq_lfc_prepare", "dsq_alpha_set_late_flags",
     "dsq_dev_lrt", "dsq_dev_chisq_sf",
+    "dsq_dev_alpha_mle5", "dsq_row_slot_plan", "dsq_row_slots_bound",
 ]
 
 
diff --git a/pydeseq2_amd/csrc/dsq_alpha_rows.h b/pydeseq2_amd/csrc/dsq_alpha_rows.h
--- a/pydeseq2_amd/csrc/dsq_alpha_rows.h
+++ b/pydeseq2_amd/csrc/dsq_alpha_rows.h
@@ -23,6 +23,35 @@
     return (sizeof(RowGene) + (size_t)npad * 2 + (size_t)kRowTail * 2 + 15) & ~(size_t)15;
 }
 
+constexpr int kRowTrip = kRowLanes * 4;
+DSQ_HD int row_slots_bound(int N, int C) { return ((N + kRowTrip - 1) / kRowTrip + (C - 1)) * kRowTrip; }
+DSQ_HD int row_plan_slots(const int* trips, int C) {
+    int t = 0;
+    for (int c = 0; c < C; ++c) t += trips[c];
+    return t * kRowTrip;
+}
+inline int row_slot_plan(const int32_t* cell_of, int N, int C, uint16_t* slot_of, int32_t* first, int32_t* trips) {
+    if (cell_of == nullptr || slot_of == nullptr || first == nullptr || trips == nullptr || N < 1 || C < 1) return -1;
+    for (int c = 0; c < C; ++c) trips[c] = 0;
+    for (int n = 0; n < N; ++n) {
+        if (cell_of[n] < 0 || cell_of[n] >= C) return -1;
+        trips[cell_of[n]] += 1;
+    }
+    int total = 0;
+    for (int c = 0; c < C; ++c) {
+        first[c] = total;
+        trips[c] = (trips[c] + kRowTrip - 1) / kRowTrip;
+        total += trips[c] * kRowTrip;
+    }
+    if (total > 65535) return -1;
+    for (int c = 0; c < C; ++c) {
+        int next = first[c];
+        for (int n = 0; n < N; ++n)
+            if (cell_of[n] == c) slot_of[n] = (uint16_t)next++;
+    }
+    return total;
+}
+
 DSQ_D void stirling_big(double z, double& lg, double& psi) {
     const double l = flog_t(z), rc = frcp(z);
     lg = (z - 0.5) * l - z + kHalfLog2Pi + stirling_tail_big(rc);
diff --git a/pydeseq2_amd/csrc/dsq_capi_dev.hip b/pydeseq2_amd/csrc/dsq_capi_dev.hip
--- a/pydeseq2_amd/csrc/dsq_capi_dev.hip
+++ b/pydeseq2_amd/csrc/dsq_capi_dev.hip
@@ -1,4 +1,5 @@
 #include "dsq_capi_internal.h"
+#include "dsq_alpha_rows.h"
 
 extern "C" {
 
@@ -147,13 +148,13 @@
 }
 
 
-int dsq_dev_alpha_mle4(dsq_ctx* ctx, const int32_t* d_y, const double* d_mu, int ldn, const double* d_Xt, int ldx,
+int dsq_dev_alpha_mle5(dsq_ctx* ctx, const int32_t* d_y, const double* d_mu, int ldn, const double* d_Xt, int ldx,
                        int N, int G, int P, const double* d_alpha_hat, double min_disp, double max_disp,
                        double prior_disp_var, int cr_reg, int prior_reg, double* d_alpha, uint8_t* d_converged,
                        int32_t* d_nfev, double* d_nll_const, int const_mode, const dsq_cells* cells,
                        const double* d_coef, const double* d_sf, double min_mu, const int32_t* d_rows, int n_rows,
                        const int32_t* d_waves, int n_waves, const double* d_cell_mu, const dsq_mix* mix,
-                       const double* d_beta) {
+                       const double* d_beta, const dsq_row_plan* row_plan) {
     DSQ_CHECK_ARG(P >= 1 && P <= DSQ_MAX_P, "P out of range");
     DSQ_CHECK_ARG(const_mode >= DSQ_CONST_COMPUTE && const_mode <= DSQ_CONST_LOAD, "const_mode out of range");
     DSQ_CHECK_ARG(d_mu != nullptr || (d_coef != nullptr && d_sf != nullptr) ||
@@ -176,8 +177,24 @@
     if (d_mu == nullptr) { ex.coef = d_coef; ex.cell_mu = d_cell_mu; ex.sf = d_sf; ex.min_mu = min_mu; }
     if (d_rows != nullptr) { ex.rows = d_rows; ex.n_rows = n_rows; ex.waves = d_waves; ex.n_waves = n_waves; }
     if (mix != nullptr) { ex.mix = &mix->d; ex.mix_beta = d_beta; ex.sf = d_sf; }
+    if (row_plan != nullptr) {
+        ex.row_plan.slot_of = row_plan->d_slot_of;
+        for (int c = 0; c < 4; ++c) ex.row_plan.trips[c] = row_plan->trips[c];
+    }
     return run_alpha(ctx, d_y, d_mu, ldn, d_Xt, ldx, N, G, P, d_alpha_hat, min_disp, max_disp, prior_disp_var, cr_reg,
                      prior_reg, d_alpha, d_converged, d_nfev, d_nll_const, const_mode, &ex);
+}
+
+int dsq_dev_alpha_mle4(dsq_ctx* ctx, const int32_t* d_y, const double* d_mu, int ldn, const double* d_Xt, int ldx,
+                       int N, int G, int P, const double* d_alpha_hat, double min_disp, double max_disp,
+                       double prior_disp_var, int cr_reg, int prior_reg, double* d_alpha, uint8_t* d_converged,
+                       int32_t* d_nfev, double* d_nll_const, int const_mode, const dsq_cells* cells,
+                       const double* d_coef, const double* d_sf, double min_mu, const int32_t* d_rows, int n_rows,
+                       const int32_t* d_waves, int n_waves, const double* d_cell_mu, const dsq_mix* mix,
+                       const double* d_beta) {
+    return dsq_dev_alpha_mle5(ctx, d_y, d_mu, ldn, d_Xt, ldx, N, G, P, d_alpha_hat, min_disp, max_disp, prior_disp_var,
+                              cr_reg, prior_reg, d_alpha, d_converged, d_nfev, d_nll_const, const_mode, cells, d_coef,
+                              d_sf, min_mu, d_rows, n_rows, d_waves, n_waves, d_cell_mu, mix, d_beta, nullptr);
 }
 
 int dsq_dev_alpha_mle3(dsq_ctx* ctx, const int32_t* d_y, const double* d_mu, int ldn, const double* d_Xt, int ldx,
@@ -411,6 +428,14 @@
 
 int dsq_alpha_needs_mu(int N, int P, int n_cells) { return dsq::alpha_needs_mu(N, P, n_cells) ? 1 : 0; }
 
+int dsq_row_slot_plan(const int32_t* h_cell_of, int N, int n_cells, uint16_t* h_slot_of, int32_t* h_first,
+                      int32_t* h_trips) {
+    if (n_cells < 1 || n_cells > 4) return -1;
+    return dsq::row_slot_plan(h_cell_of, N, n_cells, h_slot_of, h_first, h_trips);
+}
+
+int dsq_row_slots_bound(int N, int n_cells) { return dsq::row_slots_bound(N, n_cells); }
+
 int dsq_alpha_rows_eligible(int N, int P, int n_cells) {
     if (dsq::alpha_rows_eligible(N, P, n_cells, true, 1)) return 1;
     return dsq::alpha_rowsc_tail(N, P, n_cells) > 0 ? 2 : 0;
diff --git a/pydeseq2_amd/csrc/dsq_k_alpha.hip b/pydeseq2_amd/csrc/dsq_k_alpha.hip
--- a/pydeseq2_amd/csrc/dsq_k_alpha.hip
+++ b/pydeseq2_amd/csrc/dsq_k_alpha.hip
@@ -362,10 +362,10 @@
                           nll_const != nullptr && ex.eval_cap > 0 && !no_two_phase();
         hipError_t e;
         if (rows_reg)
-            e = launch_alpha_rows(st, y, ldn, N, ex.rows, ex.n_rows, queue, ex.coef, ex.sf, ex.cells, P_, ex.min_mu,
-                                  alpha_hat, min_disp, max_disp, prior_var, cr_reg, prior_reg, alpha, conv, nfev,
-                                  grid_count, grid_list, nll_const, const_mode, park ? ex.eval_cap : 0, ex.resume_state,
-                                  ex.resume_count, ex.resume_list);
+            e = launch_alpha_rows(st, y, ldn, N, ex.rows, ex.n_rows, queue, ex.coef, ex.sf, ex.cells, ex.row_plan, P_,
+                                  ex.min_mu, alpha_hat, min_disp, max_disp, prior_var, cr_reg, prior_reg, alpha, conv,
+                                  nfev, grid_count, grid_list, nll_const, const_mode, park ? ex.eval_cap : 0,
+                                  ex.resume_state, ex.resume_count, ex.resume_list);
         else
             e = launch_alpha_rows_c(st, y, ldn, N, ex.rows, ex.n_rows, queue, ex.coef, ex.cell_mu, ex.sf, ex.cells, P_,
                                     ex.min_mu, alpha_hat, min_disp, max_disp, prior_var, prior_reg, alpha, conv, nfev,
diff --git a/pydeseq2_amd/csrc/dsq_k_alpha_rows.hip b/pydeseq2_amd/csrc/dsq_k_alpha_rows.hip
--- a/pydeseq2_amd/csrc/dsq_k_alpha_rows.hip
+++ b/pydeseq2_amd/csrc/dsq_k_alpha_rows.hip
@@ -23,7 +23,7 @@
 __global__ __launch_bounds__(kRowBlock, 2) void k_alpha_rows(
     const int32_t* __restrict__ y, int ldn, int N, const int32_t* __restrict__ list, int n_list,
     int32_t* __restrict__ queue, const double* __restrict__ coef, const double* __restrict__ sf,
-    const int32_t* __restrict__ cell_of, const double* __restrict__ Xc, const double* __restrict__ XXc, double min_mu,
+    const RowSlotPlan plan, const double* __restrict__ Xc, const double* __restrict__ XXc, double min_mu,
     const double* __restrict__ alpha_hat, double min_disp, double max_disp, double prior_var, int cr_reg, int prior_reg,
     double* __restrict__ alpha_out, uint8_t* __restrict__ conv, int32_t* __restrict__ nfev,
     int32_t* __restrict__ grid_count, int32_t* __restrict__ grid_list, double* __restrict__ nll_const, int const_mode,
@@ -32,28 +32,31 @@
     constexpr int T = Tri<P>::N;
     extern __shared__ __attribute__((aligned(16))) double dyn[];
     const int npad = (N + 63) & ~63;
+    const int ns = row_plan_slots(plan.trips, C);
     double* const sf_s = dyn;
-    uint8_t* const cell_s = (uint8_t*)(sf_s + npad);
-    char* const slots0 = (char*)(cell_s + npad);
-    const size_t slot_bytes = row_slot_bytes(npad);
+    char* const slots0 = (char*)(sf_s + ns);
+    const size_t slot_bytes = row_slot_bytes(ns);
     unsigned int* const hist0 = (unsigned int*)(slots0 + slot_bytes * kRowSlots * kRowWaves);
+    const uint16_t* __restrict__ const slot_map = plan.slot_of;
 
     const int lane = threadIdx.x & 63, w = threadIdx.x >> 6;
     const int row = lane >> 4, rl = lane & 15;
     log_tab_fill();
-    for (int n = threadIdx.x; n < npad; n += kRowBlock) {
-        sf_s[n] = n < N ? sf[n] : 0.0;
-        cell_s[n] = (uint8_t)(n < N ? cell_of[n] : 0);
-    }
+    for (int n = threadIdx.x; n < ns; n += kRowBlock) sf_s[n] = 0.0;
     __syncthreads();
+    for (int n = threadIdx.x; n < N; n += kRowBlock) {
+        const int sl = slot_map[n];
+        if (sl < ns) sf_s[sl] = sf[n];
+    }
 
     auto slot_of = [&](int r) { return (RowGene*)(slots0 + slot_bytes * (size_t)(w * kRowSlots + r)); };
     RowGene* const S = slot_of(row);
     uint16_t* const cnt = (uint16_t*)((char*)S + sizeof(RowGene));
-    uint16_t* const tail = cnt + npad;
+    uint16_t* const tail = cnt + ns;
     unsigned int* const hist = hist0 + (size_t)w * kRowTail;
     if (rl == 0) { S->g = -1; S->n_tail = 0; S->n_big = 0; }
-    DeviceWave::sync();
+    for (int n = rl; n < ns; n += kRowLanes) cnt[n] = 0;
+    __syncthreads();
 
     const double lo = log(min_disp), hi = log(max_disp);
     double xx[C][T];
@@ -85,7 +88,7 @@
                 const int r = src >> 4;
                 RowGene* const Sr = slot_of(r);
                 uint16_t* const cr = (uint16_t*)((char*)Sr + sizeof(RowGene));
-                uint16_t* const tr = cr + npad;
+                uint16_t* const tr = cr + ns;
                 for (int i = lane; i < kRowTail; i += 64) hist[i] = 0u;
                 double q[C];
                 {
@@ -107,19 +110,20 @@
                 int maxc = 0, nbig = 0;
                 constexpr int CH = 8;
                 for (int base = 0; base < npad; base += 64 * CH) {
-                    int v8[CH];
+                    int v8[CH], s8[CH];
 #pragma unroll
                     for (int k = 0; k < CH; ++k) {
                         const int n = base + 64 * k + lane;
                         v8[k] = n < N ? yg[n] : 0;
+                        s8[k] = n < N ? (int)slot_map[n] : 0;
                     }
 #pragma unroll
                     for (int k = 0; k < CH; ++k) {
                         const int n = base + 64 * k + lane;
                         if (base + 64 * k >= npad) break;
                         const bool in = n < N;
-                        const int v = v8[k];
-                        cr[n] = (uint16_t)v;
+                        const int v = v8[k], sl = s8[k];
+                        if (in && sl < ns) cr[sl] = (uint16_t)v;
                         maxc = v > maxc ? v : maxc;
                         const bool isbig = v >= kRowTail;
                         if (in && v > 0 && !isbig) atomicAdd(&hist[v], 1u);
@@ -133,11 +137,14 @@
                         }
                         nbig += __popcll(bm);
                         if (want_cst && in) {
-                            const int cl = cell_s[n];
                             double qq = q[0];
-#pragma unroll
-                            for (int c = 1; c < C; ++c) qq = (cl == c) ? q[c] : qq;
-                            const double mu = dmax(sf_s[n] * qq, min_mu);
+                            int end = 0;
+#pragma unroll
+                            for (int c = 1; c < C; ++c) {
+                                end += plan.trips[c - 1] * kRowTrip;
+                                qq = (sl >= end) ? q[c] : qq;
+                            }
+                            const double mu = dmax(sf_s[sl < ns ? sl : 0] * qq, min_mu);
                             cs.add(-((double)v * flog_t(mu)));
                         }
                     }
@@ -202,7 +209,7 @@
                 double lgM, psiM;
                 stirling_big((double)kRowTail + a, lgM, psiM);
                 if (nb > 0) {
-                    for (int n = rl; n < npad; n += kRowLanes) {
+                    for (int n = rl; n < ns; n += kRowLanes) {
                         const int yi = cnt[n];
                         if (yi >= kRowTail) {
                             double lgz, psiz;
@@ -215,31 +222,29 @@
             }
         }
         ROWS_PH(3);
-        double q[C], wc[C], dwc[C];
-#pragma unroll
-        for (int c = 0; c < C; ++c) { q[c] = S->q[c]; wc[c] = 0.0; dwc[c] = 0.0; }
+        double wc[C], dwc[C];
+#pragma unroll
+        for (int c = 0; c < C; ++c) { wc[c] = 0.0; dwc[c] = 0.0; }
         constexpr int U = 4;
+        static_assert(kRowLanes * U == kRowTrip, "a trip of the loop is a trip of the slot plan");
         KSum af[U];
         double ag[U];
 #pragma unroll
         for (int u = 0; u < U; ++u) ag[u] = 0.0;
-        double wt = 0.0, dwt = 0.0;
-        for (int n0 = rl; n0 < npad; n0 += kRowLanes * U) {
-            int yi[U], cl[U];
+        double qc = 0.0, wt = 0.0, dwt = 0.0;
+        auto trip = [&](const int n0, auto last) {
+            constexpr bool LAST = decltype(last)::value;
+            int yi[U];
             double sfn[U], m[U], r1[U], L1[U];
 #pragma unroll
             for (int u = 0; u < U; ++u) {
                 yi[u] = cnt[n0 + kRowLanes * u];
                 sfn[u] = sf_s[n0 + kRowLanes * u];
-                cl[u] = cell_s[n0 + kRowLanes * u];
             }
 #pragma unroll
             for (int u = 0; u < U; ++u) {
-                double qq = q[0];
-#pragma unroll
-                for (int c = 1; c < C; ++c) qq = (cl[u] == c) ? q[c] : qq;
-                const double mm = dmax(sfn[u] * qq, min_mu);
-                m[u] = (sfn[u] == 0.0) ? 0.0 : mm;
+                const double mm = dmax(sfn[u] * qc, min_mu);
+                m[u] = (LAST && sfn[u] == 0.0) ? 0.0 : mm;
             }
 #pragma unroll
             for (int u = 0; u < U; ++u) r1[u] = frcp(1.0 + m[u] * alpha);
@@ -267,23 +272,28 @@
                 af[u].add(yv * (L1[u] - lal) + a * L1[u]);
                 ag[u] += L1[u] + (yv - m[u]) * alpha * r1[u];
                 const double wv = m[u] * r1[u];
-                const double dwv = -(wv * wv);
                 wt += wv;
-                dwt += dwv;
-#pragma unroll
-                for (int c = 1; c < C; ++c) {
-                    const double on = (cl[u] == c) ? 1.0 : 0.0;
-                    wc[c] = fma(wv, on, wc[c]);
-                    dwc[c] = fma(dwv, on, dwc[c]);
-                }
-            }
-        }
+                dwt -= wv * wv;
+            }
+        };
         {
-            double rest = 0.0, drest = 0.0;
-#pragma unroll
-            for (int c = 1; c < C; ++c) { rest += wc[c]; drest += dwc[c]; }
-            wc[0] = wt - rest;
-            dwc[0] = dwt - drest;
+            int n0 = rl;
+#pragma unroll 1
+            for (int c = 0; c < C; ++c) {
+                const int nt = plan.trips[c];
+                if (nt <= 0) continue;
+                qc = S->q[c];
+                wt = 0.0;
+                dwt = 0.0;
+                for (int t = 1; t < nt; ++t, n0 += kRowTrip) trip(n0, std::false_type{});
+                trip(n0, std::true_type{});
+                n0 += kRowTrip;
+#pragma unroll
+                for (int k = 0; k < C; ++k) {
+                    wc[k] = (k == c) ? wt : wc[k];
+                    dwc[k] = (k == c) ? dwt : dwc[k];
+                }
+            }
         }
 #pragma unroll
         for (int u = 0; u < U; ++u) { accf.merge(af[u].s, af[u].c); accg += ag[u]; }
@@ -599,28 +609,31 @@
     return hipGetLastError();
 }
 
-size_t alpha_rows_smem(int N) {
-    const int npad = (N + 63) & ~63;
-    return (size_t)npad * 8 + (size_t)npad + row_slot_bytes(npad) * kRowSlots * kRowWaves +
-           (size_t)kRowWaves * kRowTail * 4;
+size_t alpha_rows_smem(int n_slots) {
+    return (size_t)n_slots * 8 + row_slot_bytes(n_slots) * kRowSlots * kRowWaves + (size_t)kRowWaves * kRowTail * 4;
 }
 
 bool alpha_rows_eligible(int N, int P_, int n_cells, bool has_coef, int cr_reg) {
     static const bool off = getenv("DSQ_NO_ALPHA_ROWS") != nullptr;
-    return !off && has_coef && cr_reg != 0 && P_ >= 1 && P_ <= 4 && n_cells == P_ && N <= 65535 &&
-           alpha_rows_smem(N) <= 78 * 1024;
+    return !off && has_coef && cr_reg != 0 && P_ >= 1 && P_ <= 4 && n_cells == P_ && N >= 1 && N <= 65535 &&
+           alpha_rows_smem(row_slots_bound(N, n_cells)) <= 78 * 1024;
 }
 
 hipError_t launch_alpha_rows(hipStream_t st, const int32_t* y, int ldn, int N, const int32_t* list, int n_list,
-                             int32_t* queue, const double* coef, const double* sf, const CellDesign& cells, int P_,
-                             double min_mu, const double* alpha_hat, double min_disp, double max_disp, double prior_var,
-                             int cr_reg, int prior_reg, double* alpha, uint8_t* conv, int32_t* nfev, int32_t* grid_count,
-                             int32_t* grid_list, double* nll_const, int const_mode, int eval_cap, void* park_state,
-                             int32_t* park_count, int32_t* park_list) {
+                             int32_t* queue, const double* coef, const double* sf, const CellDesign& cells,
+                             const RowSlotPlan& plan, int P_, double min_mu, const double* alpha_hat, double min_disp,
+                             double max_disp, double prior_var, int cr_reg, int prior_reg, double* alpha, uint8_t* conv,
+                             int32_t* nfev, int32_t* grid_count, int32_t* grid_list, double* nll_const, int const_mode,
+                             int eval_cap, void* park_state, int32_t* park_count, int32_t* park_list) {
     if (n_list <= 0) return hipSuccess;
     const int n_cu = current_device_cus();
     if (n_cu <= 0) return hipGetLastError();
-    const size_t smem = alpha_rows_smem(N);
+    if (P_ < 1 || P_ > 4 || plan.slot_of == nullptr) return hipErrorInvalidValue;
+    const int n_slots = row_plan_slots(plan.trips, P_);
+    for (int c = 0; c < P_; ++c)
+        if (plan.trips[c] < 0) return hipErrorInvalidValue;
+    if (n_slots < N || n_slots > row_slots_bound(N, P_)) return hipErrorInvalidValue;
+    const size_t smem = alpha_rows_smem(n_slots);
     const int per_block = kRowSlots * kRowWaves;
     int blocks = (n_list + per_block - 1) / per_block;
     if (blocks > 2 * n_cu) blocks = 2 * n_cu;
@@ -639,7 +652,7 @@
                     blocks, n_list, nb);                                                                             \
         }                                                                                                            \
         hipLaunchKernelGGL(k_alpha_rows<PP>, dim3(blocks), dim3(kRowBlock), smem, st, y, ldn, N, list, n_list, queue, \
-                           coef, sf, cells.cell_of, cells.Xc, cells.XX, min_mu, alpha_hat, min_disp, max_disp,       \
+                           coef, sf, plan, cells.Xc, cells.XX, min_mu, alpha_hat, min_disp, max_disp,                \
                            prior_var, cr_reg, prior_reg, alpha, conv, nfev, grid_count, grid_list, nll_const,        \
                            const_mode, eval_cap, (Lbfgsb1d*)park_state, park_count, park_list);                     \
     } while (0)
diff --git a/pydeseq2_amd/csrc/dsq_launch.h b/pydeseq2_amd/csrc/dsq_launch.h
--- a/pydeseq2_amd/csrc/dsq_launch.h
+++ b/pydeseq2_amd/csrc/dsq_launch.h
@@ -95,6 +95,10 @@
                              const double* d_contrast, double lfc_null, int alt, double* pvals, double* stats,
                              double* se);
 
+struct RowSlotPlan {
+    const uint16_t* slot_of;
+    int trips[4];
+};
 struct AlphaExtras {
     CellDesign cells;
     const double* coef;
@@ -120,17 +124,18 @@
     const double* mix_beta;
     const uint16_t* mix_ys;
     const double* mix_mu;
+    RowSlotPlan row_plan;
 };
 constexpr int kAlphaEvalCap = 8;
 size_t alpha_resume_bytes(int G);
 constexpr int kRowTail = 512;
 bool alpha_rows_eligible(int N, int P, int n_cells, bool has_coef, int cr_reg);
 hipError_t launch_alpha_rows(hipStream_t st, const int32_t* y, int ldn, int N, const int32_t* list, int n_list,
-                             int32_t* queue, const double* coef, const double* sf, const CellDesign& cells, int P,
-                             double min_mu, const double* alpha_hat, double min_disp, double max_disp, double prior_var,
-                             int cr_reg, int prior_reg, double* alpha, uint8_t* conv, int32_t* nfev, int32_t* grid_count,
-                             int32_t* grid_list, double* nll_const, int const_mode, int eval_cap, void* park_state,
-                             int32_t* park_count, int32_t* park_list);
+                             int32_t* queue, const double* coef, const double* sf, const CellDesign& cells,
+                             const RowSlotPlan& plan, int P, double min_mu, const double* alpha_hat, double min_disp,
+                             double max_disp, double prior_var, int cr_reg, int prior_reg, double* alpha, uint8_t* conv,
+                             int32_t* nfev, int32_t* grid_count, int32_t* grid_list, double* nll_const, int const_mode,
+                             int eval_cap, void* park_state, int32_t* park_count, int32_t* park_list);
 hipError_t launch_count_big(hipStream_t st, const int32_t* y, int ldn, int N, int G, int32_t* out);
 int alpha_rowsc_tail(int N, int P, int n_cells);
 hipError_t launch_alpha_rows_c(hipStream_t st, const int32_t* y, int ldn, int N, const int32_t* list, int n_list,
diff --git a/pydeseq2_amd/pipeline.py b/pydeseq2_amd/pipeline.py
--- a/pydeseq2_amd/pipeline.py
+++ b/pydeseq2_amd/pipeline.py
@@ -10,7 +10,7 @@
 
 from . import trend as _trend
 from ._design import DesignPack, pad16
-from ._lib import ALT, HOOK_FN, I32, I64, SAMPLE_MAJOR, Context, DeviceArray, DsqCells, _PinnedPool, _PinnedSlab
+from ._lib import ALT, HOOK_FN, I32, I64, SAMPLE_MAJOR, Context, DeviceArray, DsqCells, DsqRowPlan, _PinnedPool, _PinnedSlab
 
 import ctypes as C
 import functools
@@ -168,6 +168,16 @@
             int(ctx_.lib.dsq_alpha_rows_eligible(self.N, self.P, int(D.n_design_cells)))
         if self._row_mode == 1 and not D.linear_mu:
             self._row_mode = 0
+        self._row_plan = None
+        if self._row_mode == 1:
+            slot_of, plan = np.empty(self.N, dtype=np.uint16), DsqRowPlan()
+            first = (C.c_int32 * 4)()
+            if ctx_.lib.dsq_row_slot_plan(_vp(D.cell_of.ctypes.data), self.N, int(D.n_design_cells),
+                                          _vp(slot_of.ctypes.data), first, plan.trips) < 0:
+                raise RuntimeError("dsq_row_slot_plan failed")
+            self._d_slot_of = DeviceArray.from_host(ctx_, slot_of)
+            plan.d_slot_of = self._d_slot_of.ptr
+            self._row_plan = plan
         self._mix, self._mix_slots, self._slot_of, self._mix_ys_cache = None, 0, None, None
         if self._row_mode == 0 and not D.linear_mu and not os.environ.get("DSQ_NO_ALPHA_MIX"):
             mp = _vp()
@@ -295,7 +305,8 @@
             self.kernel_log.setdefault(name, []).append((ms, int(genes)))
         else:
             self.ctx.call(cname, *args)
-        if cname in ("dsq_dev_alpha_mle", "dsq_dev_alpha_mle2", "dsq_dev_alpha_mle3", "dsq_dev_alpha_mle4"):
+        if cname in ("dsq_dev_alpha_mle", "dsq_dev_alpha_mle2", "dsq_dev_alpha_mle3", "dsq_dev_alpha_mle4",
+                     "dsq_dev_alpha_mle5"):
             kms, ng = C.c_float(), C.c_int()
             self.ctx.call("dsq_last_alpha_kernel", C.byref(kms), C.byref(ng))
             if kms.value >= 0.0:
@@ -464,7 +475,7 @@
         rows = getattr(mh, "row_lists", None) if (mh.d_mu is None or mix) else None
         if mix and rows:
             self._mix_bind(getattr(mh, "mix_slots", None), getattr(mh, "d_mu_slots", None), genes=Gs)
-        self._k(name, Gs, "dsq_dev_alpha_mle4", _vp(d_y.ptr), _vp(mh.d_mu.ptr) if mh.d_mu else None, self.ldn,
+        self._k(name, Gs, "dsq_dev_alpha_mle5", _vp(d_y.ptr), _vp(mh.d_mu.ptr) if mh.d_mu else None, self.ldn,
                 _vp(self.d_Xt.ptr), self.design.ldx, self.N, Gs, self.P, _vp(d_start.ptr), c_double(self.min_disp),
                 c_double(self.max_disp), c_double(prior_var), 1, int(prior_reg), _vp(d_out.ptr), _vp(d_conv.ptr),
                 _vp(d_nfev.ptr) if d_nfev else None, _vp(mh.nll_const.ptr), const_mode, self._cells_arg(),
@@ -472,7 +483,7 @@
                 c_double(self.min_mu), _vp(rows[0].ptr) if rows else None, rows[1] if rows else 0,
                 _vp(rows[2].ptr) if rows and rows[3] else None, rows[3] if rows else 0,
                 _vp(d_cell_mu.ptr) if use_cell else None, _vp(mix) if (mix and rows) else None,
-                _vp(d_beta.ptr) if d_beta else None)
+                _vp(d_beta.ptr) if d_beta else None, C.byref(self._row_plan) if self._row_plan is not None else None)
         if d_nfev:
             self.kernel_log.setdefault("nfev", []).append((float(self._down(d_nfev, Gs, np.int32).sum()), Gs))
 
```

New measurement: 10.78 million. No clear change (-0.6%).
